# hangg7/soar

Hardware: AMD Instinct MI355X
Metric: fwd+bwd frames/sec @100k Gaussians, 1080p; achieved HBM GB/s vs roofline (higher is better)
Workload: dtype f32

## Files before the change

### include/soar_hip.h

```cpp
#ifndef SOAR_HIP_H
#define SOAR_HIP_H

#include <stddef.h>
#include <stdint.h>

#ifdef __cplusplus
extern "C" {
#endif

#define SOAR_HIP_ABI_VERSION 8

typedef struct SoarRastParams {
    int32_t P;
    int32_t W, H;
    int32_t sh_degree;
    int32_t M;
    int32_t prefiltered;
    int32_t render_front;
    int32_t sort_descending;
    int32_t debug;
    int32_t cfg_surface;
    int32_t cfg_normalize_depth;
    int32_t cfg_perpix_depth;
    int32_t cfg_lrn_cam;
// ... 38 lines not shown
                             void *geom_buffer, void *binning_buffer, void *image_buffer,
                             int64_t num_rendered,
                             float *out_color, float *out_normal, float *out_depth, float *out_opac,
                             void *stream);

int soar_rast_forward_render_occ(const SoarRastParams *prm, const int32_t *radii,
                                 void *geom_buffer, void *binning_buffer, void *image_buffer,
                                 int64_t num_rendered,
                                 float *out_color, float *out_normal, float *out_depth, float *out_opac,
                                 const float *occ_values, float *out_occ,
                                 void *stream);

int soar_rast_backward(const SoarRastParams *prm,
                       const float *means3D, const int32_t *radii, const float *shs,
                       const float *colors_precomp, const float *scales, const float *rotations,
                       const float *cov3D_precomp,
                       const void *geom_buffer, const void *binning_buffer, const void *image_buffer,
                       int64_t num_rendered,
                       const float *dL_dout_color, const float *dL_dout_normal,
                       const float *dL_dout_depth, const float *dL_dout_opac,
                       float *dL_dmeans2D, float *dL_dcolors, float *dL_dopacity, float *dL_dmeans3D,
                       float *dL_dcov3D, float *dL_dsh, float *dL_dscales, float *dL_drotations,
                       float *dL_dviewmat, float *dL_dprojmat, float *dL_dcampos,
                       void *workspace, size_t workspace_bytes,
                       void *stream);
int soar_rast_occ_backward(const SoarRastParams *prm, const void *geom_buffer, const void *binning_buffer,
                           const void *image_buffer, int64_t num_rendered, const float *dL_dout_occ, float *dL_docc,
                           void *stream);
int soar_rast_backward_occ(const SoarRastParams *prm,
                           const float *means3D, const int32_t *radii, const float *shs,
                           const float *colors_precomp, const float *scales, const float *rotations,
                           const float *cov3D_precomp,
                           const void *geom_buffer, const void *binning_buffer, const void *image_buffer,
                           int64_t num_rendered,
                           const float *dL_dout_color, const float *dL_dout_normal,
                           const float *dL_dout_depth, const float *dL_dout_opac, const float *dL_dout_occ,
                           const float *normal_scale_dev,
                           int32_t occ_planes,
                           float *dL_dmeans2D, float *dL_dcolors, float *dL_dopacity, float *dL_dmeans3D,
                           float *dL_dcov3D, float *dL_dsh, float *dL_dscales, float *dL_drotations,
                           float *dL_dviewmat, float *dL_dprojmat, float *dL_dcampos, float *dL_docc,
                           void *workspace, size_t workspace_bytes,
                           void *stream);
int soar_rast_backward_scaled(const SoarRastParams *prm,
                              const float *means3D, const int32_t *radii, const float *shs,
                              const float *colors_precomp, const float *scales, const float *rotations,
                              const float *cov3D_precomp,
                              const void *geom_buffer, const void *binning_buffer, const void *image_buffer,
                              int64_t num_rendered,
                              const float *dL_dout_color, const float *dL_dout_normal,
                              const float *dL_dout_depth, const float *dL_dout_opac, const float *grad_scale_dev,
                              float *dL_dmeans2D, float *dL_dcolors, float *dL_dopacity, float *dL_dmeans3D,
                              float *dL_dcov3D, float *dL_dsh, float *dL_dscales, float *dL_drotations,
                              float *dL_dviewmat, float *dL_dprojmat, float *dL_dcampos,
                              void *workspace, size_t workspace_bytes,
                              void *stream);
int soar_rast_backward_plan(const SoarRastParams *prm, int32_t region,
                            const float *means3D, const int32_t *radii, const float *shs,
                            const float *colors_precomp, const float *scales, const float *rotations,
                            const float *cov3D_precomp,
                            const void *geom_buffer, const void *binning_buffer, const void *image_buffer,
                            int64_t num_rendered,
                            const float *dL_dout_color, const float *dL_dout_normal,
                            const float *dL_dout_depth, const float *dL_dout_opac,
                            float *dL_dmeans2D, float *dL_dcolors, float *dL_dopacity, float *dL_dmeans3D,
                            float *dL_dcov3D, float *dL_dsh, float *dL_dscales, float *dL_drotations,
                            float *dL_dviewmat, float *dL_dprojmat, float *dL_dcampos,
                            void *workspace, size_t workspace_bytes,
                            void *stream);
int soar_rast_backward_occ_plan(const SoarRastParams *prm, int32_t region,
                                const float *means3D, const int32_t *radii, const float *shs,
                                const float *colors_precomp, const float *scales, const float *rotations,
                                const float *cov3D_precomp,
                                const void *geom_buffer, const void *binning_buffer, const void *image_buffer,
                                int64_t num_rendered,
                                const float *dL_dout_color, const float *dL_dout_normal,
                                const float *dL_dout_depth, const float *dL_dout_opac, const float *dL_dout_occ,
                                const float *normal_scale_dev, int32_t occ_planes,
                                float *dL_dmeans2D, float *dL_dcolors, float *dL_dopacity, float *dL_dmeans3D,
                                float *dL_dcov3D, float *dL_dsh, float *dL_dscales, float *dL_drotations,
                                float *dL_dviewmat, float *dL_dprojmat, float *dL_dcampos, float *dL_docc,
                                void *workspace, size_t workspace_bytes,
                                void *stream);
int soar_rast_backward_region_counts(int64_t *single_blocks, int64_t *pairs);
int soar_rast_backward_workspace_bytes(int32_t P, size_t *bytes);

int soar_rast_mark_visible(int32_t P, const float *means3D, const float *viewmatrix, const float *projmatrix,
                           uint8_t *present, void *stream);

int soar_rast_export_state(const SoarRastParams *prm, const void *geom_buffer, const void *binning_buffer,
                           const void *image_buffer, int64_t num_rendered,
                           float *means2D, float *depths, float *conic_opacity, float *normal,
                           float *depth_plane, float *rgb, float *cov3D,
                           uint32_t *tiles_touched, uint32_t *point_offsets,
                           uint64_t *keys_unsorted, uint32_t *vals_unsorted,
                           uint64_t *keys_sorted, uint32_t *point_list, uint32_t *ranges,
                           float *final_T, float *final_D, uint32_t *n_contrib, void *stream);

int soar_lbs_knn_weights_bytes(int32_t P, int32_t V, size_t *bytes);
int soar_lbs_knn_weights(const float *xyz, int32_t P, const float *verts, int32_t V,
                         const float *vert_weights, int32_t J, int32_t K,
                         float *weights_out, int32_t *knn_idx_out,
                         void *workspace, size_t workspace_bytes, void *stream);

int soar_lbs_knn_grid_bytes(int32_t V, size_t *bytes);
int soar_lbs_knn_query_bytes(int32_t P, size_t *bytes);
int soar_lbs_knn_build_grid(const float *verts, int32_t V, const float *vert_weights, int32_t J, void *grid_buffer,
                            void *stream);
int soar_lbs_knn_query(const void *grid_buffer, int32_t V, const float *vert_weights, int32_t J,
                       const float *xyz, int32_t P, int32_t K, float *weights_out, int32_t *knn_idx_out,
                       void *query_workspace, size_t query_workspace_bytes, void *stream);
int soar_lbs_knn_query_ordered(const void *grid_buffer, int32_t V, const float *vert_weights, int32_t J,
                               const float *xyz, int32_t P, int32_t K, uint32_t *order, int32_t resort,
                               float *weights_out, int32_t *knn_idx_out,
                               void *query_workspace, size_t query_workspace_bytes, void *stream);

int soar_lbs_knn_state_bytes(int32_t P, size_t *bytes);
int soar_lbs_knn_query_state(const void *grid_buffer, int32_t V, const float *vert_weights, int32_t J, const float *xyz, int32_t P,
                             uint32_t *order, int32_t resort, float *weights_out, void *state_buffer, void *query_workspace,
                             size_t query_workspace_bytes, void *stream);
int soar_lbs_knn_refresh(const void *grid_buffer, int32_t V, int32_t J, const float *xyz, int32_t P, const uint32_t *order,
                         void *state_buffer, float *weights_out, uint32_t *searched_counter_dev, void *stream);

int soar_lbs_warp_forward(const float *xyz, const float *rot, const float *weights, const float *joint_mats,
                          const float *offsets, const float *axis_perm, int32_t P, int32_t J,
                          float *xyz_out, float *rot_out, float *pt_mats_out, void *stream);

int soar_lbs_warp_backward(const float *xyz, const float *rot, const float *weights, const float *joint_mats,
                           const float *axis_perm, int32_t P, int32_t J,
                           const float *dL_dxyz_out, const float *dL_drot_out,
                           float *dL_dxyz, float *dL_drot, void *stream);

typedef struct SoarFrameHead {
    const SoarRastParams *prm;
    void *geom_buffer;
    int32_t *radii;
} SoarFrameHead;
int soar_frames_warp_preprocess(int32_t n, const SoarFrameHead *frames, const float *xyz, const float *rot, const float *weights,
                                const float *joint_mats, int32_t P, int32_t J, const float *colors, const float *opacities, const float *scales,
                                float *xyz_out, float *rot_out, void *stream);

int soar_rast_backward_rows(const SoarRastParams *prm, const float *means3D, const int32_t *radii, const float *shs, const float *scales,
                            const float *rotations, const float *cov3D_precomp, const void *geom_buffer, const void *workspace,
                            float *dL_dmeans2D, float *dL_dcolors, float *dL_dopacity, float *dL_dmeans3D, float *dL_dcov3D, float *dL_dsh,
                            float *dL_dscales, float *dL_drotations, float *dL_dviewmat, float *dL_dprojmat, float *dL_dcampos, float *dL_docc,
                            void *stream);

typedef struct SoarFrameTail {
    const SoarRastParams *prm;
    const float *means3D;
    const float *rotations;
    const int32_t *radii;
    const void *geom_buffer;
    const void *workspace;
    float *dL_dmeans2D;
} SoarFrameTail;
int soar_frames_geometry_warp_backward(int32_t n, const SoarFrameTail *frames, const float *xyz, const float *rot, const float *weights,
                                       const float *joint_mats, int32_t P, int32_t J, const float *scales, float *dL_dxyz, float *dL_drot,
                                       float *dL_dscales, float *dL_dcolors, float *dL_docc, void *stream);
typedef struct SoarLossFinish {
    const float *sums4;
    float *loss_out;
    int32_t blocks, n;
    float w_color, w_mask, w_normal, w_depth;
} SoarLossFinish;
int soar_frames_geometry_warp_backward_losses(int32_t n, const SoarFrameTail *frames, const float *xyz, const float *rot,
// ... 114 lines not shown
    int32_t scale_width;
    int32_t warp;
    const float *xyz, *rot;
    const float *weights;
    const float *joint_mats;
    const float *offsets;
    const float *axis_perm;
    const float *colors;
    const float *scale_src;
    const float *occ;
    float *occ3;
    float *posed;
    float *grad_scratch;
    float *dL_dxyz, *dL_drot, *dL_dcolors, *dL_dscale;
    float *dL_docc;
} SoarPoseArgs;
typedef struct SoarViewArgs {
    SoarRastParams rast;
    float focal_k00, focal_k11;
    int32_t back;
    int32_t pad_;
    int64_t capacity;
    void *buffer;
    size_t buffer_bytes;
    float *out;
    int32_t *radii;
    uint32_t *status_pinned;
    const float *g_render, *g_normal, *g_depth, *g_pred_normal, *g_mask, *g_occ, *g_curv;
    float *dL_dmeans2D;
} SoarViewArgs;
int soar_view_buffer_bytes(int32_t P, int32_t W, int32_t H, int64_t capacity, int32_t back, size_t *bytes);
int soar_views_grad_scratch_floats(int32_t P, int32_t n_views, size_t *floats);
int soar_views_forward(const SoarPoseArgs *pose, int32_t n_views, const SoarViewArgs *views, void *stream);
int soar_views_backward(const SoarPoseArgs *pose, int32_t n_views, const SoarViewArgs *views, void *stream);
int soar_step_views_forward(int32_t n_poses, const SoarPoseArgs *poses, const int32_t *views_per_pose, const SoarViewArgs *views, void *stream);
int soar_step_views_backward(int32_t n_poses, const SoarPoseArgs *poses, const int32_t *views_per_pose, const SoarViewArgs *views, void *stream);
typedef struct SoarCameraSpec {
    double fovx, fovy, znear, zfar;
    double cx, cy, img_w, img_h;
    int32_t has_cxcy, pad_;
} SoarCameraSpec;
int soar_cameras_from_c2w(int32_t n, const float *c2w_dev, const float *c2w_host, const SoarCameraSpec *specs, float *out_dev, void *stream);
int soar_rast_forward_render_status(const SoarRastParams *prm, const int32_t *radii, void *geom_buffer, void *binning_buffer,
                                    void *image_buffer, int64_t num_rendered, float *out_color, float *out_normal, float *out_depth,
                                    float *out_opac, const float *occ_values, float *out_occ, uint32_t *status_pinned, void *stream);
int soar_lbs_warp_backward_views(const float *xyz, const float *rot, const float *weights, const float *joint_mats, const float *axis_perm,
                                 int32_t n, int32_t P, int32_t J, const float *dL_dxyz_out, const float *dL_drot_out, float *dL_dxyz,
                                 float *dL_drot, int32_t n_extra, const float *const *extra_src, float *const *extra_dst,
                                 const int32_t *extra_width, void *stream);

int soar_prof_enable(int on);
int soar_prof_reset(void);
int soar_prof_stage_count(void);
const char *soar_prof_stage_name(int stage);
int soar_prof_read(int stage, double *total_ms, int64_t *launches);
int soar_sum_frames(int32_t n_frames, int64_t count, const float *in_dev, float *out_dev, void *stream);
int soar_gather_step_inputs(int32_t n_frames, int32_t num_frames_seq, int32_t floats_per_frame, int32_t n_sets,
                            const int32_t *frame_ids_dev, const float *table_dev, float *mats_out_dev,
                            int32_t *set_index_out_dev, void *stream);
int soar_gather_step_inputs_ids(int32_t n_frames, int32_t num_frames_seq, int32_t floats_per_frame, int32_t n_sets,
                                const int32_t *frame_ids_host, const float *table_dev, float *mats_out_dev,
                                int32_t *set_index_out_dev, void *stream);

typedef struct SoarAdamRow {
    float *param;
    const float *grad;
    float *exp_avg;
    float *exp_avg_sq;
    int64_t count;
    float lr;
    int32_t pad_;
} SoarAdamRow;
int soar_adam_step(int32_t n_rows, const SoarAdamRow *rows_host, double beta1, double beta2, double eps, void *state_dev, void *stream);
int soar_adam_step_at(int32_t n_rows, const SoarAdamRow *rows, double beta1, double beta2, double eps, int64_t step, void *stream);
int soar_adam_step_at_gather(int32_t n_rows, const SoarAdamRow *rows, double beta1, double beta2, double eps, int64_t step,
                             int32_t n_frames, int32_t num_frames_seq, int32_t floats_per_frame, int32_t n_sets,
                             const int32_t *frame_ids_host, const float *table_dev, float *mats_out_dev, int32_t *set_index_out_dev,
                             void *stream);
int soar_adam_step_rows(int32_t n_rows, const SoarAdamRow *rows, double beta1, double beta2, double eps, void *state_dev, int32_t advance,
                        void *stream);
int soar_adam_step_rows_wide(int32_t n_rows, const SoarAdamRow *rows, double beta1, double beta2, double eps, void *state_dev,
                             int32_t advance, void *stream);

int soar_prof_timestamp(unsigned long long *ring_dev, int64_t capacity, int64_t tag, void *stream);

int soar_selftest_affine_scan(const float *m64_dev, const float *b64_dev, float *out192_dev, void *stream);

int soar_selftest_exp(const float *x_dev, int32_t n, float *out_dev, float *expf_dev, void *stream);

int soar_tsdf_integrate(int32_t n_views, int32_t H, int32_t W, const float *depth, const float *opac, const float *viewmatrix,
                        const float *projmatrix, const float *prcppoint, float origin_x, float origin_y, float origin_z, float voxel,
                        int32_t X, int32_t Y, int32_t Z, float trunc, float znear, float min_opacity, float *sum, float *weight,
                        void *stream);
int soar_mc_workspace_bytes(int32_t X, int32_t Y, int32_t Z, size_t *bytes);
int soar_mc_count(int32_t X, int32_t Y, int32_t Z, const float *values, const uint8_t *valid, float level, void *workspace,
                  size_t workspace_bytes, int64_t *counts_host, void *stream);
int soar_mc_emit(int32_t X, int32_t Y, int32_t Z, const float *values, const uint8_t *valid, float level, const void *workspace,
                 size_t workspace_bytes, float *verts, int32_t *faces, void *stream);
int soar_mesh_filter_bytes(int32_t V, int32_t F, size_t *bytes);
int soar_mesh_filter_components(int32_t V, int32_t F, const float *verts, const int32_t *faces, int32_t min_faces, float min_diag_frac,
                                void *workspace, size_t workspace_bytes, float *verts_out, int32_t *faces_out, int64_t *counts_host,
                                void *stream);
int soar_mesh_simplify_bytes(int32_t V, int32_t F, size_t *bytes);
int soar_mesh_simplify_count(int32_t V, int32_t F, const float *verts, const int32_t *faces, float cell, void *workspace,
                             size_t workspace_bytes, int64_t *counts_host, void *stream);
int soar_mesh_simplify(int32_t V, int32_t F, const float *verts, const int32_t *faces, float cell, void *workspace,
                       size_t workspace_bytes, float *verts_out, int32_t *faces_out, int64_t *counts_host, void *stream);
int soar_mesh_attr_transfer_bytes(int32_t V, int32_t K, size_t *bytes);
int soar_mesh_attr_transfer(int32_t V, int32_t N, int32_t K, const float *verts, const float *points, const float *colors,
                            const int32_t *idx, void *workspace, size_t workspace_bytes, float *color_out, float *quality_out,
                            float *d2_out, void *stream);
int soar_mesh_adjacency_bytes(int32_t V, int32_t F, size_t *bytes);
int soar_mesh_adjacency(int32_t V, int32_t F, const int32_t *faces, void *workspace, size_t workspace_bytes, int32_t *row_start,
                        int32_t *nbr, uint8_t *border, void *stream);
int soar_mesh_smooth_bytes(int32_t V, size_t *bytes);
int soar_mesh_smooth(int32_t V, int32_t nnz, const float *verts, const int32_t *row_start, const int32_t *nbr, const uint8_t *border,
                     int32_t steps, void *workspace, size_t workspace_bytes, float *verts_out, void *stream);
int soar_mesh_prune_bytes(int32_t V, int32_t F, size_t *bytes);
int soar_mesh_prune(int32_t V, int32_t F, const float *verts, const int32_t *faces, const float *quality, float thresh, void *workspace,
                    size_t workspace_bytes, float *verts_out, int32_t *faces_out, int32_t *keep_out, int64_t *counts_host, void *stream);
int soar_mesh_close_holes_bytes(int32_t V, int32_t F, size_t *bytes);
int soar_mesh_close_holes(int32_t V, int32_t F, const float *verts, const int32_t *faces, int32_t max_hole_edges, void *workspace,
                          size_t workspace_bytes, float *verts_out, int32_t *faces_out, int32_t *loop_edges_out, int64_t *counts_host,
                          void *stream);

#define SOAR_FIELD_LEVELS 16
#define SOAR_FIELD_HIDDEN 64
#define SOAR_FIELD_HEAD_FLOATS(in, out) (SOAR_FIELD_HIDDEN * (in) + SOAR_FIELD_HIDDEN + (out) * SOAR_FIELD_HIDDEN + (out))
typedef struct SoarFieldHead {
    const float *w1, *b1, *w2, *b2;
} SoarFieldHead;

typedef struct SoarFieldArgs {
    int32_t N;
    int32_t log2_T;
    int32_t normalized;
    int32_t pad_;
    float res[SOAR_FIELD_LEVELS];
    const float *xyz;
    const float *aabb;
    const float *table, *qtable;
    const float *z;
    SoarFieldHead head[5];
    float *enc, *qenc;
    float *out[5];
    const float *g_out[5];
    float *d_table, *d_qtable;
    float *d_head[5];
    float *d_xyz, *d_z;
} SoarFieldArgs;

int soar_field_workspace_bytes(int32_t N, size_t *bytes);
int soar_field_forward(const SoarFieldArgs *args, void *stream);
int soar_field_backward(const SoarFieldArgs *args, void *workspace, size_t workspace_bytes, void *stream);

#define SOAR_ENVMAP_ENC 9
#define SOAR_ENVMAP_HIDDEN 16
#define SOAR_ENVMAP_WEIGHTS (SOAR_ENVMAP_HIDDEN * SOAR_ENVMAP_ENC + SOAR_ENVMAP_HIDDEN * SOAR_ENVMAP_HIDDEN + 3 * SOAR_ENVMAP_HIDDEN)
typedef struct SoarEnvmapArgs {
    int32_t B, H, W;
    int32_t n_comp;
    int32_t color_rows;
    int32_t pad_;
    int64_t render_stride, mask_stride;
    int64_t g_comp_stride[4];
    const float *dirs;
// ... 166 lines not shown
```

### soar_amd/csrc/api.hip

```cpp
#include "soar_common.h"

#include <mutex>

#include <dlfcn.h>

#include <cstdarg>
#include <cstdio>
#include <cstring>

namespace soar {

static thread_local char g_error[1024] = "";

void set_error(const char *fmt, ...)
{
    va_list ap;
    va_start(ap, fmt);
    vsnprintf(g_error, sizeof(g_error), fmt, ap);
    va_end(ap);
}

int check_hip(hipError_t e, const char *what, const char *file, int line)
{
    if (e == hipSuccess) return 0;
// ... 531 lines not shown
            const soar::BatchCtx &bc = soar::batch_ctx();
            if (!bc.n || pending_serial != bc.serial) pending.clear();
            pending_serial = bc.serial;
            status_pinned[0] = 0xFFFFFFFFu;
            status_pinned[1] = 0xFFFFFFFFu;
            pending.push_back({status_pinned, g.header + H_TOTAL});
            if (!bc.n || bc.f == bc.n - 1) {
                for (const auto &c : pending)
                    SOAR_HIP_OK(hipMemcpyAsync(c.first, c.second, 2 * sizeof(uint32_t), hipMemcpyDeviceToHost, stream));
                pending.clear();
            }
        }
    } else {
        if (launch_scan(*prm, g, stream)) return 1;
        if (launch_binning(*prm, g, b, img, num_rendered, stream)) return 1;
    }
    if (num_rendered > 0 && launch_tile_order_binned(*prm, g, b, img, num_rendered, stream)) return 1;
    if (launch_render_forward(*prm, g, b, img, out_color, out_normal, out_depth, out_opac, occ_values, out_occ, stream)) return 1;
    return 0;
}

int soar_rast_occ_backward(const SoarRastParams *prm, const void *geom_buffer, const void *binning_buffer, const void *image_buffer,
                           int64_t num_rendered, const float *dL_dout_occ, float *dL_docc, void *stream_)
{
    hipStream_t stream = static_cast<hipStream_t>(stream_);
    if (check_params(prm)) return 1;
    if (prm->P == 0) return 0;
    if (!dL_dout_occ || !dL_docc) { set_error("soar_rast_occ_backward: a required pointer is NULL"); return 1; }
    if (prm->sort_descending || prm->render_front) {
        set_error("soar_rast_occ_backward: the fused occlusion pass belongs to a main pass with render_front = 0 and sort_descending = 0");
        return 1;
    }
    if (check_aligned(geom_buffer, "geom_buffer") || check_aligned(image_buffer, "image_buffer")) return 1;
    if (num_rendered > 0 && check_aligned(binning_buffer, "binning_buffer")) return 1;
    GeomBuf g;
    ImageBuf img;
    BinBuf b;
    carve_geom(const_cast<void *>(geom_buffer), prm->P, prm->M, &g);
    carve_image(const_cast<void *>(image_buffer), prm->W, prm->H, &img);
    carve_binning(const_cast<void *>(binning_buffer), num_rendered, &b);
    return launch_occ_backward(*prm, g, b, img, dL_dout_occ, dL_docc, stream);
}

int soar_rast_backward(const SoarRastParams *prm, const float *means3D, const int32_t *radii, const float *shs,
                       const float *colors_precomp, const float *scales, const float *rotations,
                       const float *cov3D_precomp, const void *geom_buffer, const void *binning_buffer,
                       const void *image_buffer, int64_t num_rendered, const float *dL_dout_color,
                       const float *dL_dout_normal, const float *dL_dout_depth, const float *dL_dout_opac,
                       float *dL_dmeans2D, float *dL_dcolors, float *dL_dopacity, float *dL_dmeans3D, float *dL_dcov3D,
                       float *dL_dsh, float *dL_dscales, float *dL_drotations, float *dL_dviewmat, float *dL_dprojmat,
                       float *dL_dcampos, void *workspace, size_t workspace_bytes, void *stream_)
{
    return soar_rast_backward_scaled(prm, means3D, radii, shs, colors_precomp, scales, rotations, cov3D_precomp, geom_buffer,
                                     binning_buffer, image_buffer, num_rendered, dL_dout_color, dL_dout_normal, dL_dout_depth,
                                     dL_dout_opac, nullptr, dL_dmeans2D, dL_dcolors, dL_dopacity, dL_dmeans3D, dL_dcov3D, dL_dsh,
                                     dL_dscales, dL_drotations, dL_dviewmat, dL_dprojmat, dL_dcampos, workspace, workspace_bytes,
                                     stream_);
}

int soar_rast_backward_rows(const SoarRastParams *prm, const float *means3D, const int32_t *radii, const float *shs, const float *scales,
                            const float *rotations, const float *cov3D_precomp, const void *geom_buffer, const void *workspace,
                            float *dL_dmeans2D, float *dL_dcolors, float *dL_dopacity, float *dL_dmeans3D, float *dL_dcov3D, float *dL_dsh,
                            float *dL_dscales, float *dL_drotations, float *dL_dviewmat, float *dL_dprojmat, float *dL_dcampos, float *dL_docc,
                            void *stream_)
{
    hipStream_t stream = static_cast<hipStream_t>(stream_);
    if (check_params(prm)) return 1;
    if (prm->P == 0) return 0;
    if (check_aligned(geom_buffer, "geom_buffer") || check_aligned(workspace, "workspace")) return 1;
    if (!means3D || !radii || !dL_dmeans2D || !dL_dcolors || !dL_dopacity || !dL_dmeans3D || !dL_dcov3D || !dL_dscales || !dL_drotations ||
        !dL_dviewmat || !dL_dprojmat || !dL_dcampos) {
        set_error("soar_rast_backward_rows: a required pointer is NULL");
        return 1;
    }
    GeomBuf g;
    carve_geom(const_cast<void *>(geom_buffer), prm->P, prm->M, &g);
    return launch_geometry_backward(*prm, means3D, radii, shs, scales, rotations, cov3D_precomp, g, static_cast<const float *>(workspace),
                                    dL_dmeans2D, dL_dcolors, dL_dopacity, dL_dmeans3D, dL_dcov3D, dL_dsh, dL_dscales, dL_drotations,
                                    dL_dviewmat, dL_dprojmat, dL_dcampos, true, stream, dL_docc);
}

}

static int backward_impl(const SoarRastParams *prm, const float *means3D, const int32_t *radii, const float *shs,
                              const float *colors_precomp, const float *scales, const float *rotations,
                              const float *cov3D_precomp, const void *geom_buffer, const void *binning_buffer,
                              const void *image_buffer, int64_t num_rendered, const float *dL_dout_color,
                              const float *dL_dout_normal, const float *dL_dout_depth, const float *dL_dout_opac,
                              const float *grad_scale_dev, float *dL_dmeans2D, float *dL_dcolors, float *dL_dopacity,
                              float *dL_dmeans3D, float *dL_dcov3D, float *dL_dsh, float *dL_dscales, float *dL_drotations,
                              float *dL_dviewmat, float *dL_dprojmat, float *dL_dcampos, void *workspace,
                              size_t workspace_bytes, const float *dL_dout_occ, float *dL_docc, const float *normal_scale_dev, int occ_planes,
                              int region, void *stream_)
{
    hipStream_t stream = static_cast<hipStream_t>(stream_);
    if (check_params(prm)) return 1;
    if (!dL_dviewmat || !dL_dprojmat || !dL_dcampos) { set_error("camera gradient pointers must not be NULL"); return 1; }
    if ((dL_dout_occ == nullptr) != (dL_docc == nullptr)) { set_error("soar_rast_backward_occ: dL_dout_occ and dL_docc go together"); return 1; }
    if (dL_dout_occ && (prm->render_front != 0 || prm->sort_descending != 0)) {
        set_error("soar_rast_backward_occ: the fused occlusion chain belongs to a main pass (render_front = 0, ascending)");
        return 1;
    }
    if (prm->P == 0) {
        SOAR_HIP_OK(hipMemsetAsync(dL_dviewmat, 0, 16 * sizeof(float), stream));
        SOAR_HIP_OK(hipMemsetAsync(dL_dprojmat, 0, 16 * sizeof(float), stream));
        SOAR_HIP_OK(hipMemsetAsync(dL_dcampos, 0, 3 * sizeof(float), stream));
        return 0;
    }
    if (check_aligned(geom_buffer, "geom_buffer") || check_aligned(image_buffer, "image_buffer") ||
        check_aligned(workspace, "workspace"))
        return 1;
    if (num_rendered > 0 && check_aligned(binning_buffer, "binning_buffer")) return 1;
    size_t need = 0;
    soar_rast_backward_workspace_bytes(prm->P, &need);
    if (workspace_bytes < need - ALIGN) { set_error("workspace too small: %zu < %zu", workspace_bytes, need); return 1; }
    if (!means3D || !radii || !dL_dout_color || !dL_dout_normal || !dL_dout_depth || !dL_dout_opac || !dL_dmeans2D ||
        !dL_dcolors || !dL_dopacity || !dL_dmeans3D || !dL_dcov3D || !dL_dscales || !dL_drotations) {
        set_error("soar_rast_backward: a required pointer is NULL");
        return 1;
    }
    if (prm->M > 0 && shs && !dL_dsh) { set_error("dL_dsh is NULL but SHs are in use"); return 1; }
    (void)colors_precomp;

    GeomBuf g;
    ImageBuf img;
    BinBuf b;
    carve_geom(const_cast<void *>(geom_buffer), prm->P, prm->M, &g);
    carve_image(const_cast<void *>(image_buffer), prm->W, prm->H, &img);
    carve_binning(const_cast<void *>(binning_buffer), num_rendered, &b);
    float *acc = static_cast<float *>(workspace);
    const bool wide = (prm->debug & 2) != 0;
    double *acc64 = wide ? reinterpret_cast<double *>(static_cast<char *>(workspace) + align_up(sizeof(float) * ACC_STRIDE * (size_t)prm->P))
                         : nullptr;
    {
        const ZeroRange zr[4] = {{wide ? (void *)acc64 : (void *)acc, (wide ? sizeof(double) : sizeof(float)) * ACC_STRIDE * (size_t)prm->P},
                                 {dL_dviewmat, 16 * sizeof(float)}, {dL_dprojmat, 16 * sizeof(float)}, {dL_dcampos, 3 * sizeof(float)}};
        if (launch_zero_ranges(zr, 4, stream)) return 1;
    }
    if (num_rendered > 0 || wide) {
        if (launch_render_backward(*prm, g, b, img, dL_dout_color, dL_dout_normal, dL_dout_depth, dL_dout_opac, grad_scale_dev, acc,
                                   acc64, num_rendered > 0, dL_dout_occ, dL_docc, normal_scale_dev, occ_planes, region, stream))
            return 1;
    }
    if ((prm->debug & 8) != 0) return 0;
    if (launch_geometry_backward(*prm, means3D, radii, shs, scales, rotations, cov3D_precomp, g, acc, dL_dmeans2D, dL_dcolors,
                                 dL_dopacity, dL_dmeans3D, dL_dcov3D, dL_dsh, dL_dscales, dL_drotations, dL_dviewmat,
                                 dL_dprojmat, dL_dcampos, false, stream, dL_docc))
        return 1;
    return 0;
}


extern "C" {

int soar_rast_backward_scaled(const SoarRastParams *prm, const float *means3D, const int32_t *radii, const float *shs,
                              const float *colors_precomp, const float *scales, const float *rotations,
                              const float *cov3D_precomp, const void *geom_buffer, const void *binning_buffer,
                              const void *image_buffer, int64_t num_rendered, const float *dL_dout_color,
                              const float *dL_dout_normal, const float *dL_dout_depth, const float *dL_dout_opac,
                              const float *grad_scale_dev, float *dL_dmeans2D, float *dL_dcolors, float *dL_dopacity,
                              float *dL_dmeans3D, float *dL_dcov3D, float *dL_dsh, float *dL_dscales, float *dL_drotations,
                              float *dL_dviewmat, float *dL_dprojmat, float *dL_dcampos, void *workspace,
                              size_t workspace_bytes, void *stream_)
{
    return backward_impl(prm, means3D, radii, shs, colors_precomp, scales, rotations, cov3D_precomp, geom_buffer, binning_buffer, image_buffer,
                         num_rendered, dL_dout_color, dL_dout_normal, dL_dout_depth, dL_dout_opac, grad_scale_dev, dL_dmeans2D, dL_dcolors,
                         dL_dopacity, dL_dmeans3D, dL_dcov3D, dL_dsh, dL_dscales, dL_drotations, dL_dviewmat, dL_dprojmat, dL_dcampos, workspace,
                         workspace_bytes, nullptr, nullptr, nullptr, 3, 0, stream_);
}

int soar_rast_backward_occ(const SoarRastParams *prm, const float *means3D, const int32_t *radii, const float *shs,
                           const float *colors_precomp, const float *scales, const float *rotations,
                           const float *cov3D_precomp, const void *geom_buffer, const void *binning_buffer,
                           const void *image_buffer, int64_t num_rendered, const float *dL_dout_color,
                           const float *dL_dout_normal, const float *dL_dout_depth, const float *dL_dout_opac,
                           const float *dL_dout_occ, const float *normal_scale_dev, int32_t occ_planes, float *dL_dmeans2D, float *dL_dcolors,
                           float *dL_dopacity,
                           float *dL_dmeans3D, float *dL_dcov3D, float *dL_dsh, float *dL_dscales, float *dL_drotations,
                           float *dL_dviewmat, float *dL_dprojmat, float *dL_dcampos, float *dL_docc, void *workspace,
                           size_t workspace_bytes, void *stream_)
{
    if (!dL_dout_occ || !dL_docc) { set_error("soar_rast_backward_occ: dL_dout_occ / dL_docc must not be NULL"); return 1; }
    if (occ_planes != 1 && occ_planes != 3) { set_error("soar_rast_backward_occ: occ_planes is 3 or 1, got %d", occ_planes); return 1; }
    return backward_impl(prm, means3D, radii, shs, colors_precomp, scales, rotations, cov3D_precomp, geom_buffer, binning_buffer, image_buffer,
                         num_rendered, dL_dout_color, dL_dout_normal, dL_dout_depth, dL_dout_opac, nullptr, dL_dmeans2D, dL_dcolors,
                         dL_dopacity, dL_dmeans3D, dL_dcov3D, dL_dsh, dL_dscales, dL_drotations, dL_dviewmat, dL_dprojmat, dL_dcampos, workspace,
                         workspace_bytes, dL_dout_occ, dL_docc, normal_scale_dev, occ_planes, 0, stream_);
}

int soar_rast_backward_plan(const SoarRastParams *prm, int32_t region, const float *means3D, const int32_t *radii, const float *shs,
                            const float *colors_precomp, const float *scales, const float *rotations,
                            const float *cov3D_precomp, const void *geom_buffer, const void *binning_buffer,
                            const void *image_buffer, int64_t num_rendered, const float *dL_dout_color,
                            const float *dL_dout_normal, const float *dL_dout_depth, const float *dL_dout_opac,
                            float *dL_dmeans2D, float *dL_dcolors, float *dL_dopacity, float *dL_dmeans3D, float *dL_dcov3D,
                            float *dL_dsh, float *dL_dscales, float *dL_drotations, float *dL_dviewmat, float *dL_dprojmat,
                            float *dL_dcampos, void *workspace, size_t workspace_bytes, void *stream_)
{
    if (region != 1 && region != 2) { set_error("soar_rast_backward_plan: region is 1 or 2, got %d", region); return 1; }
    return backward_impl(prm, means3D, radii, shs, colors_precomp, scales, rotations, cov3D_precomp, geom_buffer, binning_buffer, image_buffer,
                         num_rendered, dL_dout_color, dL_dout_normal, dL_dout_depth, dL_dout_opac, nullptr, dL_dmeans2D, dL_dcolors,
                         dL_dopacity, dL_dmeans3D, dL_dcov3D, dL_dsh, dL_dscales, dL_drotations, dL_dviewmat, dL_dprojmat, dL_dcampos, workspace,
                         workspace_bytes, nullptr, nullptr, nullptr, 3, region, stream_);
}

int soar_rast_backward_occ_plan(const SoarRastParams *prm, int32_t region, const float *means3D, const int32_t *radii, const float *shs,
                                const float *colors_precomp, const float *scales, const float *rotations,
                                const float *cov3D_precomp, const void *geom_buffer, const void *binning_buffer,
                                const void *image_buffer, int64_t num_rendered, const float *dL_dout_color,
                                const float *dL_dout_normal, const float *dL_dout_depth, const float *dL_dout_opac,
                                const float *dL_dout_occ, const float *normal_scale_dev, int32_t occ_planes, float *dL_dmeans2D,
                                float *dL_dcolors, float *dL_dopacity, float *dL_dmeans3D, float *dL_dcov3D, float *dL_dsh,
                                float *dL_dscales, float *dL_drotations, float *dL_dviewmat, float *dL_dprojmat, float *dL_dcampos,
                                float *dL_docc, void *workspace, size_t workspace_bytes, void *stream_)
{
    if (region != 1 && region != 2) { set_error("soar_rast_backward_occ_plan: region is 1 or 2, got %d", region); return 1; }
    if (!dL_dout_occ || !dL_docc) { set_error("soar_rast_backward_occ_plan: dL_dout_occ / dL_docc must not be NULL"); return 1; }
    if (occ_planes != 1 && occ_planes != 3) { set_error("soar_rast_backward_occ_plan: occ_planes is 3 or 1, got %d", occ_planes); return 1; }
    return backward_impl(prm, means3D, radii, shs, colors_precomp, scales, rotations, cov3D_precomp, geom_buffer, binning_buffer, image_buffer,
                         num_rendered, dL_dout_color, dL_dout_normal, dL_dout_depth, dL_dout_opac, nullptr, dL_dmeans2D, dL_dcolors,
                         dL_dopacity, dL_dmeans3D, dL_dcov3D, dL_dsh, dL_dscales, dL_drotations, dL_dviewmat, dL_dprojmat, dL_dcampos, workspace,
                         workspace_bytes, dL_dout_occ, dL_docc, normal_scale_dev, occ_planes, region, stream_);
}

int soar_rast_backward_region_counts(int64_t *single_blocks, int64_t *pairs)
{
    if (!single_blocks || !pairs) { set_error("soar_rast_backward_region_counts: NULL"); return 1; }
    long long s = 0, p = 0;
    render_backward_region_counts(&s, &p);
    *single_blocks = (int64_t)s; *pairs = (int64_t)p;
    return 0;
}

int soar_rast_mark_visible(int32_t P, const float *means3D, const float *viewmatrix, const float *projmatrix,
                           uint8_t *present, void *stream_)
{
    (void)means3D; (void)viewmatrix; (void)projmatrix;
    hipStream_t stream = static_cast<hipStream_t>(stream_);
    if (P < 0) { set_error("P < 0"); return 1; }
    if (P == 0) return 0;
    if (!present) { set_error("present is NULL"); return 1; }
    SOAR_HIP_OK(hipMemsetAsync(present, 0, (size_t)P, stream));
    return 0;
}

}

namespace soar {
namespace {
__global__ void export_records_kernel(int P, const GaussRec *rec, float *means2D, float *depths, float *conic_opacity,
                                      float *normal, float *depth_plane, float *rgb)
{
    const int i = blockIdx.x * blockDim.x + threadIdx.x;
    if (i >= P) return;
    const GaussRec r = rec[i];
    if (means2D) { means2D[2 * i] = r.q0.x; means2D[2 * i + 1] = r.q0.y; }
    if (depths) depths[i] = r.q1.z;
    if (conic_opacity) {
        conic_opacity[4 * i] = r.q0.z; conic_opacity[4 * i + 1] = r.q0.w; conic_opacity[4 * i + 2] = r.q1.x;
        conic_opacity[4 * i + 3] = r.q1.y;
    }
    if (normal) { normal[3 * i] = r.q3.x; normal[3 * i + 1] = r.q3.y; normal[3 * i + 2] = r.q3.z; }
    if (depth_plane) { depth_plane[2 * i] = r.q1.w; depth_plane[2 * i + 1] = r.q2.x; }
    if (rgb) { rgb[3 * i] = r.q2.y; rgb[3 * i + 1] = r.q2.z; rgb[3 * i + 2] = r.q2.w; }
}
__global__ void __launch_bounds__(1024) export_pack_ranges_kernel(int T, const uint2 *__restrict__ ranges, uint2 *__restrict__ packed,
                                                                  int descending)
{
    __shared__ uint32_t part[1024];
    const int tid = threadIdx.x, per = (T + 1023) / 1024, t0 = tid * per, t1 = min(T, t0 + per);
    auto tile = [&](int k) { return descending ? T - 1 - k : k; };
    uint32_t s = 0;
    for (int k = t0; k < t1; k++) s += ranges[tile(k)].y - ranges[tile(k)].x;
    part[tid] = s;
    __syncthreads();
    if (tid == 0) {
        uint32_t run = 0;
        for (int k = 0; k < 1024; k++) { const uint32_t c = part[k]; part[k] = run; run += c; }
    }
    __syncthreads();
    uint32_t run = part[tid];
    for (int k = t0; k < t1; k++) {
        const int t = tile(k);
        const uint32_t c = ranges[t].y - ranges[t].x;
        packed[t] = c ? make_uint2(run, run + c) : make_uint2(0u, 0u);
        run += c;
    }
}
__global__ void __launch_bounds__(64) export_pack_lists_kernel(const uint2 *__restrict__ ranges, const uint2 *__restrict__ packed,
                                                               const uint32_t *__restrict__ list, uint32_t *__restrict__ out)
{
    const uint2 from = ranges[blockIdx.x], to = packed[blockIdx.x];
    for (uint32_t k = threadIdx.x; k < from.y - from.x; k += 64) out[to.x + k] = list[from.x + k];
}

}
}

extern "C" int soar_rast_export_state(const SoarRastParams *prm, const void *geom_buffer, const void *binning_buffer,
                                      const void *image_buffer, int64_t num_rendered, float *means2D, float *depths,
                                      float *conic_opacity, float *normal, float *depth_plane, float *rgb, float *cov3D,
                                      uint32_t *tiles_touched, uint32_t *point_offsets, uint64_t *keys_unsorted,
                                      uint32_t *vals_unsorted, uint64_t *keys_sorted, uint32_t *point_list,
                                      uint32_t *ranges, float *final_T, float *final_D, uint32_t *n_contrib, void *stream_)
{
// ... 64 lines not shown
```

### soar_amd/csrc/lbs_knn.hip

```cpp
#include "soar_common.h"

#include <cstdio>
#include <cstdlib>
#include <cstring>
#include <rocprim/device/device_radix_sort.hpp>

namespace soar {

namespace {

constexpr int KNN_THREADS = 128;
constexpr int KNN_MAXK = 32;
constexpr int GRID_MAX = 64;
constexpr int GRID_RES = 28;
constexpr int KNN_K = 30;
constexpr int KNN_JMAX = 56;
constexpr int GRID_CELLS = GRID_MAX * GRID_MAX * GRID_MAX;

struct GridMeta {
    float minx, miny, minz, h, inv_h;
    int nx, ny, nz;
};

__global__ void __launch_bounds__(256) grid_meta_kernel(const float *__restrict__ verts, int V, GridMeta *meta)
{
    __shared__ float lo[3][256], hi[3][256];
    const int tid = threadIdx.x;
    float l[3] = {3.0e38f, 3.0e38f, 3.0e38f}, h[3] = {-3.0e38f, -3.0e38f, -3.0e38f};
    for (int v = tid; v < V; v += 256)
#pragma unroll
        for (int k = 0; k < 3; k++) {
            const float c = verts[3 * v + k];
            l[k] = fminf(l[k], c);
            h[k] = fmaxf(h[k], c);
        }
#pragma unroll
    for (int k = 0; k < 3; k++) { lo[k][tid] = l[k]; hi[k][tid] = h[k]; }
    __syncthreads();
    for (int s = 128; s > 0; s >>= 1) {
        if (tid < s)
#pragma unroll
            for (int k = 0; k < 3; k++) {
                lo[k][tid] = fminf(lo[k][tid], lo[k][tid + s]);
                hi[k][tid] = fmaxf(hi[k][tid], hi[k][tid + s]);
            }
        __syncthreads();
    }
    if (tid == 0) {
        const float ex = hi[0][0] - lo[0][0], ey = hi[1][0] - lo[1][0], ez = hi[2][0] - lo[2][0];
        const float ext = fmaxf(fmaxf(ex, ey), fmaxf(ez, 1e-6f));
        GridMeta m;
        m.h = ext / GRID_RES;
        m.inv_h = 1.0f / m.h;
        m.minx = lo[0][0]; m.miny = lo[1][0]; m.minz = lo[2][0];
        m.nx = min(GRID_MAX, (int)(ex * m.inv_h) + 1);
        m.ny = min(GRID_MAX, (int)(ey * m.inv_h) + 1);
        m.nz = min(GRID_MAX, (int)(ez * m.inv_h) + 1);
        *meta = m;
    }
}

__device__ __forceinline__ int cell_coord(float v, float lo, float inv_h, int n)
{
    return min(n - 1, max(0, (int)floorf((v - lo) * inv_h)));
}

__global__ void __launch_bounds__(256)
grid_cells_kernel(const float *__restrict__ verts, int V, const GridMeta *__restrict__ meta, uint32_t *__restrict__ keys,
                  uint32_t *__restrict__ vals)
{
    const int v = blockIdx.x * 256 + threadIdx.x;
    if (v >= V) return;
    const GridMeta m = *meta;
    const int cx = cell_coord(verts[3 * v], m.minx, m.inv_h, m.nx);
    const int cy = cell_coord(verts[3 * v + 1], m.miny, m.inv_h, m.ny);
    const int cz = cell_coord(verts[3 * v + 2], m.minz, m.inv_h, m.nz);
    keys[v] = (uint32_t)((cz * GRID_MAX + cy) * GRID_MAX + cx);
    vals[v] = (uint32_t)v;
}

__global__ void __launch_bounds__(256)
grid_ranges_kernel(const float *__restrict__ verts, int V, const uint32_t *__restrict__ keys_sorted,
// ... 573 lines not shown
}

constexpr int KNN_FSLOTS = 4;
struct KnnSlots { uint2 list[KNN_FSLOTS][KNN_KEEP]; int p[KNN_FSLOTS]; };
__device__ __forceinline__ void slots_fill_pair(KnnSlots &sl, int slot_lo, int p, uint32_t mask, uint32_t pos, float d2, int lane)
{
    const int slot = slot_lo + (lane >> 5), l5 = lane & (KNN_KEEP - 1);
    if (p >= 0 && ((mask >> l5) & 1u)) {
        const int at = __builtin_popcount(mask & ((1u << l5) - 1u));
        sl.list[slot][at] = make_uint2(pos * (uint32_t)(KNN_JMAX * sizeof(float)), __float_as_uint(1.0f / fminf(fmaxf(sqrtf(d2), 0.0001f), 1.0f)));
    }
    if (l5 == 0) sl.p[slot] = p;
}
template <int UNROLL>
__device__ __forceinline__ void slots_blend(KnnSlots &sl, int lane, const float *__restrict__ rows_padded, int J,
                                            float *__restrict__ weights_out)
{
    static_assert(KNN_K % 2 == 0 && KNN_JMAX % 4 == 0 && KNN_JMAX / 4 <= 16 && KNN_FSLOTS * 16 == WAVE && KNN_KEEP * 2 == WAVE &&
                  KNN_JMAX * sizeof(float) <= KNN_KEEP * sizeof(uint2) && KNN_JMAX <= WAVE, "slot layout");
    __builtin_amdgcn_fence(__ATOMIC_RELEASE, "wavefront");
    __builtin_amdgcn_wave_barrier();
    __builtin_amdgcn_fence(__ATOMIC_ACQUIRE, "wavefront");
    const int g = lane >> 4, t = lane & 15;
    const int p = sl.p[g];
    if (p >= 0) {
        const uint32_t t16 = (uint32_t)min(t, KNN_JMAX / 4 - 1) * 16u;
        const char *rows_bytes = reinterpret_cast<const char *>(rows_padded);
        const uint4 *mine = reinterpret_cast<const uint4 *>(sl.list[g]);
        float4 acc = make_float4(0.f, 0.f, 0.f, 0.f);
        float norm = 0.f;
#pragma unroll UNROLL
        for (int k2 = 0; k2 < KNN_K / 2; k2++) {
            const uint4 e = mine[k2];
            const float4 r0 = *reinterpret_cast<const float4 *>(rows_bytes + (e.x + t16));
            const float4 r1 = *reinterpret_cast<const float4 *>(rows_bytes + (e.z + t16));
            const float w0 = __uint_as_float(e.y), w1 = __uint_as_float(e.w);
            acc.x = __builtin_fmaf(w0, r0.x, acc.x); acc.y = __builtin_fmaf(w0, r0.y, acc.y);
            acc.z = __builtin_fmaf(w0, r0.z, acc.z); acc.w = __builtin_fmaf(w0, r0.w, acc.w);
            norm += w0;
            acc.x = __builtin_fmaf(w1, r1.x, acc.x); acc.y = __builtin_fmaf(w1, r1.y, acc.y);
            acc.z = __builtin_fmaf(w1, r1.z, acc.z); acc.w = __builtin_fmaf(w1, r1.w, acc.w);
            norm += w1;
        }
        float4 *mine_out = reinterpret_cast<float4 *>(sl.list[g]);
        if (t < KNN_JMAX / 4) mine_out[t] = make_float4(acc.x / norm, acc.y / norm, acc.z / norm, acc.w / norm);
    }
    __builtin_amdgcn_fence(__ATOMIC_RELEASE, "wavefront");
    __builtin_amdgcn_wave_barrier();
    __builtin_amdgcn_fence(__ATOMIC_ACQUIRE, "wavefront");
#pragma unroll
    for (int r = 0; r < KNN_FSLOTS; r++) {
        const int pr = sl.p[r];
        if (pr >= 0 && lane < J) weights_out[(size_t)pr * J + lane] = reinterpret_cast<const float *>(sl.list[r])[lane];
    }
    __builtin_amdgcn_fence(__ATOMIC_RELEASE, "wavefront");
    __builtin_amdgcn_wave_barrier();
}

__device__ __forceinline__ uint32_t rank_32_halves(float d2, int lane, float &h30)
{
    const int l5 = lane & (KNN_KEEP - 1), base = lane & KNN_KEEP;
    int rank = 0;
#pragma unroll
    for (int j = 0; j < KNN_KEEP; j++) {
        const float dj = __shfl(d2, base + j);
        rank += (dj < d2 || (dj == d2 && j < l5)) ? 1 : 0;
    }
    const bool in = rank < KNN_K;
    float d_in = in ? d2 : 0.f, d_out = in ? 3.0e38f : d2;
#pragma unroll
    for (int off = KNN_KEEP / 2; off > 0; off >>= 1) {
        d_in = fmaxf(d_in, __shfl_xor(d_in, off));
        d_out = fminf(d_out, __shfl_xor(d_out, off));
    }
    h30 = half_gap(d_in, d_out);
    const unsigned long long b = __ballot(in);
    return (uint32_t)(base ? (b >> 32) : b);
}

#ifndef SOAR_KNN_CERT_PAIRS
#define SOAR_KNN_CERT_PAIRS 2
#endif
constexpr int KNN_CERT_PAIRS = SOAR_KNN_CERT_PAIRS;
__global__ void __launch_bounds__(KNN_WAVES *WAVE)
knn_certify_kernel(const float *__restrict__ xyz, int P, const float4 *__restrict__ sorted_verts, const uint32_t *__restrict__ order,
                   KnnStatePtrs st)
{
    const int wave = threadIdx.x >> 6, lane = threadIdx.x & 63, l5 = lane & (KNN_KEEP - 1);
    const int q_base = ((int)blockIdx.x * KNN_WAVES + wave) * (2 * KNN_CERT_PAIRS) + (lane >> 5);
    if (q_base - (lane >> 5) >= P) return;
    int qs[KNN_CERT_PAIRS];
    float4 ra[KNN_CERT_PAIRS], rb[KNN_CERT_PAIRS], vv[KNN_CERT_PAIRS];
    float xs[KNN_CERT_PAIRS], ys[KNN_CERT_PAIRS], zs[KNN_CERT_PAIRS];
#pragma unroll
    for (int i = 0; i < KNN_CERT_PAIRS; i++) {
        qs[i] = q_base + 2 * i;
        const int qc = min(qs[i], P - 1);
        const int p = order ? (int)order[qc] : qc;
        const uint32_t pos = st.nbr[(size_t)qc * KNN_STATE_STRIDE + l5];
        ra[i] = st.ref30[qc]; rb[i] = st.ref32[qc];
        xs[i] = xyz[3 * p]; ys[i] = xyz[3 * p + 1]; zs[i] = xyz[3 * p + 2];
        vv[i] = sorted_verts[pos];
    }
#pragma unroll
    for (int i = 0; i < KNN_CERT_PAIRS; i++) {
        const int q = qs[i];
        const bool valid = q < P;
        const float x = xs[i], y = ys[i], z = zs[i];
        const float d2 = dist2_exact(x, y, z, vv[i]);
        const float ax = x - ra[i].x, ay = y - ra[i].y, az = z - ra[i].z, bx = x - rb[i].x, by = y - rb[i].y, bz = z - rb[i].z;
        const float moved_a = __builtin_amdgcn_sqrtf((ax * ax + ay * ay) + az * az) * 1.0001f + 1.0e-12f;
        const float moved_b = __builtin_amdgcn_sqrtf((bx * bx + by * by) + bz * bz) * 1.0001f + 1.0e-12f;
        const bool ok_a = ra[i].w > 0.f && moved_a < ra[i].w, ok_b = rb[i].w > 0.f && moved_b < rb[i].w;
        const bool tier3 = valid && !ok_a && !ok_b, tier2 = valid && !ok_a && ok_b;
        if (__ballot(tier3)) {
            float far = d2;
#pragma unroll
            for (int off = KNN_KEEP / 2; off > 0; off >>= 1) far = fmaxf(far, __shfl_xor(far, off));
            if (tier3 && l5 == 0) {
                const uint32_t list = knn_work_list_of((uint32_t)q);
                uint32_t *item = knn_work_item(st.work, P, list, atomicAdd(st.work + list * KNN_WORK_LINE, 1u));
                item[0] = (uint32_t)q;
                item[1] = __float_as_uint(far);
            }
        }
        if (__ballot(tier2)) {
            float h30;
            const uint32_t mask = rank_32_halves(d2, lane, h30);
            if (tier2 && l5 == 0) { st.ref30[q] = make_float4(x, y, z, h30); st.in30[q] = mask; }
        }
        if (valid) st.d2[(size_t)q * KNN_STATE_STRIDE + l5] = tier3 ? -1.f : d2;
    }
}

#ifndef SOAR_KNN_SEARCH_BLOCKS
#define SOAR_KNN_SEARCH_BLOCKS 768
#endif
#ifndef SOAR_KNN_BS_WPE
#define SOAR_KNN_BS_WPE 4
#endif
__global__ void __launch_bounds__(KNN_WAVES *WAVE) __attribute__((amdgpu_waves_per_eu(SOAR_KNN_BS_WPE, 8)))
knn_blend_search_kernel(const float *__restrict__ xyz, int P, int search_blocks, const GridMeta *__restrict__ meta,
                        const uint2 *__restrict__ cell_range, const float4 *__restrict__ sorted_verts, const float *__restrict__ rows_padded,
                        int J, const uint32_t *__restrict__ order, KnnStatePtrs st, float *__restrict__ weights_out,
                        uint32_t *__restrict__ counters)
{
    constexpr int KEEP = KNN_KEEP;
    __shared__ uint32_t c_pos[KNN_WAVES][RF_CAP];
    __shared__ float c_d[KNN_WAVES][RF_CAP];
    __shared__ uint32_t row_first[KNN_WAVES][WAVE], row_end[KNN_WAVES][WAVE];
    __shared__ __attribute__((aligned(16))) KnnSlots slots[KNN_WAVES];
    const int wave = threadIdx.x >> 6, lane = threadIdx.x & 63;
    if ((int)blockIdx.x >= search_blocks) {
        const int q0 = (((int)blockIdx.x - search_blocks) * KNN_WAVES + wave) * KNN_FSLOTS;
        if (q0 >= P) return;
        const int l5 = lane & (KNN_KEEP - 1);
        float dd[2];
        uint32_t pp[2], mm[2];
        int pq[2];
#pragma unroll
        for (int r = 0; r < 2; r++) {
            const int q = q0 + 2 * r + (lane >> 5);
            const size_t at = (size_t)min(q, P - 1) * KNN_STATE_STRIDE + l5;
            dd[r] = st.d2[at];
            pp[r] = st.nbr[at];
            mm[r] = st.in30[min(q, P - 1)];
            pq[r] = order ? (int)order[min(q, P - 1)] : min(q, P - 1);
            if (q >= P) dd[r] = -1.f;
        }
#pragma unroll
        for (int r = 0; r < 2; r++) slots_fill_pair(slots[wave], 2 * r, dd[r] >= 0.f ? pq[r] : -1, mm[r], pp[r], dd[r], lane);
        slots_blend<SOAR_KNN_SLOT_UNROLL>(slots[wave], lane, rows_padded, J, weights_out);
        return;
    }
    uint32_t *cp = c_pos[wave];
    float *cd = c_d[wave];
    const GridMeta m = *meta;
    const uint32_t searcher = blockIdx.x * KNN_WAVES + wave, my_list = searcher % KNN_WORK_LISTS;
    const uint32_t n_mine = min(st.work[my_list * KNN_WORK_LINE], knn_work_cap(P));
    for (uint32_t w = searcher / KNN_WORK_LISTS; w < n_mine; w += (uint32_t)search_blocks * KNN_WAVES / KNN_WORK_LISTS) {
        const uint32_t *item = knn_work_item(st.work, P, my_list, w);
        const size_t q = item[0];
        const float tau_ub = __uint_as_float(item[1]);
        const int p = order ? (int)order[q] : (int)q;
        const float x = xyz[3 * p], y = xyz[3 * p + 1], z = xyz[3 * p + 2];
        int n_in = 0;
        float next_d2 = 3.0e38f, ball2 = 0.f;
        bool sane = (x - x == 0.f) && (y - y == 0.f) && (z - z == 0.f) && (tau_ub >= 0.f);
        int growths = 0;
        for (float grow = 1.0f + 1.0f / 15.0f; sane; grow *= 1.3f) {
            if (++growths > 96) { sane = false; break; }
            const float ball = sqrtf(tau_ub) * grow + 1.0e-6f;
            ball2 = ball * ball;
            const float rho = ball * 1.0001f + 1.0e-7f;
            const int cx0 = cell_coord(x - rho, m.minx, m.inv_h, m.nx), cx1 = cell_coord(x + rho, m.minx, m.inv_h, m.nx);
            const int cy0 = cell_coord(y - rho, m.miny, m.inv_h, m.ny), cy1 = cell_coord(y + rho, m.miny, m.inv_h, m.ny);
            const int cz0 = cell_coord(z - rho, m.minz, m.inv_h, m.nz), cz1 = cell_coord(z + rho, m.minz, m.inv_h, m.nz);
            const int ny_b = cy1 - cy0 + 1, n_rows = ny_b * (cz1 - cz0 + 1);
            n_in = 0;
            next_d2 = 3.0e38f;
            auto select_keep = [&]() {
                if (n_in <= WAVE) {
                    const bool have = lane < n_in;
                    const uint32_t pos0 = have ? cp[lane] : 0u;
                    const float d0 = have ? cd[lane] : 3.0e38f;
                    int rk = 0;
                    for (int j = 0; j < n_in; j++) {
                        const float dj = __int_as_float(__builtin_amdgcn_readlane(__float_as_int(d0), j));
                        rk += (dj < d0 || (dj == d0 && j < lane)) ? 1 : 0;
                    }
                    const bool keep = have && rk < KEEP;
                    const unsigned long long km = __ballot(keep);
                    if (keep) {
                        const int at = (int)__builtin_amdgcn_mbcnt_hi((uint32_t)(km >> 32), __builtin_amdgcn_mbcnt_lo((uint32_t)km, 0u));
                        cp[at] = pos0;
                        cd[at] = d0;
                    }
                    float dropped = (have && !keep) ? d0 : 3.0e38f;
#pragma unroll
                    for (int off = 32; off > 0; off >>= 1) dropped = fminf(dropped, __shfl_xor(dropped, off));
                    next_d2 = fminf(next_d2, dropped);
                    n_in = (int)__builtin_popcountll(km);
                    __builtin_amdgcn_fence(__ATOMIC_RELEASE, "wavefront");
                    __builtin_amdgcn_wave_barrier();
                    return;
                }
                uint32_t e_pos[RF_CAP / WAVE];
                float e_d[RF_CAP / WAVE];
// ... 77 lines not shown
#pragma unroll
                for (int u = 0; u < TRIPS; u++) {
                    const int g0 = g00 + u * WAVE;
                    if (g0 >= n_cand) break;
                    const int g = g0 + lane;
                    const uint32_t t = tt[u];
                    const bool have = g < n_cand;
                    const float d = have ? dist2_exact(x, y, z, vv[u]) : 3.0e38f;
                    const bool in = d <= tau_cur;
                    float out_d = (have && !in) ? d : 3.0e38f;
#pragma unroll
                    for (int off = 32; off > 0; off >>= 1) out_d = fminf(out_d, __shfl_xor(out_d, off));
                    next_d2 = fminf(next_d2, out_d);
                    const unsigned long long im = __ballot(in);
                    if (im == 0ull) continue;
                    if (n_in + (int)__builtin_popcountll(im) > RF_CAP) {
                        select_keep();
                        float worst = lane < KEEP ? cd[lane] : 0.f;
#pragma unroll
                        for (int off = 32; off > 0; off >>= 1) worst = fmaxf(worst, __shfl_xor(worst, off));
                        tau_cur = worst;
                    }
                    const bool in2 = d <= tau_cur;
                    const unsigned long long im2 = __ballot(in2);
                    if (in2) {
                        const int at = n_in + (int)__builtin_amdgcn_mbcnt_hi((uint32_t)(im2 >> 32), __builtin_amdgcn_mbcnt_lo((uint32_t)im2, 0u));
                        cp[at] = t;
                        cd[at] = d;
                    }
                    float out2 = (in && !in2) ? d : 3.0e38f;
#pragma unroll
                    for (int off = 32; off > 0; off >>= 1) out2 = fminf(out2, __shfl_xor(out2, off));
                    next_d2 = fminf(next_d2, out2);
                    n_in += (int)__builtin_popcountll(im2);
                    __builtin_amdgcn_fence(__ATOMIC_RELEASE, "wavefront");
                    __builtin_amdgcn_wave_barrier();
                }
                }
                __builtin_amdgcn_fence(__ATOMIC_RELEASE, "wavefront");
                __builtin_amdgcn_wave_barrier();
            }
            if (n_in >= KEEP) { select_keep(); break; }
        }
        if (!sane) {
            const float nan = __uint_as_float(0x7FC00000u);
            if (lane < J) weights_out[(size_t)p * J + lane] = nan;
            if (lane == 0) {
                st.ref30[q] = make_float4(x, y, z, -1.f);
                st.ref32[q] = make_float4(x, y, z, -1.f);
            }
            continue;
        }
        const uint32_t pos = lane < KEEP ? cp[lane] : 0u;
        const float d2 = lane < KEEP ? cd[lane] : 3.0e38f;
        float far = lane < KEEP ? d2 : 0.f;
#pragma unroll
        for (int off = 32; off > 0; off >>= 1) far = fmaxf(far, __shfl_xor(far, off));
        const float h32 = half_gap(far, fminf(next_d2, ball2));
        float h30;
        const uint32_t mask = rank_32(lane < KEEP ? d2 : 3.0e38f, lane, h30);
        if (lane < KEEP) st.nbr[q * KNN_STATE_STRIDE + lane] = pos;
        if (lane == 0) {
            st.ref30[q] = make_float4(x, y, z, h30);
            st.ref32[q] = make_float4(x, y, z, h32);
            st.in30[q] = mask;
        }
        __builtin_amdgcn_fence(__ATOMIC_RELEASE, "wavefront");
        __builtin_amdgcn_wave_barrier();
        slots_fill_pair(slots[wave], 0, lane < KNN_KEEP ? p : -1, mask, pos, d2, lane);
        if (lane == 0) { slots[wave].p[2] = -1; slots[wave].p[3] = -1; }
        slots_blend<SOAR_KNN_SEARCH_UNROLL>(slots[wave], lane, rows_padded, J, weights_out);
    }
    if (lane == 0) {
        uint32_t *line = st.work + my_list * KNN_WORK_LINE;
        if (atomicAdd(line + 1, 1u) == (uint32_t)search_blocks * KNN_WAVES / KNN_WORK_LISTS - 1u) {
            const uint32_t n = line[0];
            if (counters && n) atomicAdd(counters, n);
            line[0] = 0u;
            line[1] = 0u;
        }
    }
}

}

}

using namespace soar;

namespace {

struct KnnGrid {
    GridMeta *meta;
    uint2 *cell_range;
    float4 *sorted_verts;
    float *rows;
    uint32_t *k0, *k1, *v0, *v1;
    void *sort_tmp;
    size_t sort_bytes;
    size_t total;
};

int carve_knn_grid(void *base, int32_t V, KnnGrid *g, hipStream_t stream)
{
    size_t sort_bytes = 0;
    (void)rocprim::radix_sort_pairs((void *)nullptr, sort_bytes, (uint32_t *)nullptr, (uint32_t *)nullptr,
                                    (uint32_t *)nullptr, (uint32_t *)nullptr, (size_t)V, 0u, 18u, stream);
    char *b = static_cast<char *>(base);
    size_t off = 0;
    auto carve = [&](size_t n) { size_t o = off; off = align_up(off + n); return b + o; };
    g->meta = reinterpret_cast<GridMeta *>(carve(sizeof(GridMeta)));
    g->cell_range = reinterpret_cast<uint2 *>(carve(sizeof(uint2) * (size_t)GRID_CELLS));
    g->sorted_verts = reinterpret_cast<float4 *>(carve(sizeof(float4) * (size_t)V));
    g->rows = reinterpret_cast<float *>(carve(sizeof(float) * (size_t)V * KNN_JMAX));
    g->k0 = reinterpret_cast<uint32_t *>(carve(4 * (size_t)V));
    g->k1 = reinterpret_cast<uint32_t *>(carve(4 * (size_t)V));
    g->v0 = reinterpret_cast<uint32_t *>(carve(4 * (size_t)V));
    g->v1 = reinterpret_cast<uint32_t *>(carve(4 * (size_t)V));
    g->sort_tmp = carve(sort_bytes);
    g->sort_bytes = sort_bytes;
    g->total = off + ALIGN;
    return 0;
}

int knn_build(const float *verts, int32_t V, const float *vert_weights, int32_t J, const KnnGrid &g, hipStream_t stream)
{
    hipLaunchKernelGGL(grid_meta_kernel, dim3(1), dim3(256), 0, stream, verts, V, g.meta);
    hipLaunchKernelGGL(grid_cells_kernel, dim3((V + 255) / 256), dim3(256), 0, stream, verts, V, g.meta, g.k0, g.v0);
    size_t sort_bytes = g.sort_bytes;
    SOAR_HIP_OK(rocprim::radix_sort_pairs(g.sort_tmp, sort_bytes, g.k0, g.k1, g.v0, g.v1, (size_t)V, 0u, 18u, stream));
    SOAR_HIP_OK(hipMemsetAsync(g.cell_range, 0, sizeof(uint2) * (size_t)GRID_CELLS, stream));
    hipLaunchKernelGGL(grid_ranges_kernel, dim3((V + 255) / 256), dim3(256), 0, stream, verts, V, g.k1, g.v1, g.cell_range,
                       g.sorted_verts);
    if (J <= KNN_JMAX)
        hipLaunchKernelGGL(pad_rows_kernel, dim3((V * KNN_JMAX + 255) / 256), dim3(256), 0, stream, vert_weights, V, J,
                           g.sorted_verts, g.rows);
    SOAR_LAUNCH_OK("lbs_knn_build_grid", stream, 0);
    return 0;
}

struct QueryWs {
    size_t sort_bytes, total;
    uint32_t *qk0, *qk1, *qv0, *qv1;
    uint32_t *item_cost, *item_order;
};
int carve_query_ws(void *base, int32_t P, QueryWs *out, hipStream_t stream)
{
    size_t qsort_bytes = 0;
    (void)rocprim::radix_sort_pairs((void *)nullptr, qsort_bytes, (uint32_t *)nullptr, (uint32_t *)nullptr,
                                    (uint32_t *)nullptr, (uint32_t *)nullptr, (size_t)(P > 0 ? P : 1), 0u, 18u, stream);
    size_t off = 0;
    auto carve = [&](size_t n) { size_t o = off; off = align_up(off + n); return o; };
    const size_t o_tmp = carve(qsort_bytes), o_qk0 = carve(4 * (size_t)P), o_qk1 = carve(4 * (size_t)P),
                 o_qv0 = carve(4 * (size_t)P), o_qv1 = carve(4 * (size_t)P), o_cost = carve(4 * KNN_SLOTS * (((size_t)P + WAVE - 1) / WAVE)),
                 o_ord = carve(4 * (KNN_SLOTS * (((size_t)P + WAVE - 1) / WAVE) + 1));
    (void)o_tmp;
    char *b = static_cast<char *>(base);
    out->sort_bytes = qsort_bytes;
    out->total = off;
    out->qk0 = reinterpret_cast<uint32_t *>(b + o_qk0); out->qk1 = reinterpret_cast<uint32_t *>(b + o_qk1);
    out->qv0 = reinterpret_cast<uint32_t *>(b + o_qv0); out->qv1 = reinterpret_cast<uint32_t *>(b + o_qv1);
    out->item_cost = reinterpret_cast<uint32_t *>(b + o_cost); out->item_order = reinterpret_cast<uint32_t *>(b + o_ord);
    return 0;
}

struct KnnState { KnnStatePtrs p; size_t total; };
// ... 112 lines not shown
    hipStream_t stream = static_cast<hipStream_t>(stream_);
    if (check_knn_sizes(P, V, J, K)) return 1;
    if (P == 0) return 0;
    if (!grid_buffer || !xyz || !vert_weights || !weights_out) { set_error("soar_lbs_knn_query: NULL pointer"); return 1; }
    if (check_ws("soar_lbs_knn_query", query_workspace, query_workspace_bytes)) return 1;
    KnnGrid g;
    if (carve_knn_grid(const_cast<void *>(grid_buffer), V, &g, stream)) return 1;
    StageTimer timer(ST_LBS_KNN, stream);
    return knn_query(g, V, vert_weights, J, xyz, P, K, weights_out, knn_idx_out, nullptr, 1, query_workspace, query_workspace_bytes,
                     stream);
}

extern "C" int soar_lbs_knn_query_ordered(const void *grid_buffer, int32_t V, const float *vert_weights, int32_t J, const float *xyz,
                                          int32_t P, int32_t K, uint32_t *order, int32_t resort, float *weights_out,
                                          int32_t *knn_idx_out, void *query_workspace, size_t query_workspace_bytes, void *stream_)
{
    hipStream_t stream = static_cast<hipStream_t>(stream_);
    if (check_knn_sizes(P, V, J, K)) return 1;
    if (P == 0) return 0;
    if (!grid_buffer || !xyz || !vert_weights || !weights_out || !order) { set_error("soar_lbs_knn_query_ordered: NULL pointer"); return 1; }
    if (check_ws("soar_lbs_knn_query_ordered", query_workspace, query_workspace_bytes)) return 1;
    KnnGrid g;
    if (carve_knn_grid(const_cast<void *>(grid_buffer), V, &g, stream)) return 1;
    StageTimer timer(ST_LBS_KNN, stream);
    return knn_query(g, V, vert_weights, J, xyz, P, K, weights_out, knn_idx_out, order, resort, query_workspace,
                     query_workspace_bytes, stream);
}

extern "C" int soar_lbs_knn_state_bytes(int32_t P, size_t *bytes)
{
    if (P < 0 || !bytes) { set_error("soar_lbs_knn_state_bytes: bad arguments"); return 1; }
    KnnState st;
    carve_knn_state(nullptr, P, &st);
    *bytes = st.total;
    return 0;
}

extern "C" int soar_lbs_knn_query_state(const void *grid_buffer, int32_t V, const float *vert_weights, int32_t J, const float *xyz,
                                        int32_t P, uint32_t *order, int32_t resort, float *weights_out, void *state_buffer,
                                        void *query_workspace, size_t query_workspace_bytes, void *stream_)
{
    hipStream_t stream = static_cast<hipStream_t>(stream_);
    if (check_knn_sizes(P, V, J, KNN_K)) return 1;
    if (V < KNN_STATE_STRIDE) { set_error("soar_lbs_knn_query_state: the neighbour state keeps %d vertices per query, V=%d", KNN_STATE_STRIDE, V); return 1; }
    if (P == 0) return 0;
    if (!grid_buffer || !xyz || !vert_weights || !weights_out || !order || !state_buffer) { set_error("soar_lbs_knn_query_state: NULL pointer"); return 1; }
    if (check_ws("soar_lbs_knn_query_state", query_workspace, query_workspace_bytes) || check_ws("soar_lbs_knn_query_state", state_buffer, 0)) return 1;
    KnnGrid g;
    if (carve_knn_grid(const_cast<void *>(grid_buffer), V, &g, stream)) return 1;
    if (V <= KNN_KEEP) { set_error("soar_lbs_knn_query_state: the neighbour state keeps %d vertices per query, V = %d", KNN_KEEP, V); return 1; }
    KnnState st;
    carve_knn_state(state_buffer, P, &st);
    StageTimer timer(ST_LBS_KNN, stream);
    SOAR_HIP_OK(hipMemsetAsync(st.p.work, 0, KNN_WORK_LISTS * KNN_WORK_LINE * sizeof(uint32_t), stream));
    return knn_query(g, V, vert_weights, J, xyz, P, KNN_K, weights_out, nullptr, order, resort, query_workspace, query_workspace_bytes,
                     stream, &st);
}

extern "C" int soar_lbs_knn_refresh(const void *grid_buffer, int32_t V, int32_t J, const float *xyz, int32_t P, const uint32_t *order,
                                    void *state_buffer, float *weights_out, uint32_t *searched_counter_dev, void *stream_)
{
    hipStream_t stream = static_cast<hipStream_t>(stream_);
    if (check_knn_sizes(P, V, J, KNN_K)) return 1;
    if (J > KNN_JMAX) { set_error("soar_lbs_knn_refresh: J <= %d", KNN_JMAX); return 1; }
    if (V < KNN_STATE_STRIDE) { set_error("soar_lbs_knn_refresh: the neighbour state keeps %d vertices per query, V=%d", KNN_STATE_STRIDE, V); return 1; }
    if (P == 0) return 0;
    if (!grid_buffer || !xyz || !weights_out || !state_buffer || !order) { set_error("soar_lbs_knn_refresh: NULL pointer"); return 1; }
    if (check_ws("soar_lbs_knn_refresh", state_buffer, 0)) return 1;
    KnnGrid g;
    if (carve_knn_grid(const_cast<void *>(grid_buffer), V, &g, stream)) return 1;
    KnnState st;
    carve_knn_state(state_buffer, P, &st);
    StageTimer timer(ST_LBS_KNN, stream);
    const int per_block = KNN_WAVES * 2 * KNN_CERT_PAIRS, nblocks = (P + per_block - 1) / per_block;
    static_assert(SOAR_KNN_SEARCH_BLOCKS * KNN_WAVES % KNN_WORK_LISTS == 0, "searchers per list");
    hipLaunchKernelGGL(knn_certify_kernel, dim3(nblocks), dim3(KNN_WAVES * WAVE), 0, stream, xyz, P, g.sorted_verts, order, st.p);
    const int search_blocks = SOAR_KNN_SEARCH_BLOCKS, blend_blocks = (P + KNN_WAVES * KNN_FSLOTS - 1) / (KNN_WAVES * KNN_FSLOTS);
    hipLaunchKernelGGL(knn_blend_search_kernel, dim3(search_blocks + blend_blocks), dim3(KNN_WAVES * WAVE), 0, stream, xyz, P, search_blocks,
                       g.meta, g.cell_range, g.sorted_verts, g.rows, J, order, st.p, weights_out, searched_counter_dev);
    SOAR_LAUNCH_OK("lbs_knn_refresh", stream, 0);
    return 0;
}

extern "C" int soar_lbs_knn_weights_bytes(int32_t P, int32_t V, size_t *bytes)
{
    if (P < 0 || V <= 0 || !bytes) { set_error("soar_lbs_knn_weights_bytes: bad arguments"); return 1; }
    KnnGrid g;
    if (carve_knn_grid(nullptr, V, &g, nullptr)) return 1;
    QueryWs ws;
    if (carve_query_ws(nullptr, P, &ws, nullptr)) return 1;
    *bytes = align_up(g.total) + ws.total;
    return 0;
}

extern "C" int soar_lbs_knn_weights(const float *xyz, int32_t P, const float *verts, int32_t V, const float *vert_weights,
                                    int32_t J, int32_t K, float *weights_out, int32_t *knn_idx_out, void *workspace,
                                    size_t workspace_bytes, void *stream_)
{
    hipStream_t stream = static_cast<hipStream_t>(stream_);
    if (check_knn_sizes(P, V, J, K)) return 1;
    if (P == 0) return 0;
    if (!xyz || !verts || !vert_weights || !weights_out) { set_error("soar_lbs_knn_weights: NULL pointer"); return 1; }
    if (check_ws("soar_lbs_knn_weights", workspace, workspace_bytes)) return 1;
    KnnGrid g;
    if (carve_knn_grid(workspace, V, &g, stream)) return 1;
    QueryWs ws;
    if (carve_query_ws(nullptr, P, &ws, stream)) return 1;
    const size_t grid_part = align_up(g.total);
    if (workspace_bytes < grid_part + ws.total) {
        set_error("soar_lbs_knn_weights: workspace too small (%zu bytes, need %zu)", workspace_bytes, grid_part + ws.total);
        return 1;
    }
    StageTimer timer(ST_LBS_KNN, stream);
    if (knn_build(verts, V, vert_weights, J, g, stream)) return 1;
    return knn_query(g, V, vert_weights, J, xyz, P, K, weights_out, knn_idx_out, nullptr, 1,
                     static_cast<char *>(workspace) + grid_part, workspace_bytes - grid_part, stream);
}
```

### soar_amd/csrc/optim.hip

```cpp
#include "soar_common.h"

#include <cmath>
#include <cstdint>

namespace soar {

namespace {

constexpr int ADAM_MAX_ROWS = 8;
constexpr int ADAM_MAX_ROWS_WIDE = 40;
template <int N>
struct AdamTableT {
    SoarAdamRow row[N];
    int64_t first_block[N + 1];
    int n;
};
using AdamTable = AdamTableT<ADAM_MAX_ROWS>;
using AdamTableWide = AdamTableT<ADAM_MAX_ROWS_WIDE>;
struct AdamState {
    int32_t step;
    float bias_correction1, bias_correction2_sqrt;
    int32_t pad;
};

__global__ void adam_tick_kernel(AdamState *st, double beta1, double beta2)
{
    const int t = st->step + 1;
    st->step = t;
    st->bias_correction1 = (float)(1.0 - pow(beta1, (double)t));
    st->bias_correction2_sqrt = (float)sqrt(1.0 - pow(beta2, (double)t));
}

struct AdamGather {
    int n_frames, num_frames_seq, floats_per_frame, n_sets;
    int64_t first_block;
    int32_t id[MAX_BATCH];
    const float *table;
    float *mats_out;
    int32_t *set_out;
};

template <typename Table>
__global__ void __launch_bounds__(256) adam_update_kernel(Table tab, const AdamState *__restrict__ st_dev, AdamState st_host, float beta2,
                                                          float one_minus_b1, float one_minus_b2, float eps, AdamGather ga)
{
    if (ga.n_frames && (int64_t)blockIdx.x >= ga.first_block) {
        const int f = (int)((int64_t)blockIdx.x - ga.first_block);
        int id = ga.id[f] % ga.num_frames_seq;
        if (id < 0) id += ga.num_frames_seq;
        for (int k = threadIdx.x; k < ga.floats_per_frame; k += 256)
            ga.mats_out[(size_t)f * ga.floats_per_frame + k] = ga.table[(size_t)id * ga.floats_per_frame + k];
        if (threadIdx.x == 0 && ga.set_out) ga.set_out[f] = ga.n_sets > 0 ? id % ga.n_sets : 0;
        return;
    }
    const AdamState *st = st_dev ? st_dev : &st_host;
    if (st->step <= 0) return;
    int r = 0;
    while (r + 1 < tab.n && (int64_t)blockIdx.x >= tab.first_block[r + 1]) r++;
    const SoarAdamRow row = tab.row[r];
    const int64_t i0 = ((int64_t)blockIdx.x - tab.first_block[r]) * 1024 + threadIdx.x * 4;
    const float step_size = row.lr / st->bias_correction1, bc2s = st->bias_correction2_sqrt;
    auto update = [&](float g, float &p, float &m, float &v) {
#pragma clang fp contract(off)
        m = m + (g - m) * one_minus_b1;
        v = beta2 * v + one_minus_b2 * (g * g);
        const float denom = sqrtf(v) / bc2s + eps;
        p = p - step_size * (m / denom);
    };
    const bool vec = i0 + 3 < row.count && (((uintptr_t)row.param | (uintptr_t)row.grad | (uintptr_t)row.exp_avg | (uintptr_t)row.exp_avg_sq) & 15u) == 0u;
    if (vec) {
        const float4 g = *reinterpret_cast<const float4 *>(row.grad + i0);
        float4 p = *reinterpret_cast<const float4 *>(row.param + i0), m = *reinterpret_cast<const float4 *>(row.exp_avg + i0),
               v = *reinterpret_cast<const float4 *>(row.exp_avg_sq + i0);
        update(g.x, p.x, m.x, v.x); update(g.y, p.y, m.y, v.y); update(g.z, p.z, m.z, v.z); update(g.w, p.w, m.w, v.w);
        *reinterpret_cast<float4 *>(row.param + i0) = p;
        *reinterpret_cast<float4 *>(row.exp_avg + i0) = m;
        *reinterpret_cast<float4 *>(row.exp_avg_sq + i0) = v;
        return;
    }
    for (int k = 0; k < 4; k++) {
        const int64_t i = i0 + k;
        if (i >= row.count) break;
        float p = row.param[i], m = row.exp_avg[i], v = row.exp_avg_sq[i];
        update(row.grad[i], p, m, v);
        row.param[i] = p;
        row.exp_avg[i] = m;
        row.exp_avg_sq[i] = v;
    }
}

template <typename Table>
bool adam_fill(Table &tab, int32_t n_rows, const SoarAdamRow *rows_host, int max_rows, int64_t &blocks, const char *who)
{
    tab.n = n_rows;
    blocks = 0;
    for (int r = 0; r < n_rows; r++) {
        const SoarAdamRow &w = rows_host[r];
        if (w.count < 0 || (w.count && (!w.param || !w.grad || !w.exp_avg || !w.exp_avg_sq))) {
            set_error("%s: row %d has a NULL pointer or a negative count", who, r);
            return false;
        }
        tab.row[r] = w;
        tab.first_block[r] = blocks;
        blocks += (w.count + 1023) / 1024;
    }
    for (int r = n_rows; r <= max_rows; r++) tab.first_block[r] = blocks;
    return true;
}

}

}

using namespace soar;

extern "C" int soar_adam_step(int32_t n_rows, const SoarAdamRow *rows_host, double beta1, double beta2, double eps, void *state_dev,
                              void *stream_)
{
    return soar_adam_step_rows(n_rows, rows_host, beta1, beta2, eps, state_dev, 1, stream_);
}

static int adam_step_at(int32_t n_rows, const SoarAdamRow *rows_host, double beta1, double beta2, double eps, int64_t step,
                        const AdamGather *gather, hipStream_t stream);

extern "C" int soar_adam_step_at(int32_t n_rows, const SoarAdamRow *rows_host, double beta1, double beta2, double eps, int64_t step,
                                 void *stream_)
{
    return adam_step_at(n_rows, rows_host, beta1, beta2, eps, step, nullptr, static_cast<hipStream_t>(stream_));
}

extern "C" int soar_adam_step_at_gather(int32_t n_rows, const SoarAdamRow *rows_host, double beta1, double beta2, double eps, int64_t step,
                                        int32_t n_frames, int32_t num_frames_seq, int32_t floats_per_frame, int32_t n_sets,
                                        const int32_t *frame_ids_host, const float *table_dev, float *mats_out_dev,
                                        int32_t *set_index_out_dev, void *stream_)
{
    if (n_frames <= 0 || n_frames > MAX_BATCH || num_frames_seq <= 0 || floats_per_frame <= 0 || !frame_ids_host || !table_dev || !mats_out_dev) {
        set_error("soar_adam_step_at_gather: bad gather arguments (at most %d frames per step)", MAX_BATCH);
        return 1;
    }
    AdamGather ga = {};
    ga.n_frames = n_frames; ga.num_frames_seq = num_frames_seq; ga.floats_per_frame = floats_per_frame; ga.n_sets = n_sets;
    for (int f = 0; f < n_frames; f++) ga.id[f] = frame_ids_host[f];
    ga.table = table_dev; ga.mats_out = mats_out_dev; ga.set_out = set_index_out_dev;
    return adam_step_at(n_rows, rows_host, beta1, beta2, eps, step, &ga, static_cast<hipStream_t>(stream_));
}

static int adam_step_at(int32_t n_rows, const SoarAdamRow *rows_host, double beta1, double beta2, double eps, int64_t step,
                        const AdamGather *gather, hipStream_t stream)
{
    if (n_rows < 0 || n_rows > ADAM_MAX_ROWS || (n_rows && !rows_host) || step < 1) {
        set_error("soar_adam_step_at: 0 <= n_rows <= %d, rows must be given, step >= 1", ADAM_MAX_ROWS);
        return 1;
    }
    AdamTable tab;
    tab.n = n_rows;
    int64_t blocks = 0;
    for (int r = 0; r < n_rows; r++) {
        const SoarAdamRow &w = rows_host[r];
        if (w.count < 0 || (w.count && (!w.param || !w.grad || !w.exp_avg || !w.exp_avg_sq))) {
            set_error("soar_adam_step_at: row %d has a NULL pointer or a negative count", r);
            return 1;
        }
        tab.row[r] = w;
        tab.first_block[r] = blocks;
        blocks += (w.count + 1023) / 1024;
    }
    for (int r = n_rows; r <= ADAM_MAX_ROWS; r++) tab.first_block[r] = blocks;
    AdamState st;
    st.step = (int32_t)step;
    st.bias_correction1 = (float)(1.0 - pow(beta1, (double)step));
    st.bias_correction2_sqrt = (float)sqrt(1.0 - pow(beta2, (double)step));
    st.pad = 0;
    AdamGather ga = {};
    if (gather) { ga = *gather; ga.first_block = blocks; }
    StageTimer timer(ST_OPTIMIZER, stream);
    if (blocks + ga.n_frames > 0)
        hipLaunchKernelGGL(adam_update_kernel<AdamTable>, dim3((unsigned)(blocks + ga.n_frames)), dim3(256), 0, stream, tab, (const AdamState *)nullptr, st,
                           (float)beta2, (float)(1.0 - beta1), (float)(1.0 - beta2), (float)eps, ga);
    SOAR_LAUNCH_OK("adam_step_at", stream, 0);
    return 0;
}

extern "C" int soar_adam_step_rows(int32_t n_rows, const SoarAdamRow *rows_host, double beta1, double beta2, double eps, void *state_dev,
                                   int32_t advance, void *stream_)
{
    hipStream_t stream = static_cast<hipStream_t>(stream_);
    if (n_rows < 0 || n_rows > ADAM_MAX_ROWS || (n_rows && !rows_host) || !state_dev) {
        set_error("soar_adam_step: 0 <= n_rows <= %d, rows and the 16-byte device state must be given", ADAM_MAX_ROWS);
        return 1;
    }
    AdamTable tab;
    int64_t blocks = 0;
    if (!adam_fill(tab, n_rows, rows_host, ADAM_MAX_ROWS, blocks, "soar_adam_step")) return 1;
    AdamState *st = static_cast<AdamState *>(state_dev);
    StageTimer timer(ST_OPTIMIZER, stream);
    if (advance) hipLaunchKernelGGL(adam_tick_kernel, dim3(1), dim3(1), 0, stream, st, beta1, beta2);
    if (blocks > 0)
        hipLaunchKernelGGL(adam_update_kernel<AdamTable>, dim3((unsigned)blocks), dim3(256), 0, stream, tab, st, AdamState{}, (float)beta2,
                           (float)(1.0 - beta1), (float)(1.0 - beta2), (float)eps, AdamGather{});
    SOAR_LAUNCH_OK("adam_step", stream, 0);
    return 0;
}

extern "C" int soar_adam_step_rows_wide(int32_t n_rows, const SoarAdamRow *rows_host, double beta1, double beta2, double eps, void *state_dev,
                                        int32_t advance, void *stream_)
{
    hipStream_t stream = static_cast<hipStream_t>(stream_);
    if (n_rows < 0 || n_rows > ADAM_MAX_ROWS_WIDE || (n_rows && !rows_host) || !state_dev) {
        set_error("soar_adam_step_rows_wide: 0 <= n_rows <= %d, rows and the 16-byte device state must be given", ADAM_MAX_ROWS_WIDE);
        return 1;
    }
    AdamTableWide tab;
    int64_t blocks = 0;
    if (!adam_fill(tab, n_rows, rows_host, ADAM_MAX_ROWS_WIDE, blocks, "soar_adam_step_rows_wide")) return 1;
    AdamState *st = static_cast<AdamState *>(state_dev);
    StageTimer timer(ST_OPTIMIZER, stream);
    if (advance) hipLaunchKernelGGL(adam_tick_kernel, dim3(1), dim3(1), 0, stream, st, beta1, beta2);
    if (blocks > 0)
        hipLaunchKernelGGL(adam_update_kernel<AdamTableWide>, dim3((unsigned)blocks), dim3(256), 0, stream, tab, st, AdamState{}, (float)beta2,
                           (float)(1.0 - beta1), (float)(1.0 - beta2), (float)eps, AdamGather{});
    SOAR_LAUNCH_OK("adam_step_rows_wide", stream, 0);
    return 0;
}
```

### soar_amd/hip_lib.py

```python
from __future__ import annotations

import ctypes as C
import os
from typing import Optional

_HERE = os.path.dirname(os.path.abspath(__file__))
LIB_PATH = os.environ.get("SOAR_HIP_LIB") or os.path.join(_HERE, "_lib", "libsoar_hip.so")
if os.environ.get("SOAR_HIP_LIB"):
    import sys as _sys
    print(f"[soar_amd] SOAR_HIP_LIB is set: loading {LIB_PATH} instead of the in-tree build (development A/B runs only)", file=_sys.stderr)

FRAME_LOSS_SCRATCH_FLOATS = 4 * 2048
ABI_VERSION = 8
c_f32p = C.c_void_p
_vp = C.c_void_p


class SoarRastParams(C.Structure):
    _fields_ = [
        ("P", C.c_int32), ("W", C.c_int32), ("H", C.c_int32), ("sh_degree", C.c_int32), ("M", C.c_int32),
        ("prefiltered", C.c_int32), ("render_front", C.c_int32), ("sort_descending", C.c_int32), ("debug", C.c_int32),
        ("cfg_surface", C.c_int32), ("cfg_normalize_depth", C.c_int32), ("cfg_perpix_depth", C.c_int32),
        ("cfg_lrn_cam", C.c_int32),
        ("tanfovx", C.c_float), ("tanfovy", C.c_float), ("scale_modifier", C.c_float),
        ("bg_dev", _vp), ("viewmatrix_dev", _vp), ("projmatrix_dev", _vp), ("prcppoint_dev", _vp),
        ("patchbbox_dev", _vp), ("campos_dev", _vp),
    ]


class SoarDensifyRow(C.Structure):
    _fields_ = [("src", _vp), ("dst", _vp), ("width", C.c_int32), ("mode", C.c_int32)]


class SoarAdamRow(C.Structure):
    _fields_ = [("param", _vp), ("grad", _vp), ("exp_avg", _vp), ("exp_avg_sq", _vp), ("count", C.c_int64), ("lr", C.c_float),
                ("pad_", C.c_int32)]


class SoarPoseArgs(C.Structure):
    _fields_ = [("P", C.c_int32), ("J", C.c_int32), ("scale_width", C.c_int32), ("warp", C.c_int32),
                ("xyz", _vp), ("rot", _vp), ("weights", _vp), ("joint_mats", _vp), ("offsets", _vp), ("axis_perm", _vp),
                ("colors", _vp), ("scale_src", _vp), ("occ", _vp), ("occ3", _vp), ("posed", _vp),
                ("grad_scratch", _vp), ("dL_dxyz", _vp), ("dL_drot", _vp), ("dL_dcolors", _vp), ("dL_dscale", _vp), ("dL_docc", _vp)]


class SoarCameraSpec(C.Structure):
    _fields_ = [("fovx", C.c_double), ("fovy", C.c_double), ("znear", C.c_double), ("zfar", C.c_double), ("cx", C.c_double),
                ("cy", C.c_double), ("img_w", C.c_double), ("img_h", C.c_double), ("has_cxcy", C.c_int32), ("pad_", C.c_int32)]


class SoarFrameHead(C.Structure):
    _fields_ = [("prm", _vp), ("geom_buffer", _vp), ("radii", _vp)]


class SoarFrameTail(C.Structure):
    _fields_ = [("prm", _vp), ("means3D", _vp), ("rotations", _vp), ("radii", _vp), ("geom_buffer", _vp), ("workspace", _vp),
                ("dL_dmeans2D", _vp)]


class SoarLossFinish(C.Structure):
    _fields_ = [("sums4", _vp), ("loss_out", _vp), ("blocks", C.c_int32), ("n", C.c_int32), ("w_color", C.c_float), ("w_mask", C.c_float),
                ("w_normal", C.c_float), ("w_depth", C.c_float)]


class SoarViewArgs(C.Structure):
    _fields_ = [("rast", SoarRastParams), ("focal_k00", C.c_float), ("focal_k11", C.c_float), ("back", C.c_int32), ("pad_", C.c_int32),
                ("capacity", C.c_int64),
                ("buffer", _vp), ("buffer_bytes", C.c_size_t), ("out", _vp), ("radii", _vp), ("status_pinned", _vp),
                ("g_render", _vp), ("g_normal", _vp), ("g_depth", _vp), ("g_pred_normal", _vp), ("g_mask", _vp), ("g_occ", _vp),
                ("g_curv", _vp), ("dL_dmeans2D", _vp)]


class SoarAvatarLossArgs(C.Structure):
    _fields_ = [("H", C.c_int32), ("W", C.c_int32), ("cos_limit", C.c_float), ("cos_weight", C.c_float),
                ("render", _vp), ("gt_rgb", _vp), ("mask_img", _vp), ("gt_mask", _vp), ("normal", _vp), ("gt_normal", _vp), ("occ", _vp),
                ("sel", _vp), ("sel_normal", _vp), ("sel_occ", _vp), ("stats", _vp), ("stats_occ", _vp), ("scratch", _vp), ("counts", _vp),
                ("up_l1", _vp), ("up_l1m", _vp), ("up_cos", _vp), ("up_occ", _vp), ("up_ssim", _vp), ("g_ssim", _vp),
                ("g_render", _vp), ("g_mask", _vp), ("g_normal", _vp), ("g_occ", _vp),
                ("normal_raw", C.c_int32), ("occ_grad_summed", C.c_int32), ("cos_scale_out", _vp), ("background", _vp)]


class SoarFieldHead(C.Structure):
    _fields_ = [("w1", _vp), ("b1", _vp), ("w2", _vp), ("b2", _vp)]


FIELD_LEVELS = 16


class SoarFieldArgs(C.Structure):
    _fields_ = [("N", C.c_int32), ("log2_T", C.c_int32), ("normalized", C.c_int32), ("pad_", C.c_int32),
                ("res", C.c_float * FIELD_LEVELS), ("xyz", _vp), ("aabb", _vp), ("table", _vp), ("qtable", _vp), ("z", _vp),
                ("head", SoarFieldHead * 5), ("enc", _vp), ("qenc", _vp), ("out", _vp * 5), ("g_out", _vp * 5),
                ("d_table", _vp), ("d_qtable", _vp), ("d_head", _vp * 5), ("d_xyz", _vp), ("d_z", _vp)]


class SoarEnvmapArgs(C.Structure):
    _fields_ = [("B", C.c_int32), ("H", C.c_int32), ("W", C.c_int32), ("n_comp", C.c_int32), ("color_rows", C.c_int32),
                ("pad_", C.c_int32), ("render_stride", C.c_int64), ("mask_stride", C.c_int64), ("g_comp_stride", C.c_int64 * 4),
                ("dirs", _vp), ("w1", _vp), ("w2", _vp), ("w3", _vp), ("color", _vp), ("render", _vp), ("mask", _vp),
                ("bg", _vp), ("comp", _vp), ("g_comp", _vp), ("g_bg", _vp), ("g_mask", _vp), ("d_w1", _vp), ("d_w2", _vp), ("d_w3", _vp)]


LPIPS_LAYERS, LPIPS_TAPS = 13, 5


class SoarLpipsWeights(C.Structure):
    _fields_ = [("conv_w", _vp * LPIPS_LAYERS), ("conv_b", _vp * LPIPS_LAYERS), ("lin", _vp * LPIPS_TAPS), ("shift", _vp), ("scale", _vp)]


class SoarLpipsArgs(C.Structure):
    _fields_ = [("N", C.c_int32), ("H", C.c_int32), ("W", C.c_int32), ("grads", C.c_int32), ("in0", _vp), ("in1", _vp),
                ("in0_stride", C.c_int64 * 4), ("in1_stride", C.c_int64 * 4), ("weights", _vp), ("out", _vp), ("g_out", _vp),
                ("g_in0", _vp), ("g_in1", _vp), ("g_in0_stride", C.c_int64 * 4), ("g_in1_stride", C.c_int64 * 4)]


class SoarVaeArgs(C.Structure):
    _fields_ = [("N", C.c_int32), ("H", C.c_int32), ("W", C.c_int32), ("image_size", C.c_int32), ("x", _vp), ("x_stride", C.c_int64 * 4),
                ("weights", _vp), ("scale_factor", C.c_float), ("eps", _vp), ("mean", _vp), ("logvar", _vp), ("latents", _vp),
                ("g_latents", _vp), ("g_scale", _vp), ("grad_scale", _vp), ("grad_scale_stride", C.c_int64 * 3), ("g_x", _vp),
                ("g_x_stride", C.c_int64 * 4)]


SDS_PLAIN, SDS_RECON = 0, 1


class SoarSdsArgs(C.Structure):
    _fields_ = [("B", C.c_int32), ("n_view", C.c_int32), ("h", C.c_int32), ("w", C.c_int32), ("mode", C.c_int32), ("n_timesteps", C.c_int32),
                ("guidance_scale", C.c_float), ("recon_std_rescale", C.c_float), ("grad_clip", C.c_float), ("t", _vp), ("tables", _vp),
                ("latents", _vp), ("noise", _vp), ("eps_pred", _vp), ("x_in", _vp), ("loss", _vp), ("grad_norm", _vp), ("g_lat", _vp)]


DATA_CROP, DATA_MAX_VIEWS, DATA_SMALL_FLOATS = 512, 8, 256


class SoarDataStepArgs(C.Structure):
    _fields_ = [("B", C.c_int32), ("H", C.c_int32), ("W", C.c_int32), ("n_frames", C.c_int32), ("Hv", C.c_int32), ("Wv", C.c_int32),
                ("frame", C.c_int32), ("rays_d_normalize", C.c_int32), ("gt_has_cxcy", C.c_int32), ("n_small", C.c_int32),
                ("near_plane", C.c_double), ("far_plane", C.c_double), ("gt_near", C.c_double),
                ("c2w", (C.c_float * 16) * DATA_MAX_VIEWS), ("focal", C.c_float * DATA_MAX_VIEWS), ("tan_half", C.c_float * DATA_MAX_VIEWS),
                ("gt_c2w", C.c_float * 16), ("gt_tan_half", C.c_float), ("gt_cx", C.c_float), ("gt_cy", C.c_float),
                ("small", C.c_float * DATA_SMALL_FLOATS),
                ("images", _vp), ("masks", _vp), ("normal_F", _vp), ("normal_B", _vp), ("normal_mask", _vp),
                ("rgb_crop", _vp), ("mask_crop", _vp), ("normal_Ks", _vp),
                ("rays_d", _vp), ("cam_d", _vp), ("gt_rays_d", _vp), ("gt_cam_d", _vp),
                ("gt_rgb", _vp), ("gt_mask", _vp), ("gt_normal_F", _vp), ("gt_normal_B", _vp), ("gt_normal_mask", _vp),
                ("gt_rgb_crop", _vp), ("gt_mask_crop", _vp),
                ("mvp_mtx", _vp), ("proj", _vp), ("gt_mvp_mtx", _vp), ("small_out", _vp)]


class SoarEvalArgs(C.Structure):
    _fields_ = [("N", C.c_int32), ("H", C.c_int32), ("W", C.c_int32), ("pad_", C.c_int32), ("pred", _vp), ("gt_rgb", _vp), ("gt_mask", _vp),
                ("pred_stride", C.c_int64 * 4), ("gt_stride", C.c_int64 * 4), ("mask_stride", C.c_int64 * 3),
                ("gt_white", _vp), ("pred2", _vp), ("gt2", _vp), ("grid", _vp), ("metrics", _vp)]


class SoarPlaybackArgs(C.Structure):
    _fields_ = [("B", C.c_int32), ("H", C.c_int32), ("W", C.c_int32), ("normal_as_rgb", C.c_int32), ("render", _vp), ("normal", _vp),
                ("mask", _vp), ("occ", _vp), ("render_stride", C.c_int64), ("normal_stride", C.c_int64), ("mask_stride", C.c_int64),
                ("occ_stride", C.c_int64), ("rgb", _vp), ("normal_out", _vp), ("occ_out", _vp), ("mask_out", _vp)]


SIGNATURES = {
    "soar_last_error": (C.c_char_p, []),
    "soar_abi_version": (C.c_int, []),
    "soar_rast_geometry_bytes": (C.c_int, [C.c_int32, C.c_int32, C.POINTER(C.c_size_t)]),
    "soar_rast_image_bytes": (C.c_int, [C.c_int32, C.c_int32, C.POINTER(C.c_size_t)]),
    "soar_rast_binning_bytes": (C.c_int, [C.c_int64, C.POINTER(C.c_size_t)]),
    "soar_rast_backward_workspace_bytes": (C.c_int, [C.c_int32, C.POINTER(C.c_size_t)]),
    "soar_rast_forward_geometry": (C.c_int, [C.POINTER(SoarRastParams)] + [_vp] * 7 + [_vp, _vp, C.POINTER(C.c_int64), _vp]),
    "soar_rast_num_rendered": (C.c_int, [_vp, C.c_int32, C.c_int32, C.POINTER(C.c_int64), _vp]),
    "soar_rast_binning_status": (C.c_int, [_vp, C.c_int32, C.c_int32, C.POINTER(C.c_int64), C.POINTER(C.c_int64), _vp]),
    "soar_rast_binning_status_sticky": (C.c_int, [_vp, C.c_int32, C.c_int32, C.POINTER(C.c_int64), C.POINTER(C.c_int64), C.c_int32, _vp]),
    "soar_rast_binning_status_async": (C.c_int, [_vp, C.c_int32, C.c_int32, _vp, _vp]),
    "soar_rast_prefilter_violations": (C.c_int, [_vp, C.c_int32, C.c_int32, C.POINTER(C.c_int64), _vp]),
    "soar_rast_forward_render": (C.c_int, [C.POINTER(SoarRastParams), _vp, _vp, _vp, _vp, C.c_int64, _vp, _vp, _vp, _vp, _vp]),
    "soar_rast_forward_render_occ": (C.c_int, [C.POINTER(SoarRastParams), _vp, _vp, _vp, _vp, C.c_int64, _vp, _vp, _vp, _vp,
                                               _vp, _vp, _vp]),
    "soar_rast_backward": (C.c_int, [C.POINTER(SoarRastParams)] + [_vp] * 7 + [_vp, _vp, _vp, C.c_int64] + [_vp] * 4
                           + [_vp] * 11 + [_vp, C.c_size_t, _vp]),
    "soar_rast_backward_scaled": (C.c_int, [C.POINTER(SoarRastParams)] + [_vp] * 7 + [_vp, _vp, _vp, C.c_int64] + [_vp] * 5
                                  + [_vp] * 11 + [_vp, C.c_size_t, _vp]),
    "soar_rast_backward_occ": (C.c_int, [C.POINTER(SoarRastParams)] + [_vp] * 7 + [_vp, _vp, _vp, C.c_int64] + [_vp] * 6 + [C.c_int32]
                               + [_vp] * 12 + [_vp, C.c_size_t, _vp]),
    "soar_rast_backward_plan": (C.c_int, [C.POINTER(SoarRastParams), C.c_int32] + [_vp] * 7 + [_vp, _vp, _vp, C.c_int64] + [_vp] * 4
                                + [_vp] * 11 + [_vp, C.c_size_t, _vp]),
    "soar_rast_backward_occ_plan": (C.c_int, [C.POINTER(SoarRastParams), C.c_int32] + [_vp] * 7 + [_vp, _vp, _vp, C.c_int64] + [_vp] * 6
                                    + [C.c_int32] + [_vp] * 12 + [_vp, C.c_size_t, _vp]),
    "soar_rast_backward_region_counts": (C.c_int, [C.POINTER(C.c_int64), C.POINTER(C.c_int64)]),
    "soar_batch_begin": (C.c_int, [C.c_int32]),
    "soar_batch_frame": (C.c_int, [C.c_int32]),
    "soar_batch_end": (C.c_int, []),
    "soar_rast_occ_backward": (C.c_int, [C.POINTER(SoarRastParams), _vp, _vp, _vp, C.c_int64, _vp, _vp, _vp]),
    "soar_rast_mark_visible": (C.c_int, [C.c_int32, _vp, _vp, _vp, _vp, _vp]),
    "soar_rast_export_state": (C.c_int, [C.POINTER(SoarRastParams), _vp, _vp, _vp, C.c_int64] + [_vp] * 17 + [_vp]),
    "soar_lbs_knn_weights_bytes": (C.c_int, [C.c_int32, C.c_int32, C.POINTER(C.c_size_t)]),
    "soar_lbs_knn_weights": (C.c_int, [_vp, C.c_int32, _vp, C.c_int32, _vp, C.c_int32, C.c_int32, _vp, _vp, _vp, C.c_size_t, _vp]),
    "soar_lbs_knn_grid_bytes": (C.c_int, [C.c_int32, C.POINTER(C.c_size_t)]),
    "soar_lbs_knn_query_bytes": (C.c_int, [C.c_int32, C.POINTER(C.c_size_t)]),
    "soar_lbs_knn_build_grid": (C.c_int, [_vp, C.c_int32, _vp, C.c_int32, _vp, _vp]),
    "soar_lbs_knn_query": (C.c_int, [_vp, C.c_int32, _vp, C.c_int32, _vp, C.c_int32, C.c_int32, _vp, _vp, _vp, C.c_size_t, _vp]),
    "soar_lbs_knn_query_ordered": (C.c_int, [_vp, C.c_int32, _vp, C.c_int32, _vp, C.c_int32, C.c_int32, _vp, C.c_int32, _vp, _vp,
                                             _vp, C.c_size_t, _vp]),
    "soar_lbs_knn_state_bytes": (C.c_int, [C.c_int32, C.POINTER(C.c_size_t)]),
    "soar_lbs_knn_query_state": (C.c_int, [_vp, C.c_int32, _vp, C.c_int32, _vp, C.c_int32, _vp, C.c_int32, _vp, _vp, _vp, C.c_size_t, _vp]),
    "soar_lbs_knn_refresh": (C.c_int, [_vp, C.c_int32, C.c_int32, _vp, C.c_int32, _vp, _vp, _vp, _vp, _vp]),
    "soar_lbs_warp_forward": (C.c_int, [_vp] * 6 + [C.c_int32, C.c_int32] + [_vp] * 4),
    "soar_lbs_warp_backward": (C.c_int, [_vp] * 5 + [C.c_int32, C.c_int32] + [_vp] * 5),
    "soar_lbs_warp_forward_batch": (C.c_int, [_vp] * 4 + [C.c_int32] * 3 + [_vp] * 3),
    "soar_lbs_warp_backward_sum": (C.c_int, [_vp] * 4 + [C.c_int32] * 3 + [_vp] * 4 + [C.c_int32, _vp, _vp, _vp, _vp]),
    "soar_frames_warp_preprocess": (C.c_int, [C.c_int32, _vp] + [_vp] * 4 + [C.c_int32, C.c_int32] + [_vp] * 6),
    "soar_rast_backward_rows": (C.c_int, [_vp] * 22),
    "soar_frames_geometry_warp_backward": (C.c_int, [C.c_int32, _vp] + [_vp] * 4 + [C.c_int32, C.c_int32] + [_vp] * 7),
    "soar_frames_geometry_warp_backward_losses": (C.c_int, [C.c_int32, _vp] + [_vp] * 4 + [C.c_int32, C.c_int32] + [_vp] * 8),
    "soar_dist2_knn3": (C.c_int, [_vp, C.c_int32, _vp, _vp]),
    "soar_depth2normal": (C.c_int, [C.c_int32, C.c_int32, _vp, _vp, C.c_float, C.c_float, C.c_float, C.c_float, _vp, _vp]),
    "soar_depth2normal_backward": (C.c_int, [C.c_int32, C.c_int32, _vp, _vp, C.c_float, C.c_float, C.c_float, C.c_float, _vp, _vp,
                                             _vp]),
    "soar_normal2curv": (C.c_int, [C.c_int32, C.c_int32, _vp, _vp, _vp, _vp]),
    "soar_normal2curv_backward": (C.c_int, [C.c_int32, C.c_int32, _vp, _vp, _vp, _vp, _vp]),
    "soar_view_finish": (C.c_int, [C.c_int32, C.c_int32, _vp, _vp, _vp, _vp, C.c_float, C.c_float, _vp, _vp, _vp, _vp]),
    "soar_view_finish_backward": (C.c_int, [C.c_int32, C.c_int32, _vp, _vp, _vp, _vp, C.c_float, C.c_float, _vp, _vp, _vp, _vp,
                                            _vp, _vp]),
    "soar_ssim_scratch_floats": (C.c_int, [C.c_int32, C.c_int32, C.c_int32, C.POINTER(C.c_size_t)]),
    "soar_ssim": (C.c_int, [C.c_int32, C.c_int32, C.c_int32, _vp, _vp, _vp, _vp, _vp, _vp]),
    "soar_ssim_rendered": (C.c_int, [C.c_int32, C.c_int32, C.c_int32, _vp, _vp, _vp, _vp, _vp, _vp, _vp]),
    "soar_densify_stats": (C.c_int, [C.c_int32, _vp, _vp, C.c_int32, _vp, _vp, _vp, _vp, _vp, _vp]),
    "soar_densify_plan_bytes": (C.c_int, [C.c_int32, C.POINTER(C.c_size_t)]),
    "soar_densify_plan": (C.c_int, [C.c_int32, _vp, _vp, _vp, C.c_int32, C.c_int32, C.c_float, C.c_float, C.c_float, C.c_float,
                                    C.c_float, _vp, C.POINTER(C.c_int64), _vp]),
    "soar_densify_flags": (C.c_int, [C.c_int32, _vp, _vp, _vp]),
    "soar_densify_apply": (C.c_int, [C.c_int32, C.c_int32, _vp, C.c_int32, C.POINTER(SoarDensifyRow), _vp, _vp, _vp, C.c_int32, _vp]),
    "soar_smplx_joint_mats": (C.c_int, [C.c_int32, C.c_int32, C.c_int32, _vp, C.c_int32, _vp, _vp, _vp, _vp, _vp, _vp, _vp, _vp]),
    "soar_image_loss_scratch_floats": (C.c_int, [C.POINTER(C.c_size_t)]),
    "soar_masked_l1": (C.c_int, [C.c_int32, C.c_int32, C.c_int32, _vp, _vp, _vp, _vp, _vp, _vp]),
    "soar_masked_l1_backward": (C.c_int, [C.c_int32, C.c_int32, C.c_int32, _vp, _vp, _vp, _vp, _vp, _vp, _vp]),
    "soar_cos_loss": (C.c_int, [C.c_int32, C.c_int32, C.c_int32, _vp, _vp, _vp, C.c_float, C.c_float, _vp, _vp, _vp]),
    "soar_cos_loss_backward": (C.c_int, [C.c_int32, C.c_int32, C.c_int32, _vp, _vp, _vp, C.c_float, C.c_float, _vp, _vp, _vp, _vp]),
    "soar_frame_loss": (C.c_int, [C.c_int32, C.c_int32, _vp, _vp, _vp, _vp, _vp, _vp, _vp, C.c_float, C.c_float, C.c_float,
                                  C.c_float, _vp, _vp, _vp, _vp, _vp, _vp, _vp, _vp, C.c_int32, _vp]),
    "soar_frame_loss_pooled": (C.c_int, [C.c_int32, C.c_int32, _vp, _vp, _vp, _vp, _vp, C.c_int32, _vp, C.c_float, C.c_float, C.c_float,
                                         C.c_float, _vp, _vp, _vp, _vp, _vp, _vp, _vp, _vp, C.c_int32, _vp]),
    "soar_frame_loss_partials": (C.c_int, [C.c_int32, C.c_int32, _vp, _vp, _vp, _vp, _vp, _vp, _vp, C.c_float, C.c_float, C.c_float,
                                           C.c_float, _vp, _vp, _vp, _vp, _vp, _vp, _vp, _vp, C.c_int32, _vp, _vp]),
    "soar_frame_loss_pooled_partials": (C.c_int, [C.c_int32, C.c_int32, _vp, _vp, _vp, _vp, _vp, C.c_int32, _vp, C.c_float, C.c_float,
                                                  C.c_float, C.c_float, _vp, _vp, _vp, _vp, _vp, _vp, _vp, _vp, C.c_int32, _vp, _vp]),
    "soar_selftest_exp": (C.c_int, [_vp, C.c_int32, _vp, _vp, _vp]),
    "soar_selftest_affine_scan": (C.c_int, [_vp, _vp, _vp, _vp]),
    "soar_prof_enable": (C.c_int, [C.c_int]),
    "soar_prof_reset": (C.c_int, []),
    "soar_prof_stage_count": (C.c_int, []),
    "soar_prof_stage_name": (C.c_char_p, [C.c_int]),
    "soar_prof_read": (C.c_int, [C.c_int, C.POINTER(C.c_double), C.POINTER(C.c_int64)]),
    "soar_sum_frames": (C.c_int, [C.c_int32, C.c_int64, _vp, _vp, _vp]),
    "soar_gather_step_inputs": (C.c_int, [C.c_int32, C.c_int32, C.c_int32, C.c_int32, _vp, _vp, _vp, _vp, _vp]),
    "soar_gather_step_inputs_ids": (C.c_int, [C.c_int32, C.c_int32, C.c_int32, C.c_int32, C.POINTER(C.c_int32), _vp, _vp, _vp, _vp]),
    "soar_prof_timestamp": (C.c_int, [_vp, C.c_int64, C.c_int64, _vp]),
    "soar_view_buffer_bytes": (C.c_int, [C.c_int32, C.c_int32, C.c_int32, C.c_int64, C.c_int32, C.POINTER(C.c_size_t)]),
    "soar_views_grad_scratch_floats": (C.c_int, [C.c_int32, C.c_int32, C.POINTER(C.c_size_t)]),
    "soar_views_forward": (C.c_int, [C.POINTER(SoarPoseArgs), C.c_int32, C.POINTER(SoarViewArgs), _vp]),
    "soar_views_backward": (C.c_int, [C.POINTER(SoarPoseArgs), C.c_int32, C.POINTER(SoarViewArgs), _vp]),
    "soar_step_views_forward": (C.c_int, [C.c_int32, C.POINTER(SoarPoseArgs), C.POINTER(C.c_int32), C.POINTER(SoarViewArgs), _vp]),
    "soar_step_views_backward": (C.c_int, [C.c_int32, C.POINTER(SoarPoseArgs), C.POINTER(C.c_int32), C.POINTER(SoarViewArgs), _vp]),
    "soar_cameras_from_c2w": (C.c_int, [C.c_int32, _vp, C.POINTER(C.c_float), C.POINTER(SoarCameraSpec), _vp, _vp]),
    "soar_rast_forward_render_status": (C.c_int, [C.POINTER(SoarRastParams), _vp, _vp, _vp, _vp, C.c_int64, _vp, _vp, _vp, _vp,
                                                  _vp, _vp, _vp, _vp]),
    "soar_lbs_warp_backward_views": (C.c_int, [_vp] * 5 + [C.c_int32] * 3 + [_vp] * 4 + [C.c_int32, _vp, _vp, _vp, _vp]),
    "soar_avatar_loss_scratch_floats": (C.c_int, [C.POINTER(C.c_size_t)]),
    "soar_avatar_pixel_losses": (C.c_int, [C.POINTER(SoarAvatarLossArgs), C.c_int32, _vp]),
    "soar_adam_step": (C.c_int, [C.c_int32, C.POINTER(SoarAdamRow), C.c_double, C.c_double, C.c_double, _vp, _vp]),
    "soar_adam_step_at": (C.c_int, [C.c_int32, C.POINTER(SoarAdamRow), C.c_double, C.c_double, C.c_double, C.c_int64, _vp]),
    "soar_adam_step_at_gather": (C.c_int, [C.c_int32, C.POINTER(SoarAdamRow), C.c_double, C.c_double, C.c_double, C.c_int64] + [C.c_int32] * 4
                                 + [C.POINTER(C.c_int32), _vp, _vp, _vp, _vp]),
    "soar_adam_step_rows": (C.c_int, [C.c_int32, C.POINTER(SoarAdamRow), C.c_double, C.c_double, C.c_double, _vp, C.c_int32, _vp]),
    "soar_adam_step_rows_wide": (C.c_int, [C.c_int32, C.POINTER(SoarAdamRow), C.c_double, C.c_double, C.c_double, _vp, C.c_int32, _vp]),
    "soar_tsdf_integrate": (C.c_int, [C.c_int32] * 3 + [_vp] * 5 + [C.c_float] * 4 + [C.c_int32] * 3 + [C.c_float] * 3 + [_vp] * 3),
    "soar_mc_workspace_bytes": (C.c_int, [C.c_int32] * 3 + [C.POINTER(C.c_size_t)]),
    "soar_mc_count": (C.c_int, [C.c_int32] * 3 + [_vp, _vp, C.c_float, _vp, C.c_size_t, C.POINTER(C.c_int64), _vp]),
    "soar_mc_emit": (C.c_int, [C.c_int32] * 3 + [_vp, _vp, C.c_float, _vp, C.c_size_t, _vp, _vp, _vp]),
    "soar_mesh_filter_bytes": (C.c_int, [C.c_int32, C.c_int32, C.POINTER(C.c_size_t)]),
    "soar_mesh_filter_components": (C.c_int, [C.c_int32, C.c_int32, _vp, _vp, C.c_int32, C.c_float, _vp, C.c_size_t, _vp, _vp,
                                              C.POINTER(C.c_int64), _vp]),
    "soar_mesh_simplify_bytes": (C.c_int, [C.c_int32, C.c_int32, C.POINTER(C.c_size_t)]),
    "soar_mesh_simplify_count": (C.c_int, [C.c_int32, C.c_int32, _vp, _vp, C.c_float, _vp, C.c_size_t, C.POINTER(C.c_int64), _vp]),
    "soar_mesh_simplify": (C.c_int, [C.c_int32, C.c_int32, _vp, _vp, C.c_float, _vp, C.c_size_t, _vp, _vp, C.POINTER(C.c_int64), _vp]),
    "soar_mesh_attr_transfer_bytes": (C.c_int, [C.c_int32, C.c_int32, C.POINTER(C.c_size_t)]),
    "soar_mesh_attr_transfer": (C.c_int, [C.c_int32, C.c_int32, C.c_int32, _vp, _vp, _vp, _vp, _vp, C.c_size_t, _vp, _vp, _vp, _vp]),
    "soar_mesh_adjacency_bytes": (C.c_int, [C.c_int32, C.c_int32, C.POINTER(C.c_size_t)]),
    "soar_mesh_adjacency": (C.c_int, [C.c_int32, C.c_int32, _vp, _vp, C.c_size_t, _vp, _vp, _vp, _vp]),
# ... 87 lines not shown
```

### soar_amd/lbs.py

```python
from __future__ import annotations

from typing import Optional, Tuple

import torch

from . import hip_lib
from .hip_lib import check, ptr

KNN_K = 30


def _need_hip(t: torch.Tensor, name: str):
    if not t.is_cuda:
        raise RuntimeError(f"{name} is on '{t.device}': soar_amd runs on HIP devices only; there is no CPU fallback")


def _f32(t: torch.Tensor) -> torch.Tensor:
    return t.detach().float().contiguous()


def _stream(device):
    return torch.cuda.current_stream(device).cuda_stream


# ... 3 lines not shown
        _need_hip(verts, "verts")
        L = hip_lib.lib()
        self.verts = _f32(verts)
        self.V = int(self.verts.shape[0])
        self.weights = _f32(vert_weights.to(verts.device)).reshape(self.V, -1)
        self.J = int(self.weights.shape[1])
        import ctypes as C
        n = C.c_size_t(0)
        check(L.soar_lbs_knn_grid_bytes(self.V, C.byref(n)), "soar_lbs_knn_grid_bytes")
        self.buffer = torch.empty(int(n.value), dtype=torch.uint8, device=verts.device)
        with torch.cuda.device(verts.device):
            check(L.soar_lbs_knn_build_grid(ptr(self.verts), self.V, ptr(self.weights), self.J, ptr(self.buffer),
                                            _stream(verts.device)), "soar_lbs_knn_build_grid")

    RESORT_EVERY = 8

    def query_workspace(self, P: int) -> torch.Tensor:
        import ctypes as C
        n = C.c_size_t(0)
        check(hip_lib.lib().soar_lbs_knn_query_bytes(int(P), C.byref(n)), "soar_lbs_knn_query_bytes")
        return torch.empty(int(n.value), dtype=torch.uint8, device=self.verts.device)

    def query(self, xyz: torch.Tensor, K: int = 30, return_idx: bool = False, out: Optional[torch.Tensor] = None):
        _need_hip(xyz, "xyz")
        L = hip_lib.lib()
        x = _f32(xyz)
        P = int(x.shape[0])
        if out is None:
            out = torch.empty((P, self.J), dtype=torch.float32, device=x.device)
        idx = torch.empty((P, K), dtype=torch.int32, device=x.device) if return_idx else None
        order = getattr(self, "_order", None)
        resort = order is None or order.numel() != P or self._since_sort >= self.RESORT_EVERY
        if resort:
            if order is None or order.numel() != P:
                order = self._order = torch.empty((P,), dtype=torch.int32, device=x.device)
            self._since_sort = 0
        self._since_sort += 1
        stream = _stream(x.device)
        cache = self.__dict__.setdefault("_query_ws", {})
        ws = cache.get((P, stream))
        if ws is None:
            ws = cache[(P, stream)] = self.query_workspace(P)
        with torch.cuda.device(x.device):
            check(L.soar_lbs_knn_query_ordered(ptr(self.buffer), self.V, ptr(self.weights), self.J, ptr(x), P, K, ptr(order),
                                               int(resort), ptr(out), ptr(idx), ptr(ws), ws.numel(), stream),
                  "soar_lbs_knn_query_ordered")
        return (out, idx) if return_idx else out


class KnnFollower:

    RESORT_EVERY = 1024

    def __init__(self, grid: "KnnGrid", P: int):
        import ctypes as C
        self.grid, self.P = grid, int(P)
        dev = grid.verts.device
        n = C.c_size_t(0)
        check(hip_lib.lib().soar_lbs_knn_state_bytes(self.P, C.byref(n)), "soar_lbs_knn_state_bytes")
        self.state = torch.empty(int(n.value), dtype=torch.uint8, device=dev)
        self.order = torch.empty((self.P,), dtype=torch.int32, device=dev)
        self.ws = grid.query_workspace(self.P)
        self.searched = torch.zeros((1,), dtype=torch.int32, device=dev)
        self.calls = 0

    def full(self, xyz: torch.Tensor, out: torch.Tensor, stream: Optional[int] = None) -> torch.Tensor:
        g = self.grid
        stream = _stream(xyz.device) if stream is None else stream
        check(hip_lib.lib().soar_lbs_knn_query_state(ptr(g.buffer), g.V, ptr(g.weights), g.J, ptr(xyz), self.P, ptr(self.order), 1,
                                                     ptr(out), ptr(self.state), ptr(self.ws), self.ws.numel(), stream),
              "soar_lbs_knn_query_state")
        self.calls = 1
        return out

    def refresh(self, xyz: torch.Tensor, out: torch.Tensor, stream: Optional[int] = None) -> torch.Tensor:
        g = self.grid
        stream = _stream(xyz.device) if stream is None else stream
        if self.calls == 0 or self.calls % self.RESORT_EVERY == 0:
            return self.full(xyz, out, stream)
        check(hip_lib.lib().soar_lbs_knn_refresh(ptr(g.buffer), g.V, g.J, ptr(xyz), self.P, ptr(self.order), ptr(self.state), ptr(out),
                                                 ptr(self.searched), stream), "soar_lbs_knn_refresh")
        self.calls += 1
        return out

    def __call__(self, xyz: torch.Tensor, out: Optional[torch.Tensor] = None) -> torch.Tensor:
        _need_hip(xyz, "xyz")
        x = _f32(xyz)
        if int(x.shape[0]) != self.P:
            raise ValueError(f"KnnFollower was built for {self.P} queries, got {int(x.shape[0])}")
        if out is None:
            out = torch.empty((self.P, self.grid.J), dtype=torch.float32, device=x.device)
        with torch.cuda.device(x.device):
            return self.refresh(x, out)


def knn_blend_weights(xyz: torch.Tensor, verts: torch.Tensor, vert_weights: torch.Tensor, K: int = KNN_K,
                      return_idx: bool = False):
    _need_hip(xyz, "xyz")
    L = hip_lib.lib()
    x, v, w = _f32(xyz), _f32(verts.to(xyz.device)), _f32(vert_weights.to(xyz.device))
    P, V, J = x.shape[0], v.shape[0], w.shape[-1]
    w = w.reshape(V, J)
    out = torch.empty((P, J), dtype=torch.float32, device=x.device)
    idx = torch.empty((P, K), dtype=torch.int32, device=x.device) if return_idx else None
    import ctypes as C
    n = C.c_size_t(0)
    check(L.soar_lbs_knn_weights_bytes(P, V, C.byref(n)), "soar_lbs_knn_weights_bytes")
    ws = torch.empty(int(n.value), dtype=torch.uint8, device=x.device)
    with torch.cuda.device(x.device):
        check(L.soar_lbs_knn_weights(ptr(x), P, ptr(v), V, ptr(w), J, K, ptr(out), ptr(idx), ptr(ws), ws.numel(),
                                     _stream(x.device)), "soar_lbs_knn_weights")
    return (out, idx) if return_idx else out


class _LbsWarp(torch.autograd.Function):
    @staticmethod
    def forward(ctx, xyz, rot, weights, joint_mats, offsets, axis_perm):
        _need_hip(xyz, "xyz")
        L = hip_lib.lib()
        dev = xyz.device
        x, q, A = _f32(xyz), _f32(rot), _f32(joint_mats).reshape(-1, 16)
        off = _f32(offsets) if offsets is not None else None
        T = _f32(axis_perm.to(dev)) if axis_perm is not None else None
        P = x.shape[0]
        if weights is None:
            w, J = None, 0
            if A.shape[0] != P:
                raise ValueError(f"per-point matrices must be [{P},4,4], got {tuple(joint_mats.shape)}")
        else:
            w, J = _f32(weights), A.shape[0]
            if w.shape != (P, J):
                raise ValueError(f"weights must be [{P},{J}], got {tuple(w.shape)}")
        xyz_out = torch.empty_like(x)
        rot_out = torch.empty_like(q)
        with torch.cuda.device(dev):
            check(L.soar_lbs_warp_forward(ptr(x), ptr(q), ptr(w), ptr(A), ptr(off), ptr(T), P, J, ptr(xyz_out),
                                          ptr(rot_out), None, _stream(dev)), "soar_lbs_warp_forward")
        ctx.J = J
        ctx.save_for_backward(x, q, w if w is not None else torch.empty(0, device=dev), A,
                              T if T is not None else torch.empty(0, device=dev))
        ctx.has_offsets = offsets is not None and offsets.requires_grad
        return xyz_out, rot_out

    @staticmethod
    def backward(ctx, g_xyz_out, g_rot_out):
        L = hip_lib.lib()
        x, q, w, A, T = ctx.saved_tensors
        dev = x.device
        P, J = x.shape[0], ctx.J
        gx = _f32(g_xyz_out) if g_xyz_out is not None else torch.zeros_like(x)
        gq = _f32(g_rot_out) if g_rot_out is not None else torch.zeros_like(q)
        g_xyz = torch.empty_like(x)
        g_rot = torch.empty_like(q)
        with torch.cuda.device(dev):
            check(L.soar_lbs_warp_backward(ptr(x), ptr(q), ptr(w), ptr(A), ptr(T), P, J, ptr(gx), ptr(gq), ptr(g_xyz),
                                           ptr(g_rot), _stream(dev)), "soar_lbs_warp_backward")
        g_off = None
        if ctx.has_offsets:
            g_off = gx if T.numel() == 0 else gx @ T.t()
        return g_xyz, g_rot, None, None, g_off, None


def lbs_warp(xyz: torch.Tensor, rot: torch.Tensor, weights: torch.Tensor, joint_mats: torch.Tensor,
             offsets: Optional[torch.Tensor] = None, axis_perm: Optional[torch.Tensor] = None
             ) -> Tuple[torch.Tensor, torch.Tensor]:
    return _LbsWarp.apply(xyz, rot, weights, joint_mats, offsets, axis_perm)
# ... 28 lines not shown
```

### soar_amd/optim.py

```python
from __future__ import annotations

import ctypes as C
from typing import Dict, Optional

import torch

from . import hip_lib
from .hip_lib import check, ptr

REFERENCE_LR = {"xyz": 1.6e-5, "rot": 1e-3, "scales": 5e-3, "colors": 1e-2, "opacity": 1e-2, "occ": 0.1}


class FusedAdam:
    def __init__(self, flat, lr: Optional[Dict[str, float]] = None, betas=(0.9, 0.999), eps: float = 1e-15):
        self.flat = flat
        self.lr = dict(REFERENCE_LR if lr is None else lr)
        self.betas, self.eps = (float(betas[0]), float(betas[1])), float(eps)
        self.names = [n for n in flat.leaves if n in self.lr]
        dev = flat.flat.device
        self.exp_avg = {n: torch.zeros_like(flat.leaves[n]) for n in self.names}
        self.exp_avg_sq = {n: torch.zeros_like(flat.leaves[n]) for n in self.names}
        self.state = torch.zeros((4,), dtype=torch.int32, device=dev)
        self.device_counter, self.steps = False, 0
        self._rows = None

    def _table(self, names=None):
        names = self.names if names is None else names
        rows = (hip_lib.SoarAdamRow * len(names))()
        for k, n in enumerate(names):
            p = self.flat.leaves[n]
            if not p.is_contiguous():
                raise ValueError(f"leaf {n} must be contiguous")
            rows[k].param, rows[k].grad = ptr(p), ptr(self.flat.views[n])
            rows[k].exp_avg, rows[k].exp_avg_sq = ptr(self.exp_avg[n]), ptr(self.exp_avg_sq[n])
            rows[k].count, rows[k].lr = p.numel(), self.lr[n]
        return rows

    def step(self, stream: Optional[int] = None, names=None, advance: bool = True, gather=None) -> None:
        self.flat.check_views()
        dev = self.flat.flat.device
        names = self.names if names is None else [n for n in self.names if n in names]
        rows = self._table(names)
        with torch.cuda.device(dev):
            stream = torch.cuda.current_stream(dev).cuda_stream if stream is None else stream
            if self.device_counter:
                if gather is not None:
                    raise ValueError("gather rides with the host step counter only (device_counter = False)")
                check(hip_lib.lib().soar_adam_step_rows(len(names), rows, self.betas[0], self.betas[1], self.eps, ptr(self.state),
                                                        1 if advance else 0, stream), "soar_adam_step_rows")
            else:
                if advance:
                    self.steps += 1
                if gather is not None:
                    check(hip_lib.lib().soar_adam_step_at_gather(len(names), rows, self.betas[0], self.betas[1], self.eps, self.steps,
                                                                 *gather, stream), "soar_adam_step_at_gather")
                    return
                check(hip_lib.lib().soar_adam_step_at(len(names), rows, self.betas[0], self.betas[1], self.eps, self.steps, stream),
                      "soar_adam_step_at")
```

### soar_amd/step_plan.py

```python
from __future__ import annotations

import ctypes as C
import os
from typing import Dict, List, Optional, Sequence

import torch

from . import hip_lib
from .hip_lib import check, ptr
from .rasterizer import _Ctx


class FrameStepPlan:
    def __init__(self, seq, n_frames: int, targets: Dict[str, torch.Tensor], bg: torch.Tensor, capacity: int, flat,
                 loss_weights: Sequence[float] = (1.0, 1.0, 0.1, 0.01), use_graphs: bool = True, batched: Optional[bool] = None,
                 loss: str = "synthetic", lambdas: Optional[Dict[str, float]] = None):
        if loss not in ("synthetic", "avatar"):
            raise ValueError(f"loss must be 'synthetic' or 'avatar', got {loss!r}")
        self.loss_kind = loss
        if loss == "avatar" and (use_graphs or not torch.is_tensor(targets)):
            raise ValueError("loss='avatar' needs a resident target pool and use_graphs=False")
        L = hip_lib.lib()
        self.L, self.seq, self.flat, self.n = L, seq, flat, int(n_frames)
        dev = seq.device
# ... 10 lines not shown
            self.pool = targets
            self.targets = None
        else:
            self.targets = [targets[k].to(**f).contiguous() for k in ("color", "mask", "normal")]
        self.frame_sel = torch.zeros((self.n,), dtype=torch.int32, device=dev)
        self.frame_ids = torch.zeros((self.n,), dtype=torch.int32, device=dev)
        self._ids_pinned = torch.zeros((64, self.n), dtype=torch.int32).pin_memory()
        self._ids_copied = [None] * 64
        self.mats = torch.empty((self.n, 55, 4, 4), **f)
        self.blend_weights = torch.empty((P, seq.lbs_weights.shape[1]), **f)
        self.ones = torch.ones((P, 1), **f)
        self.ctx = _Ctx(P, 0, H, W, seq.camera.tanfovx, seq.camera.tanfovy, 1.0, 0, False, False, False, False, self.bg,
                        seq.view, seq.proj, seq.prcp, seq.patch, seq.campos, seq.config, dev)
        nbytes = C.c_size_t(0)
        check(L.soar_rast_geometry_bytes(P, 0, C.byref(nbytes)), "geometry_bytes"); geom_b = nbytes.value
        check(L.soar_rast_image_bytes(W, H, C.byref(nbytes)), "image_bytes"); img_b = nbytes.value
        check(L.soar_rast_binning_bytes(self.capacity, C.byref(nbytes)), "binning_bytes"); bin_b = nbytes.value
        check(L.soar_rast_backward_workspace_bytes(P, C.byref(nbytes)), "workspace_bytes"); work_b = nbytes.value
        u8 = dict(dtype=torch.uint8, device=dev)
        self.xyz_p_all, self.rot_p_all = torch.empty((self.n, P, 3), **f), torch.empty((self.n, P, 4), **f)
        self.g_means3D_all, self.g_rot_p_all = torch.empty((self.n, P, 3), **f), torch.empty((self.n, P, 4), **f)
        self.views: List[dict] = []
        for i in range(self.n):
            v = dict(
                xyz_p=self.xyz_p_all[i], rot_p=self.rot_p_all[i], radii=torch.empty((P,), dtype=torch.int32, device=dev),
                color=torch.empty((3, H, W), **f), normal=torch.empty((3, H, W), **f), depth=torch.empty((1, H, W), **f),
                opac=torch.empty((1, H, W), **f), occ=torch.empty((3, H, W), **f),
                geom=torch.empty(geom_b, **u8), img=torch.empty(img_b, **u8), binning=torch.empty(bin_b, **u8),
                work=torch.empty(work_b, **u8), loss=torch.empty((), **f), sums=torch.empty((hip_lib.FRAME_LOSS_SCRATCH_FLOATS,), **f),
                gC=torch.empty((3, H, W), **f), gN=torch.empty((3, H, W), **f), gD=torch.empty((1, H, W), **f),
                gO=torch.empty((1, H, W), **f),
                g_means2D=torch.empty((P, 3), **f), g_colors=torch.empty((P, 3), **f), g_opacity=torch.empty((P, 1), **f),
                g_means3D=self.g_means3D_all[i], g_cov3D=torch.empty((P, 6), **f), g_scales=torch.empty((P, 3), **f),
                g_rot_p=self.g_rot_p_all[i], g_view=torch.empty((4, 4), **f), g_proj=torch.empty((4, 4), **f),
                g_campos=torch.empty((3,), **f))
            v["geom"][:256].zero_()
            self.views.append(v)
        self.fused_tail = os.environ.get("SOAR_PLAN_FUSED_TAIL", "1") != "0" and self.n <= 8
        if self.fused_tail:
            self.ctx.params.debug |= 8
            self._tail_frames = (hip_lib.SoarFrameTail * self.n)()
            for i, v in enumerate(self.views):
                t = self._tail_frames[i]
                t.prm = C.addressof(self.ctx.params)
                t.means3D, t.rotations, t.radii = v["xyz_p"].data_ptr(), v["rot_p"].data_ptr(), v["radii"].data_ptr()
                t.geom_buffer, t.workspace, t.dL_dmeans2D = v["geom"].data_ptr(), v["work"].data_ptr(), v["g_means2D"].data_ptr()
        env = os.environ.get("SOAR_PLAN_BWD_REGION")
        self.bwd_region = int(env) if env in ("1", "2") else (2 if W * H >= (1 << 20) else 1)
        self.fused_head = os.environ.get("SOAR_PLAN_FUSED_HEAD", "1") != "0" and self.n <= 8
        if self.fused_head:
            self.ctx.params.debug |= 16
            self._head_frames = (hip_lib.SoarFrameHead * self.n)()
            for i, v in enumerate(self.views):
                h = self._head_frames[i]
                h.prm, h.geom_buffer, h.radii = C.addressof(self.ctx.params), v["geom"].data_ptr(), v["radii"].data_ptr()
        self.g_xyz = torch.empty((self.n, P, 3), **f)
        self.g_rot = torch.empty((self.n, P, 4), **f)
        self.g_scales = torch.empty((self.n, P, 3), **f)
        self.g_colors = torch.empty((self.n, P, 3), **f)
        self.losses = torch.empty((self.n,), **f)
        from . import lbs as _lbs
        self.knn = _lbs.KnnFollower(seq.knn_grid, P)
        for name in ("opacity", "occ"):
            if name in flat.views:
                flat.views[name].zero_()
        if loss == "avatar":
            self._setup_avatar(lambdas)
        self.steps = 0
        self.STAMP_CAP = 8192
        self.stamps = torch.zeros((1 + 2 * self.STAMP_CAP,), dtype=torch.int64, device=dev) if os.environ.get("SOAR_PLAN_TIMESTAMPS") in ("1", "2") else None
        self.fine_stamps = os.environ.get("SOAR_PLAN_TIMESTAMPS") == "2"
        self.stale = None
        self._baked = self._leaf_signature()
        self.streams = [torch.cuda.Stream(device=dev) for _ in range(self.n)]
        if batched is None:
            env = os.environ.get("SOAR_PLAN_BATCHED")
            batched = (env != "0") if env in ("0", "1") else (self.W * self.H <= 3_000_000)
        self.batched = bool(batched) and self.n <= 8
        fold = self.batched and not use_graphs
        self.loss_in_tail = fold and self.fused_tail and loss == "synthetic" and os.environ.get("SOAR_PLAN_LOSS_IN_TAIL", "1") != "0"
        if self.loss_in_tail:
            self._loss_finish = (hip_lib.SoarLossFinish * self.n)()
        self.gather_in_adam = fold and self.n <= 8 and os.environ.get("SOAR_PLAN_GATHER_IN_ADAM", "1") != "0"
        self._call_cache = {}
        self.optimizer = None
        self.optimizer_in_two_parts = None
        self.graphs = None
        self._ids_by_value = not use_graphs and self.n <= 8
        if use_graphs:
            if os.environ.get("DEBUG_CLR_GRAPH_PACKET_CAPTURE") != "0":
                raise RuntimeError("FrameStepPlan(use_graphs=True) needs DEBUG_CLR_GRAPH_PACKET_CAPTURE=0 in the environment "
                                   "before the HIP runtime starts (see the module docstring); use use_graphs=False otherwise")
            self._capture()

    def _setup_avatar(self, lambdas):
        from .losses import _AvatarStageLoss as S
        L, dev, H, W, P = self.L, self.device, self.H, self.W, self.P
        f = dict(dtype=torch.float32, device=dev)
        lam = dict(recon=1.0, mask=1.0, normal=1.0, occ=0.1)
        lam.update(lambdas or {})
        self.lam = lam
        pool = self.pool
        n_sets = int(pool.shape[0])
        m = pool[:, 3:4]
        self.av = dict(rgb=pool[:, 0:3], mask=m, normal=pool[:, 4:7],
                       sel=(m > 1e-5).reshape(n_sets, H, W).contiguous().view(torch.uint8),
                       sel_occ=(m > 0).reshape(n_sets, H, W).contiguous().view(torch.uint8),
                       blended=(pool[:, 0:3] * m + self.bg.reshape(1, 3, 1, 1) * (1 - m)).contiguous())
        k = C.c_size_t(0)
        check(L.soar_image_loss_scratch_floats(C.byref(k)), "soar_image_loss_scratch_floats")
        n_loss = int(k.value)
        check(L.soar_ssim_scratch_floats(3, H, W, C.byref(k)), "soar_ssim_scratch_floats")
        n_ssim = int(k.value)
        coef = [0.0] * S.N
        coef[S.L1], coef[S.SSIM], coef[S.ONE] = 0.8 * lam["recon"], -0.2 * lam["recon"], 0.2 * lam["recon"]
        coef[S.L1M], coef[S.COS] = lam["mask"], 0.2 * lam["normal"]
        self.av_coef = torch.tensor(coef, **f)
        self.av_occ_up = torch.tensor([lam["occ"]], **f)
        self.av_counts = torch.stack([self.av["sel"].reshape(n_sets, -1).sum(1).float(), torch.full((n_sets,), float(H * W), **f),
                                      torch.zeros((n_sets,), **f), self.av["sel_occ"].reshape(n_sets, -1).sum(1).float()], dim=1).contiguous()
        self.av_cos_scale_all = torch.zeros((self.n,), **f)
        check(L.soar_avatar_loss_scratch_floats(C.byref(k)), "soar_avatar_loss_scratch_floats")
        n_pix = int(k.value)
        self._av_args = {}
        self.av_focal = (H / (2.0 * self.seq.camera.tanfovy), W / (2.0 * self.seq.camera.tanfovx))
        self.g_occ_all = torch.empty((self.n, P), **f)
        self.av_gC_all, self.av_g_ssim_all = torch.empty((self.n, 3, H, W), **f), torch.empty((self.n, 3, H, W), **f)
        self.av_terms_all, self.av_occ_terms_all = torch.zeros((self.n, S.N), **f), torch.zeros((self.n, 2), **f)
        self.av_terms_all[:, S.ONE] = 1.0
        for i, v in enumerate(self.views):
            g_nd = torch.zeros((4, H, W), **f)
            v.update(normal_out=torch.empty((3, H, W), **f), curv=torch.empty((1, H, W), **f), pred=torch.empty((3, H, W), **f),
                     gC=self.av_gC_all[i], g_ssim=self.av_g_ssim_all[i], g_nd=g_nd,
                     g_occ_img=torch.empty((3, H, W), **f), terms=self.av_terms_all[i], occ_terms=self.av_occ_terms_all[i],
                     av_scratch=torch.empty((max(n_loss, n_ssim),), **f), av_pix_scratch=torch.empty((n_pix,), **f))
            v["gN"], v["gD"] = g_nd[:3], g_nd[3:]

    def _av(self, i: int):
        from .losses import _AvatarStageLoss as S
        v = self.views[i]
        k = self._frames_now[i] % int(self.pool.shape[0])
        at = lambda t, j: t.data_ptr() + 4 * j
        return S, self.L, v, self.W, self.H, self.av, k, at, ptr(v["av_scratch"]), v["terms"], self.av_coef

    def _av_finish(self, i, stream):
        S, L, v, W, H, a, k, at, sc, t, up = self._av(i)
        check(L.soar_view_finish(W, H, ptr(v["normal"]), ptr(v["depth"]), ptr(v["opac"]), ptr(self.ctx.keep[3]), self.av_focal[0],
                                 self.av_focal[1], ptr(v["normal_out"]), ptr(v["curv"]), ptr(v["pred"]), stream), "soar_view_finish")

    def _av_ssim(self, i, stream):
        S, L, v, W, H, a, k, at, sc, t, up = self._av(i)
        check(L.soar_ssim_rendered(3, H, W, ptr(v["color"]), ptr(a["blended"][k]), at(t, S.SSIM), sc, ptr(v["g_ssim"]), ptr(v["opac"]), stream),
              "soar_ssim_rendered")

    def _av_pixel_args(self, i):
        S, L, v, W, H, a, k, at, sc, t, up = self._av(i)
        return hip_lib.SoarAvatarLossArgs(
            H=H, W=W, cos_limit=1.0, cos_weight=1.0, render=ptr(v["color"]), gt_rgb=ptr(a["rgb"][k]), mask_img=ptr(v["opac"]),
            gt_mask=ptr(a["mask"][k]), normal=ptr(v["normal_out"]), gt_normal=ptr(a["normal"][k]), occ=ptr(v["occ"]),
            sel=ptr(a["sel"][k]), sel_normal=ptr(a["sel"][k]), sel_occ=ptr(a["sel_occ"][k]), stats=at(t, S.L1), stats_occ=ptr(v["occ_terms"]),
            scratch=ptr(v["av_pix_scratch"]), counts=ptr(self.av_counts[k]), up_l1=at(up, S.L1), up_l1m=at(up, S.L1M), up_cos=at(up, S.COS),
            up_occ=ptr(self.av_occ_up), up_ssim=at(up, S.SSIM), g_ssim=ptr(v["g_ssim"]), g_render=ptr(v["gC"]), g_mask=ptr(v["gO"]),
            g_normal=ptr(v["gN"]), g_occ=ptr(v["g_occ_img"]), normal_raw=1, occ_grad_summed=1, cos_scale_out=self.av_cos_scale_all.data_ptr() + 4 * i,
            background=self.ctx.params.bg_dev)

    def _av_pixel(self, i, stream):
        key = ("av_pixel", i, self._frames_now[i] % int(self.pool.shape[0]))
        args = self._av_args.get(key)
        if args is None:
            args = self._av_args[key] = self._av_pixel_args(i)
        check(self.L.soar_avatar_pixel_losses(C.byref(args), 3, stream), "soar_avatar_pixel_losses")

    def _f_avatar_loss(self, i: int, frame: int, stream: int) -> None:
        v, up = self.views[i], self.av_coef
        for stage in (self._av_finish, self._av_ssim, self._av_pixel):
            stage(i, stream)
        torch.add(torch.dot(v["terms"], up), v["occ_terms"][0] * self.av_occ_up[0], out=self.losses[i])

    def _leaf_signature(self):
        s = self.seq
        return tuple((t.data_ptr(), tuple(t.shape)) for t in (s.xyz, s.rot, s.scales, s.colors, s.occ))

    def invalidate(self, reason: str):
        self.stale = reason

    def _check_fresh(self):
        if self.stale is None and self._leaf_signature() != self._baked:
            self.stale = "the sequence's parameter tensors changed (pointer or shape) since the plan was built"
        if self.stale is not None:
            raise RuntimeError(f"FrameStepPlan is stale: {self.stale}; build a new plan (buffers and HIP graphs hold the old "
                               "pointers)")

    RESORT_EVERY = 1024

    def _stamp(self, k: int, stream: int) -> None:
        if self.stamps is not None:
            check(self.L.soar_prof_timestamp(self.stamps.data_ptr(), self.STAMP_CAP, k, stream), "timestamp")

    def _stage_stamp(self, i: int, stage: int, stream: int) -> None:
        if self.stamps is not None and self.fine_stamps:
            self._stamp(100 + 10 * i + stage, stream)

    def _gather_args(self):
        s = self.seq
        n_sets = int(self.pool.shape[0]) if self.pool is not None else 0
        return (self.n, s.num_frames, 55 * 16, n_sets, (C.c_int32 * self.n)(*self._frames_now), ptr(s.cano2live), ptr(self.mats), ptr(self.frame_sel))

    def _prologue(self, stream: int, resort: bool = True, gathered: bool = False) -> None:
        L, s = self.L, self.seq
        self._stamp(0, stream)
        n_sets = int(self.pool.shape[0]) if self.pool is not None else 0
        if gathered:
            pass
        elif self._ids_by_value:
            ids = (C.c_int32 * self.n)(*self._frames_now)
            check(L.soar_gather_step_inputs_ids(self.n, s.num_frames, 55 * 16, n_sets, ids, ptr(s.cano2live), ptr(self.mats),
                                                ptr(self.frame_sel), stream), "gather_step_inputs")
        else:
            check(L.soar_gather_step_inputs(self.n, s.num_frames, 55 * 16, n_sets, ptr(self.frame_ids), ptr(s.cano2live), ptr(self.mats),
                                            ptr(self.frame_sel), stream), "gather_step_inputs")
        if resort:
            self.knn.full(s.xyz.detach(), self.blend_weights, stream)
        else:
            self.knn.calls = 1
            self.knn.refresh(s.xyz.detach(), self.blend_weights, stream)
        self._stamp(1, stream)

    def _warp_all(self, stream: int) -> None:
        L, s = self.L, self.seq
        J = int(self.blend_weights.shape[1])
        if self.fused_head:
            check(L.soar_frames_warp_preprocess(self.n, self._head_frames, ptr(s.xyz.detach()), ptr(s.rot.detach()), ptr(self.blend_weights),
                                                ptr(self.mats), self.P, J, ptr(s.colors.detach()), ptr(self.ones), ptr(s.scales.detach()),
                                                ptr(self.xyz_p_all), ptr(self.rot_p_all), stream), "frames_warp_preprocess")
            return
        check(L.soar_lbs_warp_forward_batch(ptr(s.xyz.detach()), ptr(s.rot.detach()), ptr(self.blend_weights), ptr(self.mats), self.n,
                                            self.P, J, ptr(self.xyz_p_all), ptr(self.rot_p_all), stream), "warp_forward_batch")

    def _call(self, key, build) -> None:
        c = self._call_cache.get(key)
        if c is None:
            c = self._call_cache[key] = build()
        if c[0](*c[1]) != 0:
            check(1, c[2])

    def _f_geometry(self, i: int, stream: int) -> None:
        def build():
            L, s, v = self.L, self.seq, self.views[i]
            return (L.soar_rast_forward_geometry, (C.byref(self.ctx.params), ptr(v["xyz_p"]), None, ptr(s.colors.detach()), ptr(self.ones),
                                                   ptr(s.scales.detach()), ptr(v["rot_p"]), None, ptr(v["geom"]), ptr(v["radii"]), None, stream),
                    "geometry")
        self._call(("geometry", i, stream), build)

    def _f_render(self, i: int, stream: int) -> None:
        def build():
            L, s, v = self.L, self.seq, self.views[i]
            return (L.soar_rast_forward_render_occ, (C.byref(self.ctx.params), ptr(v["radii"]), ptr(v["geom"]), ptr(v["binning"]), ptr(v["img"]),
                                                     self.capacity, ptr(v["color"]), ptr(v["normal"]), ptr(v["depth"]), ptr(v["opac"]),
                                                     ptr(s.occ), ptr(v["occ"]), stream), "render")
        self._call(("render", i, stream), build)

    def _f_loss(self, i: int, stream: int) -> None:
        def build():
            L, v, W, H = self.L, self.views[i], self.W, self.H
            wc, wm, wn, wd = self.weights
            if self.loss_in_tail:
                fin = C.addressof(self._loss_finish[i])
                if self.pool is not None:
                    return (L.soar_frame_loss_pooled_partials, (W, H, ptr(v["color"]), ptr(v["normal"]), ptr(v["depth"]), ptr(v["opac"]), ptr(self.pool),
                                                                int(self.pool.shape[0]), ptr(self.frame_sel[i]), wc, wm, wn, wd, ptr(self.losses[i]),
                                                                ptr(v["sums"]), ptr(v["gC"]), ptr(v["gN"]), ptr(v["gD"]), ptr(v["gO"]), ptr(v["img"]),
                                                                self.ctx.params.bg_dev, int(self.ctx.params.cfg_normalize_depth), fin, stream),
                            "frame_loss_pooled_partials")
                tc, tm, tn = self.targets
                return (L.soar_frame_loss_partials, (W, H, ptr(v["color"]), ptr(v["normal"]), ptr(v["depth"]), ptr(v["opac"]), ptr(tc), ptr(tm), ptr(tn),
                                                     wc, wm, wn, wd, ptr(self.losses[i]), ptr(v["sums"]), ptr(v["gC"]), ptr(v["gN"]), ptr(v["gD"]),
                                                     ptr(v["gO"]), ptr(v["img"]), self.ctx.params.bg_dev, int(self.ctx.params.cfg_normalize_depth),
                                                     fin, stream), "frame_loss_partials")
            if self.pool is not None:
                return (L.soar_frame_loss_pooled, (W, H, ptr(v["color"]), ptr(v["normal"]), ptr(v["depth"]), ptr(v["opac"]), ptr(self.pool),
                                                   int(self.pool.shape[0]), ptr(self.frame_sel[i]), wc, wm, wn, wd, ptr(self.losses[i]),
                                                   ptr(v["sums"]), ptr(v["gC"]), ptr(v["gN"]), ptr(v["gD"]), ptr(v["gO"]), ptr(v["img"]),
                                                   self.ctx.params.bg_dev, int(self.ctx.params.cfg_normalize_depth), stream),
                        "frame_loss_pooled")
            tc, tm, tn = self.targets
            return (L.soar_frame_loss, (W, H, ptr(v["color"]), ptr(v["normal"]), ptr(v["depth"]), ptr(v["opac"]), ptr(tc), ptr(tm), ptr(tn),
                                        wc, wm, wn, wd, ptr(self.losses[i]), ptr(v["sums"]), ptr(v["gC"]), ptr(v["gN"]), ptr(v["gD"]),
                                        ptr(v["gO"]), ptr(v["img"]), self.ctx.params.bg_dev, int(self.ctx.params.cfg_normalize_depth), stream),
                    "frame_loss")
        self._call(("loss", i, stream), build)

    def _f_backward(self, i: int, stream: int) -> None:
        def build():
            L, s, v = self.L, self.seq, self.views[i]
            return (L.soar_rast_backward_plan, (C.byref(self.ctx.params), self.bwd_region, ptr(v["xyz_p"]), ptr(v["radii"]), None,
                                                ptr(s.colors.detach()), ptr(s.scales.detach()), ptr(v["rot_p"]), None, ptr(v["geom"]),
                                                ptr(v["binning"]), ptr(v["img"]), self.capacity, ptr(v["gC"]), ptr(v["gN"]), ptr(v["gD"]),
                                                ptr(v["gO"]), ptr(v["g_means2D"]), ptr(self.g_colors[i]), ptr(v["g_opacity"]),
                                                ptr(v["g_means3D"]), ptr(v["g_cov3D"]), None, ptr(self.g_scales[i]), ptr(v["g_rot_p"]),
                                                ptr(v["g_view"]), ptr(v["g_proj"]), ptr(v["g_campos"]), ptr(v["work"]), v["work"].numel(),
                                                stream), "backward")
        self._call(("backward", i, stream), build)

    def _f_backward_occ(self, i: int, stream: int) -> None:
        def build():
            L, s, v = self.L, self.seq, self.views[i]
            return (L.soar_rast_backward_occ_plan, (C.byref(self.ctx.params), self.bwd_region, ptr(v["xyz_p"]), ptr(v["radii"]), None, ptr(s.colors.detach()),
                                               ptr(s.scales.detach()), ptr(v["rot_p"]), None, ptr(v["geom"]), ptr(v["binning"]), ptr(v["img"]),
                                               self.capacity, ptr(v["gC"]), ptr(v["gN"]), ptr(v["gD"]), ptr(v["gO"]), ptr(v["g_occ_img"]),
                                               self.av_cos_scale_all.data_ptr() + 4 * i, 1, ptr(v["g_means2D"]), ptr(self.g_colors[i]), ptr(v["g_opacity"]), ptr(v["g_means3D"]),
                                               ptr(v["g_cov3D"]), None, ptr(self.g_scales[i]), ptr(v["g_rot_p"]), ptr(v["g_view"]),
                                               ptr(v["g_proj"]), ptr(v["g_campos"]), ptr(self.g_occ_all[i]), ptr(v["work"]), v["work"].numel(),
                                               stream), "backward_occ")
        self._call(("backward_occ", i, stream), build)

    def _frame(self, i: int, stream: int) -> None:
        self._stamp(2 + 2 * i, stream)
        if self.loss_kind == "avatar":
            self._f_geometry(i, stream)
            self._f_render(i, stream)
            self._f_avatar_loss(i, self._frames_now[i], stream)
            self._f_backward_occ(i, stream)
            self._stamp(3 + 2 * i, stream)
            return
        for k, stage in enumerate((self._f_geometry, self._f_render, self._f_loss, self._f_backward)):
            self._stage_stamp(i, k, stream)
            stage(i, stream)
        self._stage_stamp(i, 4, stream)
        self._stamp(3 + 2 * i, stream)

    def _frames_batched(self, stream: int, frames: Optional[Sequence[int]] = None) -> None:
        L = self.L
        frames = list(range(self.n)) if frames is None else list(frames)
        for i in frames:
            self._stamp(2 + 2 * i, stream)
        def batch(stages):
            check(L.soar_batch_begin(len(frames)), "batch_begin")
            try:
                for stage in stages:
                    for k, i in enumerate(frames):
                        check(L.soar_batch_frame(k), "batch_frame")
                        stage(i, stream)
            finally:
                L.soar_batch_end()
        if self.loss_kind == "avatar":
            from .losses import _AvatarStageLoss as S
            batch((self._f_geometry, self._f_render, self._av_finish, self._av_ssim, self._av_pixel, self._f_backward_occ))
            if len(frames) == self.n:
                torch.addmv(self.av_occ_terms_all[:, 0] * self.av_occ_up[0], self.av_terms_all, self.av_coef, out=self.losses)
            else:
                for i in frames:
                    v = self.views[i]
                    torch.add(torch.dot(v["terms"], self.av_coef), v["occ_terms"][0] * self.av_occ_up[0], out=self.losses[i])
        else:
            batch((self._f_geometry, self._f_render, self._f_loss, self._f_backward))
        for i in frames:
            self._stamp(3 + 2 * i, stream)

    def _epilogue(self, stream: int) -> None:
        L, s = self.L, self.seq
        self._stamp(2 * self.n + 2, stream)
        J = int(self.blend_weights.shape[1])
        fv = self.flat.views
        src = (C.c_void_p * 2)(ptr(self.g_scales), ptr(self.g_colors))
        dst = (C.c_void_p * 2)(ptr(fv["scales"]), ptr(fv["colors"]))
        width = (C.c_int32 * 2)(3, 3)
        if self.fused_tail:
            occ = ptr(fv["occ"]) if (self.loss_kind == "avatar" and "occ" in fv) else None
            if self.loss_in_tail:
                check(L.soar_frames_geometry_warp_backward_losses(self.n, self._tail_frames, ptr(s.xyz.detach()), ptr(s.rot.detach()),
                                                                  ptr(self.blend_weights), ptr(self.mats), self.P, J, ptr(s.scales.detach()),
                                                                  ptr(fv["xyz"]), ptr(fv["rot"]), ptr(fv["scales"]), ptr(fv["colors"]), occ,
                                                                  self._loss_finish, stream), "frames_geometry_warp_backward_losses")
            else:
                check(L.soar_frames_geometry_warp_backward(self.n, self._tail_frames, ptr(s.xyz.detach()), ptr(s.rot.detach()), ptr(self.blend_weights),
                                                           ptr(self.mats), self.P, J, ptr(s.scales.detach()), ptr(fv["xyz"]), ptr(fv["rot"]),
                                                           ptr(fv["scales"]), ptr(fv["colors"]), occ, stream), "frames_geometry_warp_backward")
            self._stamp(2 * self.n + 3, stream)
            return
        check(L.soar_lbs_warp_backward_sum(ptr(s.xyz.detach()), ptr(s.rot.detach()), ptr(self.blend_weights), ptr(self.mats), self.n,
                                           self.P, J, ptr(self.g_means3D_all), ptr(self.g_rot_p_all), ptr(fv["xyz"]), ptr(fv["rot"]),
                                           2, src, dst, width, stream), "warp_backward_sum")
        if self.loss_kind == "avatar" and "occ" in fv:
            check(L.soar_sum_frames(self.n, self.P, ptr(self.g_occ_all), ptr(fv["occ"]), stream), "sum_frames")
        self._stamp(2 * self.n + 3, stream)

    def _capture(self) -> None:
        dev = self.device
        self.frame_ids.copy_(torch.arange(self.n, dtype=torch.int32) % max(self.seq.num_frames, 1))
        self._run_eager()
        torch.cuda.synchronize(dev)
        cap = torch.cuda.Stream(device=dev)
        graphs = {}
        with torch.cuda.device(dev):
            for name, resort in (("prologue_resort", True), ("prologue", False)):
                g = torch.cuda.CUDAGraph()
                with torch.cuda.graph(g, stream=cap):
                    self._prologue(cap.cuda_stream, resort)
                graphs[name] = g
                g = torch.cuda.CUDAGraph()
                with torch.cuda.graph(g, stream=cap):
                    self._prologue(cap.cuda_stream, resort)
                    self._warp_all(cap.cuda_stream)
                graphs[name + "+warp"] = g
            for i in range(self.n):
                g = torch.cuda.CUDAGraph()
                with torch.cuda.graph(g, stream=cap):
                    self._frame(i, cap.cuda_stream)
                graphs[i] = g
            for name, fn in (("warp", self._warp_all), ("epilogue", self._epilogue)):
                g = torch.cuda.CUDAGraph()
                with torch.cuda.graph(g, stream=cap):
                    fn(cap.cuda_stream)
                graphs[name] = g
        torch.cuda.synchronize(dev)
        self.graphs = graphs

    def _run_eager(self) -> None:
        dev = self.device
        main = torch.cuda.current_stream(dev)
        with torch.cuda.device(dev):
            opt = self.optimizer if (self.optimizer is not None and self.steps > 0) else None
            in_flight = any(p is not None for p in self.flat.pending) if self.optimizer_in_two_parts is None else self.optimizer_in_two_parts
            in_flight = in_flight and self.flat.n_buckets > 1
            self.flat.wait_bucket(0)
            ride = opt is not None and self.gather_in_adam and self._ids_by_value and not opt.device_counter
            if opt is not None:
                opt.step(main.cuda_stream, names=("xyz",) if in_flight else None, advance=True, gather=self._gather_args() if ride else None)
            self._prologue(main.cuda_stream, self.steps % self.RESORT_EVERY == 0, gathered=ride)
            self.flat.wait_all()
            if opt is not None and in_flight:
                opt.step(main.cuda_stream, names=tuple(n for n in opt.names if n != "xyz"), advance=False)
            self._warp_all(main.cuda_stream)
            if self.batched:
                self._frames_batched(main.cuda_stream)
            else:
                self._fan_out(main, lambda i, s: self._frame(i, s.cuda_stream))
            self._epilogue(main.cuda_stream)
        self.steps += 1
        self.ctx.params.debug |= 4

    def _fan_out(self, main, fn) -> None:
        ev = torch.cuda.Event()
        ev.record(main)
        done = []
        for i, s in enumerate(self.streams):
            s.wait_event(ev)
            with torch.cuda.stream(s):
                fn(i, s)
            e = torch.cuda.Event()
            e.record(s)
            done.append(e)
        for e in done:
            main.wait_event(e)

    def run(self, frames: Sequence[int]):
        if len(frames) != self.n:
            raise ValueError(f"the plan was built for {self.n} frames per step, got {len(frames)}")
        self._check_fresh()
        dev = self.device
        self._frames_now = [int(f) % self.seq.num_frames for f in frames]
        if self._ids_by_value:
            self._run_eager()
            return self.losses
        k_slot = self.steps % self._ids_pinned.shape[0]
        slot = self._ids_pinned[k_slot]
        if self._ids_copied[k_slot] is not None:
            self._ids_copied[k_slot].synchronize()
        for k, f in enumerate(frames):
            slot[k] = int(f) % self.seq.num_frames
        self.frame_ids.copy_(slot, non_blocking=True)
        ev = self._ids_copied[k_slot] or torch.cuda.Event()
        ev.record(torch.cuda.current_stream(dev))
        self._ids_copied[k_slot] = ev
        if self.graphs is None:
            self._run_eager()
            return self.losses
        main = torch.cuda.current_stream(dev)
        self.flat.wait_bucket(0)
        name = "prologue_resort" if self.steps % self.RESORT_EVERY == 0 else "prologue"
        if any(p is not None for p in self.flat.pending):
            self.graphs[name].replay()
            self.flat.wait_all()
            self.graphs["warp"].replay()
        else:
            self.graphs[name + "+warp"].replay()
        self._fan_out(main, lambda i, s: self.graphs[i].replay())
        self.graphs["epilogue"].replay()
        self.steps += 1
        return self.losses

    def check(self, reset: bool = True):
        out = []
        for v in self.views:
            n, o = C.c_int64(0), C.c_int64(0)
            with torch.cuda.device(self.device):
                check(self.L.soar_rast_binning_status_sticky(ptr(v["geom"]), self.P, 0, C.byref(n), C.byref(o), 1 if reset else 0,
                                                             torch.cuda.current_stream(self.device).cuda_stream), "binning_status_sticky")
            out.append((int(n.value), int(o.value)))
        bad = [o for _, o in out if o]
        if bad:
            raise RuntimeError(f"binning capacity exceeded in a step since the last check: {max(bad)} (tile, Gaussian) instances needed; "
                               "raise `capacity`")
        return out
```

Baseline: 5512.

## Fold Adam step and backward zeroing into the KNN refresh launch

Adds a KNN refresh entry point that carries riders: the fused Adam update (with optional per-frame gather) and the zeroing of backward accumulator ranges. These now run inside the KNN certify/blend kernel instead of as separate launches. The backward then skips its own zero-range launch when the rows are already cleared. This removes several small kernel launches and a pass over parameter memory per step. The cost is tighter coupling and ordering constraints: Adam must update xyz before the KNN reads it, and the folding applies only to non-resort, non-collective, batched steps.

After: 5461. No clear change (-0.9%).

```diff
diff --git a/include/soar_hip.h b/include/soar_hip.h
--- a/include/soar_hip.h
+++ b/include/soar_hip.h
@@ -144,6 +144,33 @@
                                 float *dL_dviewmat, float *dL_dprojmat, float *dL_dcampos, float *dL_docc,
                                 void *workspace, size_t workspace_bytes,
                                 void *stream);
+int soar_rast_backward_plan_cleared(const SoarRastParams *prm, int32_t region, int32_t rows_cleared,
+                                    const float *means3D, const int32_t *radii, const float *shs,
+                                    const float *colors_precomp, const float *scales, const float *rotations,
+                                    const float *cov3D_precomp,
+                                    const void *geom_buffer, const void *binning_buffer, const void *image_buffer,
+                                    int64_t num_rendered,
+                                    const float *dL_dout_color, const float *dL_dout_normal,
+                                    const float *dL_dout_depth, const float *dL_dout_opac,
+                                    float *dL_dmeans2D, float *dL_dcolors, float *dL_dopacity, float *dL_dmeans3D,
+                                    float *dL_dcov3D, float *dL_dsh, float *dL_dscales, float *dL_drotations,
+                                    float *dL_dviewmat, float *dL_dprojmat, float *dL_dcampos,
+                                    void *workspace, size_t workspace_bytes,
+                                    void *stream);
+int soar_rast_backward_occ_plan_cleared(const SoarRastParams *prm, int32_t region, int32_t rows_cleared,
+                                        const float *means3D, const int32_t *radii, const float *shs,
+                                        const float *colors_precomp, const float *scales, const float *rotations,
+                                        const float *cov3D_precomp,
+                                        const void *geom_buffer, const void *binning_buffer, const void *image_buffer,
+                                        int64_t num_rendered,
+                                        const float *dL_dout_color, const float *dL_dout_normal,
+                                        const float *dL_dout_depth, const float *dL_dout_opac, const float *dL_dout_occ,
+                                        const float *normal_scale_dev, int32_t occ_planes,
+                                        float *dL_dmeans2D, float *dL_dcolors, float *dL_dopacity, float *dL_dmeans3D,
+                                        float *dL_dcov3D, float *dL_dsh, float *dL_dscales, float *dL_drotations,
+                                        float *dL_dviewmat, float *dL_dprojmat, float *dL_dcampos, float *dL_docc,
+                                        void *workspace, size_t workspace_bytes,
+                                        void *stream);
 int soar_rast_backward_region_counts(int64_t *single_blocks, int64_t *pairs);
 int soar_rast_backward_workspace_bytes(int32_t P, size_t *bytes);
 
@@ -424,6 +451,29 @@
 int soar_adam_step_rows_wide(int32_t n_rows, const SoarAdamRow *rows, double beta1, double beta2, double eps, void *state_dev,
                              int32_t advance, void *stream);
 
+typedef struct SoarZeroRange {
+    void *ptr;
+    size_t bytes;
+} SoarZeroRange;
+typedef struct SoarKnnStepRiders {
+    int32_t n_rows, xyz_row;
+    const SoarAdamRow *rows;
+    double beta1, beta2, eps;
+    int64_t step;
+    int32_t n_frames, num_frames_seq, floats_per_frame, n_sets;
+    const int32_t *frame_ids;
+    const float *table;
+    float *mats_out;
+    int32_t *set_index_out;
+    int32_t n_zero, in_certify;
+    const SoarZeroRange *zero;
+} SoarKnnStepRiders;
+int soar_lbs_knn_refresh_step(const void *grid_buffer, int32_t V, int32_t J, float *xyz, int32_t P, const uint32_t *order,
+                              void *state_buffer, float *weights_out, uint32_t *searched_counter_dev, const SoarKnnStepRiders *riders,
+                              void *stream);
+int soar_rast_backward_zero_ranges(const SoarRastParams *prm, void *workspace, float *dL_dviewmat, float *dL_dprojmat, float *dL_dcampos,
+                                   SoarZeroRange *out, int32_t *count);
+
 int soar_prof_timestamp(unsigned long long *ring_dev, int64_t capacity, int64_t tag, void *stream);
 
 int soar_selftest_affine_scan(const float *m64_dev, const float *b64_dev, float *out192_dev, void *stream);
diff --git a/soar_amd/csrc/adam_update.h b/soar_amd/csrc/adam_update.h
--- /dev/null
+++ b/soar_amd/csrc/adam_update.h
@@ -0,0 +1,104 @@
+#pragma once
+
+#include "soar_common.h"
+
+#include <cstdint>
+
+namespace soar {
+
+constexpr int ADAM_MAX_ROWS = 8;
+template <int N>
+struct AdamTableT {
+    SoarAdamRow row[N];
+    int64_t first_block[N + 1];
+    int n;
+};
+using AdamTable = AdamTableT<ADAM_MAX_ROWS>;
+struct AdamState {
+    int32_t step;
+    float bias_correction1, bias_correction2_sqrt;
+    int32_t pad;
+};
+struct AdamCoef { float beta2, one_minus_b1, one_minus_b2, eps; };
+
+struct AdamGather {
+    int n_frames, num_frames_seq, floats_per_frame, n_sets;
+    int64_t first_block;
+    int32_t id[MAX_BATCH];
+    const float *table;
+    float *mats_out;
+    int32_t *set_out;
+};
+
+__device__ __forceinline__ void adam_update_element(float g, float &p, float &m, float &v, float step_size, float bc2s, const AdamCoef &c)
+{
+#pragma clang fp contract(off)
+    m = m + (g - m) * c.one_minus_b1;
+    v = c.beta2 * v + c.one_minus_b2 * (g * g);
+    const float denom = sqrtf(v) / bc2s + c.eps;
+    p = p - step_size * (m / denom);
+}
+
+__device__ __forceinline__ void adam_gather_workgroup(const AdamGather &ga, int f)
+{
+    int id = ga.id[f] % ga.num_frames_seq;
+    if (id < 0) id += ga.num_frames_seq;
+    for (int k = threadIdx.x; k < ga.floats_per_frame; k += 256)
+        ga.mats_out[(size_t)f * ga.floats_per_frame + k] = ga.table[(size_t)id * ga.floats_per_frame + k];
+    if (threadIdx.x == 0 && ga.set_out) ga.set_out[f] = ga.n_sets > 0 ? id % ga.n_sets : 0;
+}
+
+template <typename Table>
+__device__ __forceinline__ void adam_rows_workgroup(const Table &tab, const AdamState *st, const AdamCoef &c, int64_t blk)
+{
+    if (st->step <= 0) return;
+    int r = 0;
+    while (r + 1 < tab.n && blk >= tab.first_block[r + 1]) r++;
+    const SoarAdamRow row = tab.row[r];
+    const int64_t i0 = (blk - tab.first_block[r]) * 1024 + threadIdx.x * 4;
+    const float step_size = row.lr / st->bias_correction1, bc2s = st->bias_correction2_sqrt;
+    const bool vec = i0 + 3 < row.count && (((uintptr_t)row.param | (uintptr_t)row.grad | (uintptr_t)row.exp_avg | (uintptr_t)row.exp_avg_sq) & 15u) == 0u;
+    if (vec) {
+        const float4 g = *reinterpret_cast<const float4 *>(row.grad + i0);
+        float4 p = *reinterpret_cast<const float4 *>(row.param + i0), m = *reinterpret_cast<const float4 *>(row.exp_avg + i0),
+               v = *reinterpret_cast<const float4 *>(row.exp_avg_sq + i0);
+        adam_update_element(g.x, p.x, m.x, v.x, step_size, bc2s, c); adam_update_element(g.y, p.y, m.y, v.y, step_size, bc2s, c);
+        adam_update_element(g.z, p.z, m.z, v.z, step_size, bc2s, c); adam_update_element(g.w, p.w, m.w, v.w, step_size, bc2s, c);
+        *reinterpret_cast<float4 *>(row.param + i0) = p;
+        *reinterpret_cast<float4 *>(row.exp_avg + i0) = m;
+        *reinterpret_cast<float4 *>(row.exp_avg_sq + i0) = v;
+        return;
+    }
+    for (int k = 0; k < 4; k++) {
+        const int64_t i = i0 + k;
+        if (i >= row.count) break;
+        float p = row.param[i], m = row.exp_avg[i], v = row.exp_avg_sq[i];
+        adam_update_element(row.grad[i], p, m, v, step_size, bc2s, c);
+        row.param[i] = p;
+        row.exp_avg[i] = m;
+        row.exp_avg_sq[i] = v;
+    }
+}
+
+template <typename Table>
+inline bool adam_fill(Table &tab, int32_t n_rows, const SoarAdamRow *rows_host, int max_rows, int64_t &blocks, const char *who)
+{
+    tab.n = n_rows;
+    blocks = 0;
+    for (int r = 0; r < n_rows; r++) {
+        const SoarAdamRow &w = rows_host[r];
+        if (w.count < 0 || (w.count && (!w.param || !w.grad || !w.exp_avg || !w.exp_avg_sq))) {
+            set_error("%s: row %d has a NULL pointer or a negative count", who, r);
+            return false;
+        }
+        tab.row[r] = w;
+        tab.first_block[r] = blocks;
+        blocks += (w.count + 1023) / 1024;
+    }
+    for (int r = n_rows; r <= max_rows; r++) tab.first_block[r] = blocks;
+    return true;
+}
+
+AdamState adam_state_at(double beta1, double beta2, int64_t step);
+
+}
diff --git a/soar_amd/csrc/api.hip b/soar_amd/csrc/api.hip
--- a/soar_amd/csrc/api.hip
+++ b/soar_amd/csrc/api.hip
@@ -637,6 +637,17 @@
 
 }
 
+static void backward_zero_ranges(const SoarRastParams &prm, void *workspace, float *dL_dviewmat, float *dL_dprojmat, float *dL_dcampos,
+                                 ZeroRange zr[4])
+{
+    const bool wide = (prm.debug & 2) != 0;
+    void *acc64 = static_cast<char *>(workspace) + align_up(sizeof(float) * ACC_STRIDE * (size_t)prm.P);
+    zr[0] = {wide ? acc64 : workspace, (wide ? sizeof(double) : sizeof(float)) * ACC_STRIDE * (size_t)prm.P};
+    zr[1] = {dL_dviewmat, 16 * sizeof(float)};
+    zr[2] = {dL_dprojmat, 16 * sizeof(float)};
+    zr[3] = {dL_dcampos, 3 * sizeof(float)};
+}
+
 static int backward_impl(const SoarRastParams *prm, const float *means3D, const int32_t *radii, const float *shs,
                               const float *colors_precomp, const float *scales, const float *rotations,
                               const float *cov3D_precomp, const void *geom_buffer, const void *binning_buffer,
@@ -646,7 +657,7 @@
                               float *dL_dmeans3D, float *dL_dcov3D, float *dL_dsh, float *dL_dscales, float *dL_drotations,
                               float *dL_dviewmat, float *dL_dprojmat, float *dL_dcampos, void *workspace,
                               size_t workspace_bytes, const float *dL_dout_occ, float *dL_docc, const float *normal_scale_dev, int occ_planes,
-                              int region, void *stream_)
+                              int region, void *stream_, bool rows_cleared = false)
 {
     hipStream_t stream = static_cast<hipStream_t>(stream_);
     if (check_params(prm)) return 1;
@@ -687,9 +698,9 @@
     const bool wide = (prm->debug & 2) != 0;
     double *acc64 = wide ? reinterpret_cast<double *>(static_cast<char *>(workspace) + align_up(sizeof(float) * ACC_STRIDE * (size_t)prm->P))
                          : nullptr;
-    {
-        const ZeroRange zr[4] = {{wide ? (void *)acc64 : (void *)acc, (wide ? sizeof(double) : sizeof(float)) * ACC_STRIDE * (size_t)prm->P},
-                                 {dL_dviewmat, 16 * sizeof(float)}, {dL_dprojmat, 16 * sizeof(float)}, {dL_dcampos, 3 * sizeof(float)}};
+    if (!rows_cleared) {
+        ZeroRange zr[4];
+        backward_zero_ranges(*prm, workspace, dL_dviewmat, dL_dprojmat, dL_dcampos, zr);
         if (launch_zero_ranges(zr, 4, stream)) return 1;
     }
     if (num_rendered > 0 || wide) {
@@ -776,6 +787,58 @@
                          num_rendered, dL_dout_color, dL_dout_normal, dL_dout_depth, dL_dout_opac, nullptr, dL_dmeans2D, dL_dcolors,
                          dL_dopacity, dL_dmeans3D, dL_dcov3D, dL_dsh, dL_dscales, dL_drotations, dL_dviewmat, dL_dprojmat, dL_dcampos, workspace,
                          workspace_bytes, dL_dout_occ, dL_docc, normal_scale_dev, occ_planes, region, stream_);
+}
+
+int soar_rast_backward_zero_ranges(const SoarRastParams *prm, void *workspace, float *dL_dviewmat, float *dL_dprojmat, float *dL_dcampos,
+                                   SoarZeroRange *out, int32_t *count)
+{
+    if (check_params(prm)) return 1;
+    if (!out || !count) { set_error("soar_rast_backward_zero_ranges: out / count is NULL"); return 1; }
+    *count = 0;
+    if (prm->P == 0) return 0;
+    if (!workspace || !dL_dviewmat || !dL_dprojmat || !dL_dcampos) { set_error("soar_rast_backward_zero_ranges: a required pointer is NULL"); return 1; }
+    if (check_aligned(workspace, "workspace")) return 1;
+    ZeroRange zr[4];
+    backward_zero_ranges(*prm, workspace, dL_dviewmat, dL_dprojmat, dL_dcampos, zr);
+    for (int r = 0; r < 4; r++) { out[r].ptr = zr[r].ptr; out[r].bytes = zr[r].bytes; }
+    *count = 4;
+    return 0;
+}
+
+int soar_rast_backward_plan_cleared(const SoarRastParams *prm, int32_t region, int32_t rows_cleared, const float *means3D, const int32_t *radii,
+                                    const float *shs, const float *colors_precomp, const float *scales, const float *rotations,
+                                    const float *cov3D_precomp, const void *geom_buffer, const void *binning_buffer,
+                                    const void *image_buffer, int64_t num_rendered, const float *dL_dout_color,
+                                    const float *dL_dout_normal, const float *dL_dout_depth, const float *dL_dout_opac,
+                                    float *dL_dmeans2D, float *dL_dcolors, float *dL_dopacity, float *dL_dmeans3D, float *dL_dcov3D,
+                                    float *dL_dsh, float *dL_dscales, float *dL_drotations, float *dL_dviewmat, float *dL_dprojmat,
+                                    float *dL_dcampos, void *workspace, size_t workspace_bytes, void *stream_)
+{
+    if (region != 1 && region != 2) { set_error("soar_rast_backward_plan_cleared: region is 1 or 2, got %d", region); return 1; }
+    return backward_impl(prm, means3D, radii, shs, colors_precomp, scales, rotations, cov3D_precomp, geom_buffer, binning_buffer, image_buffer,
+                         num_rendered, dL_dout_color, dL_dout_normal, dL_dout_depth, dL_dout_opac, nullptr, dL_dmeans2D, dL_dcolors,
+                         dL_dopacity, dL_dmeans3D, dL_dcov3D, dL_dsh, dL_dscales, dL_drotations, dL_dviewmat, dL_dprojmat, dL_dcampos, workspace,
+                         workspace_bytes, nullptr, nullptr, nullptr, 3, region, stream_, rows_cleared != 0);
+}
+
+int soar_rast_backward_occ_plan_cleared(const SoarRastParams *prm, int32_t region, int32_t rows_cleared, const float *means3D,
+                                        const int32_t *radii, const float *shs, const float *colors_precomp, const float *scales,
+                                        const float *rotations, const float *cov3D_precomp, const void *geom_buffer,
+                                        const void *binning_buffer, const void *image_buffer, int64_t num_rendered,
+                                        const float *dL_dout_color, const float *dL_dout_normal, const float *dL_dout_depth,
+                                        const float *dL_dout_opac, const float *dL_dout_occ, const float *normal_scale_dev,
+                                        int32_t occ_planes, float *dL_dmeans2D, float *dL_dcolors, float *dL_dopacity, float *dL_dmeans3D,
+                                        float *dL_dcov3D, float *dL_dsh, float *dL_dscales, float *dL_drotations, float *dL_dviewmat,
+                                        float *dL_dprojmat, float *dL_dcampos, float *dL_docc, void *workspace, size_t workspace_bytes,
+                                        void *stream_)
+{
+    if (region != 1 && region != 2) { set_error("soar_rast_backward_occ_plan_cleared: region is 1 or 2, got %d", region); return 1; }
+    if (!dL_dout_occ || !dL_docc) { set_error("soar_rast_backward_occ_plan_cleared: dL_dout_occ / dL_docc must not be NULL"); return 1; }
+    if (occ_planes != 1 && occ_planes != 3) { set_error("soar_rast_backward_occ_plan_cleared: occ_planes is 3 or 1, got %d", occ_planes); return 1; }
+    return backward_impl(prm, means3D, radii, shs, colors_precomp, scales, rotations, cov3D_precomp, geom_buffer, binning_buffer, image_buffer,
+                         num_rendered, dL_dout_color, dL_dout_normal, dL_dout_depth, dL_dout_opac, nullptr, dL_dmeans2D, dL_dcolors,
+                         dL_dopacity, dL_dmeans3D, dL_dcov3D, dL_dsh, dL_dscales, dL_drotations, dL_dviewmat, dL_dprojmat, dL_dcampos, workspace,
+                         workspace_bytes, dL_dout_occ, dL_docc, normal_scale_dev, occ_planes, region, stream_, rows_cleared != 0);
 }
 
 int soar_rast_backward_region_counts(int64_t *single_blocks, int64_t *pairs)
diff --git a/soar_amd/csrc/lbs_knn.hip b/soar_amd/csrc/lbs_knn.hip
--- a/soar_amd/csrc/lbs_knn.hip
+++ b/soar_amd/csrc/lbs_knn.hip
@@ -1,3 +1,4 @@
+#include "adam_update.h"
 #include "soar_common.h"
 
 #include <cstdio>
@@ -737,9 +738,17 @@
 #define SOAR_KNN_CERT_PAIRS 2
 #endif
 constexpr int KNN_CERT_PAIRS = SOAR_KNN_CERT_PAIRS;
-__global__ void __launch_bounds__(KNN_WAVES *WAVE)
-knn_certify_kernel(const float *__restrict__ xyz, int P, const float4 *__restrict__ sorted_verts, const uint32_t *__restrict__ order,
-                   KnnStatePtrs st)
+struct KnnAdamXyz {
+    float *param;
+    const float *grad;
+    float *exp_avg, *exp_avg_sq;
+    float lr;
+    AdamState st;
+    AdamCoef coef;
+};
+template <bool ADAM>
+__device__ __forceinline__ void knn_certify_body(const float *xyz, int P, const float4 *__restrict__ sorted_verts,
+                                                 const uint32_t *__restrict__ order, const KnnStatePtrs &st, const KnnAdamXyz &adam)
 {
     const int wave = threadIdx.x >> 6, lane = threadIdx.x & 63, l5 = lane & (KNN_KEEP - 1);
     const int q_base = ((int)blockIdx.x * KNN_WAVES + wave) * (2 * KNN_CERT_PAIRS) + (lane >> 5);
@@ -747,6 +756,9 @@
     int qs[KNN_CERT_PAIRS];
     float4 ra[KNN_CERT_PAIRS], rb[KNN_CERT_PAIRS], vv[KNN_CERT_PAIRS];
     float xs[KNN_CERT_PAIRS], ys[KNN_CERT_PAIRS], zs[KNN_CERT_PAIRS];
+    int ps[ADAM ? KNN_CERT_PAIRS : 1];
+    float gg[ADAM ? KNN_CERT_PAIRS : 1][3], mm[ADAM ? KNN_CERT_PAIRS : 1][3], ww[ADAM ? KNN_CERT_PAIRS : 1][3];
+    (void)ps; (void)gg; (void)mm; (void)ww;
 #pragma unroll
     for (int i = 0; i < KNN_CERT_PAIRS; i++) {
         qs[i] = q_base + 2 * i;
@@ -756,11 +768,28 @@
         ra[i] = st.ref30[qc]; rb[i] = st.ref32[qc];
         xs[i] = xyz[3 * p]; ys[i] = xyz[3 * p + 1]; zs[i] = xyz[3 * p + 2];
         vv[i] = sorted_verts[pos];
+        if constexpr (ADAM) {
+            ps[i] = p;
+#pragma unroll
+            for (int c = 0; c < 3; c++) { gg[i][c] = adam.grad[3 * p + c]; mm[i][c] = adam.exp_avg[3 * p + c]; ww[i][c] = adam.exp_avg_sq[3 * p + c]; }
+        }
     }
 #pragma unroll
     for (int i = 0; i < KNN_CERT_PAIRS; i++) {
         const int q = qs[i];
         const bool valid = q < P;
+        if constexpr (ADAM) {
+            const float step_size = adam.lr / adam.st.bias_correction1, bc2s = adam.st.bias_correction2_sqrt;
+            adam_update_element(gg[i][0], xs[i], mm[i][0], ww[i][0], step_size, bc2s, adam.coef);
+            adam_update_element(gg[i][1], ys[i], mm[i][1], ww[i][1], step_size, bc2s, adam.coef);
+            adam_update_element(gg[i][2], zs[i], mm[i][2], ww[i][2], step_size, bc2s, adam.coef);
+            if (valid && l5 == 0) {
+                const size_t at = 3 * (size_t)ps[i];
+                adam.param[at] = xs[i]; adam.param[at + 1] = ys[i]; adam.param[at + 2] = zs[i];
+#pragma unroll
+                for (int c = 0; c < 3; c++) { adam.exp_avg[at + c] = mm[i][c]; adam.exp_avg_sq[at + c] = ww[i][c]; }
+            }
+        }
         const float x = xs[i], y = ys[i], z = zs[i];
         const float d2 = dist2_exact(x, y, z, vv[i]);
         const float ax = x - ra[i].x, ay = y - ra[i].y, az = z - ra[i].z, bx = x - rb[i].x, by = y - rb[i].y, bz = z - rb[i].z;
@@ -788,17 +817,73 @@
     }
 }
 
+__global__ void __launch_bounds__(KNN_WAVES *WAVE)
+knn_certify_kernel(const float *__restrict__ xyz, int P, const float4 *__restrict__ sorted_verts, const uint32_t *__restrict__ order,
+                   KnnStatePtrs st)
+{
+    knn_certify_body<false>(xyz, P, sorted_verts, order, st, KnnAdamXyz{});
+}
+
+constexpr int KNN_ZERO_MAX = MAX_BATCH * 4;
+constexpr size_t KNN_ZERO_BLOCK_WORDS = 256 * 4 * 8;
+struct KnnRiders {
+    unsigned first, adam_blocks, gather_blocks, zero_blocks;
+    AdamTable tab;
+    AdamState st;
+    AdamCoef coef;
+    AdamGather ga;
+    int n_zero;
+    uint32_t *zero_ptr[KNN_ZERO_MAX];
+    size_t zero_words[KNN_ZERO_MAX];
+    unsigned zero_first[KNN_ZERO_MAX + 1];
+};
+__device__ __forceinline__ void knn_rider_workgroup(const KnnRiders &rd, unsigned blk)
+{
+    static_assert(KNN_WAVES * WAVE == 256, "the riders' workgroups are those of adam_update_kernel / zero_ranges_kernel");
+    if (blk < rd.adam_blocks) { adam_rows_workgroup(rd.tab, &rd.st, rd.coef, (int64_t)blk); return; }
+    blk -= rd.adam_blocks;
+    if (blk < rd.gather_blocks) { adam_gather_workgroup(rd.ga, (int)blk); return; }
+    blk -= rd.gather_blocks;
+    if (blk >= rd.zero_blocks) return;
+    int r = 0;
+    while (r + 1 < rd.n_zero && blk >= rd.zero_first[r + 1]) r++;
+    const size_t b0 = (size_t)(blk - rd.zero_first[r]) * KNN_ZERO_BLOCK_WORDS;
+    uint32_t *p = rd.zero_ptr[r];
+    const size_t n = rd.zero_words[r];
+    if (b0 + KNN_ZERO_BLOCK_WORDS <= n && (reinterpret_cast<uintptr_t>(p) & 15) == 0) {
+#pragma unroll
+        for (int u = 0; u < 8; u++) *reinterpret_cast<uint4 *>(p + b0 + (size_t)u * 1024 + threadIdx.x * 4) = make_uint4(0u, 0u, 0u, 0u);
+    } else {
+        for (size_t w = b0 + threadIdx.x; w < n && w < b0 + KNN_ZERO_BLOCK_WORDS; w += 256) p[w] = 0u;
+    }
+}
+
+__global__ void __launch_bounds__(KNN_WAVES *WAVE)
+knn_certify_step_kernel(float *xyz, int P, const float4 *__restrict__ sorted_verts, const uint32_t *__restrict__ order, KnnStatePtrs st,
+                        KnnAdamXyz ax, KnnRiders rd)
+{
+    if (blockIdx.x >= rd.first) { knn_rider_workgroup(rd, blockIdx.x - rd.first); return; }
+    knn_certify_body<true>(xyz, P, sorted_verts, order, st, ax);
+}
+__global__ void __launch_bounds__(KNN_WAVES *WAVE)
+knn_certify_riders_kernel(const float *xyz, int P, const float4 *__restrict__ sorted_verts, const uint32_t *__restrict__ order, KnnStatePtrs st,
+                          KnnRiders rd)
+{
+    if (blockIdx.x >= rd.first) { knn_rider_workgroup(rd, blockIdx.x - rd.first); return; }
+    knn_certify_body<false>(xyz, P, sorted_verts, order, st, KnnAdamXyz{});
+}
+
 #ifndef SOAR_KNN_SEARCH_BLOCKS
 #define SOAR_KNN_SEARCH_BLOCKS 768
 #endif
 #ifndef SOAR_KNN_BS_WPE
 #define SOAR_KNN_BS_WPE 4
 #endif
-__global__ void __launch_bounds__(KNN_WAVES *WAVE) __attribute__((amdgpu_waves_per_eu(SOAR_KNN_BS_WPE, 8)))
-knn_blend_search_kernel(const float *__restrict__ xyz, int P, int search_blocks, const GridMeta *__restrict__ meta,
-                        const uint2 *__restrict__ cell_range, const float4 *__restrict__ sorted_verts, const float *__restrict__ rows_padded,
-                        int J, const uint32_t *__restrict__ order, KnnStatePtrs st, float *__restrict__ weights_out,
-                        uint32_t *__restrict__ counters)
+__device__ __forceinline__ void
+knn_blend_search_body(const float *__restrict__ xyz, int P, int search_blocks, const GridMeta *__restrict__ meta,
+                      const uint2 *__restrict__ cell_range, const float4 *__restrict__ sorted_verts, const float *__restrict__ rows_padded,
+                      int J, const uint32_t *__restrict__ order, const KnnStatePtrs &st, float *__restrict__ weights_out,
+                      uint32_t *__restrict__ counters)
 {
     constexpr int KEEP = KNN_KEEP;
     __shared__ uint32_t c_pos[KNN_WAVES][RF_CAP];
@@ -1042,6 +1127,25 @@
     }
 }
 
+__global__ void __launch_bounds__(KNN_WAVES *WAVE) __attribute__((amdgpu_waves_per_eu(SOAR_KNN_BS_WPE, 8)))
+knn_blend_search_kernel(const float *__restrict__ xyz, int P, int search_blocks, const GridMeta *__restrict__ meta,
+                        const uint2 *__restrict__ cell_range, const float4 *__restrict__ sorted_verts, const float *__restrict__ rows_padded,
+                        int J, const uint32_t *__restrict__ order, KnnStatePtrs st, float *__restrict__ weights_out,
+                        uint32_t *__restrict__ counters)
+{
+    knn_blend_search_body(xyz, P, search_blocks, meta, cell_range, sorted_verts, rows_padded, J, order, st, weights_out, counters);
+}
+
+__global__ void __launch_bounds__(KNN_WAVES *WAVE) __attribute__((amdgpu_waves_per_eu(SOAR_KNN_BS_WPE, 8)))
+knn_blend_search_riders_kernel(const float *__restrict__ xyz, int P, int search_blocks, const GridMeta *__restrict__ meta,
+                               const uint2 *__restrict__ cell_range, const float4 *__restrict__ sorted_verts,
+                               const float *__restrict__ rows_padded, int J, const uint32_t *__restrict__ order, KnnStatePtrs st,
+                               float *__restrict__ weights_out, uint32_t *__restrict__ counters, KnnRiders rd)
+{
+    if (blockIdx.x >= rd.first) { knn_rider_workgroup(rd, blockIdx.x - rd.first); return; }
+    knn_blend_search_body(xyz, P, search_blocks, meta, cell_range, sorted_verts, rows_padded, J, order, st, weights_out, counters);
+}
+
 }
 
 }
@@ -1320,6 +1424,101 @@
     return 0;
 }
 
+extern "C" int soar_lbs_knn_refresh_step(const void *grid_buffer, int32_t V, int32_t J, float *xyz, int32_t P, const uint32_t *order,
+                                         void *state_buffer, float *weights_out, uint32_t *searched_counter_dev, const SoarKnnStepRiders *rd_host,
+                                         void *stream_)
+{
+    hipStream_t stream = static_cast<hipStream_t>(stream_);
+    if (check_knn_sizes(P, V, J, KNN_K)) return 1;
+    if (J > KNN_JMAX) { set_error("soar_lbs_knn_refresh_step: J <= %d", KNN_JMAX); return 1; }
+    if (V < KNN_STATE_STRIDE) { set_error("soar_lbs_knn_refresh_step: the neighbour state keeps %d vertices per query, V=%d", KNN_STATE_STRIDE, V); return 1; }
+    if (!rd_host) { set_error("soar_lbs_knn_refresh_step: riders is NULL (soar_lbs_knn_refresh is the plain form)"); return 1; }
+    if (P == 0) { set_error("soar_lbs_knn_refresh_step: P = 0: nothing would carry the riders"); return 1; }
+    if (!grid_buffer || !xyz || !weights_out || !state_buffer) { set_error("soar_lbs_knn_refresh_step: NULL pointer"); return 1; }
+    if (check_ws("soar_lbs_knn_refresh_step", state_buffer, 0)) return 1;
+    const SoarKnnStepRiders &h = *rd_host;
+    KnnRiders rd = {};
+    KnnAdamXyz ax = {};
+    const bool adam = h.n_rows > 0;
+    int64_t adam_blocks = 0;
+    if (adam) {
+        if (h.n_rows > ADAM_MAX_ROWS || !h.rows || h.step < 1 || h.xyz_row < 0 || h.xyz_row >= h.n_rows) {
+            set_error("soar_lbs_knn_refresh_step: 1 <= n_rows <= %d, rows given, 0 <= xyz_row < n_rows, step >= 1", ADAM_MAX_ROWS);
+            return 1;
+        }
+        const SoarAdamRow &x = h.rows[h.xyz_row];
+        if (x.param != xyz || x.count != 3 * (int64_t)P || !x.grad || !x.exp_avg || !x.exp_avg_sq) {
+            set_error("soar_lbs_knn_refresh_step: row %d must be the positions themselves ([P,3] at xyz) with gradient and moments", h.xyz_row);
+            return 1;
+        }
+        SoarAdamRow others[ADAM_MAX_ROWS];
+        int n_others = 0;
+        for (int r = 0; r < h.n_rows; r++)
+            if (r != h.xyz_row) others[n_others++] = h.rows[r];
+        if (!adam_fill(rd.tab, n_others, others, ADAM_MAX_ROWS, adam_blocks, "soar_lbs_knn_refresh_step")) return 1;
+        rd.st = adam_state_at(h.beta1, h.beta2, h.step);
+        rd.coef = AdamCoef{(float)h.beta2, (float)(1.0 - h.beta1), (float)(1.0 - h.beta2), (float)h.eps};
+        ax.param = x.param; ax.grad = x.grad; ax.exp_avg = x.exp_avg; ax.exp_avg_sq = x.exp_avg_sq; ax.lr = x.lr;
+        ax.st = rd.st; ax.coef = rd.coef;
+    }
+    if (h.n_frames) {
+        if (h.n_frames < 0 || h.n_frames > MAX_BATCH || h.num_frames_seq <= 0 || h.floats_per_frame <= 0 || !h.frame_ids || !h.table || !h.mats_out) {
+            set_error("soar_lbs_knn_refresh_step: bad gather arguments (at most %d frames per step)", MAX_BATCH);
+            return 1;
+        }
+        rd.ga.n_frames = h.n_frames; rd.ga.num_frames_seq = h.num_frames_seq; rd.ga.floats_per_frame = h.floats_per_frame; rd.ga.n_sets = h.n_sets;
+        for (int f = 0; f < h.n_frames; f++) rd.ga.id[f] = h.frame_ids[f];
+        rd.ga.table = h.table; rd.ga.mats_out = h.mats_out; rd.ga.set_out = h.set_index_out;
+    }
+    if (h.n_zero < 0 || h.n_zero > KNN_ZERO_MAX || (h.n_zero && !h.zero)) {
+        set_error("soar_lbs_knn_refresh_step: 0 <= n_zero <= %d ranges", KNN_ZERO_MAX);
+        return 1;
+    }
+    size_t zero_blocks = 0;
+    rd.n_zero = h.n_zero;
+    for (int r = 0; r < h.n_zero; r++) {
+        if (!h.zero[r].ptr || (h.zero[r].bytes & 3) || (reinterpret_cast<uintptr_t>(h.zero[r].ptr) & 3)) {
+            set_error("soar_lbs_knn_refresh_step: zero range %d: a non-NULL, 4-byte aligned pointer and a multiple of 4 bytes", r);
+            return 1;
+        }
+        rd.zero_ptr[r] = static_cast<uint32_t *>(h.zero[r].ptr);
+        rd.zero_words[r] = h.zero[r].bytes / 4;
+        rd.zero_first[r] = (unsigned)zero_blocks;
+        zero_blocks += (rd.zero_words[r] + KNN_ZERO_BLOCK_WORDS - 1) / KNN_ZERO_BLOCK_WORDS;
+    }
+    for (int r = h.n_zero; r <= KNN_ZERO_MAX; r++) rd.zero_first[r] = (unsigned)zero_blocks;
+    if (adam_blocks + zero_blocks > (size_t)1 << 30) { set_error("soar_lbs_knn_refresh_step: too many rider workgroups"); return 1; }
+    rd.adam_blocks = (unsigned)adam_blocks; rd.gather_blocks = (unsigned)h.n_frames; rd.zero_blocks = (unsigned)zero_blocks;
+    const unsigned riders = rd.adam_blocks + rd.gather_blocks + rd.zero_blocks;
+    KnnGrid g;
+    if (carve_knn_grid(const_cast<void *>(grid_buffer), V, &g, stream)) return 1;
+    KnnState st;
+    carve_knn_state(state_buffer, P, &st);
+    StageTimer timer(ST_LBS_KNN, stream);
+    const int per_block = KNN_WAVES * 2 * KNN_CERT_PAIRS, nblocks = (P + per_block - 1) / per_block;
+    const int search_blocks = SOAR_KNN_SEARCH_BLOCKS, blend_blocks = (P + KNN_WAVES * KNN_FSLOTS - 1) / (KNN_WAVES * KNN_FSLOTS);
+    const bool in_cert = h.in_certify != 0 && riders > 0, in_blend = !in_cert && riders > 0;
+    rd.first = (unsigned)nblocks;
+    if (adam)
+        hipLaunchKernelGGL(knn_certify_step_kernel, dim3((unsigned)nblocks + (in_cert ? riders : 0u)), dim3(KNN_WAVES * WAVE), 0, stream, xyz, P,
+                           g.sorted_verts, order, st.p, ax, rd);
+    else if (in_cert)
+        hipLaunchKernelGGL(knn_certify_riders_kernel, dim3((unsigned)nblocks + riders), dim3(KNN_WAVES * WAVE), 0, stream, (const float *)xyz, P,
+                           g.sorted_verts, order, st.p, rd);
+    else
+        hipLaunchKernelGGL(knn_certify_kernel, dim3(nblocks), dim3(KNN_WAVES * WAVE), 0, stream, (const float *)xyz, P, g.sorted_verts, order, st.p);
+    rd.first = (unsigned)(search_blocks + blend_blocks);
+    if (in_blend)
+        hipLaunchKernelGGL(knn_blend_search_riders_kernel, dim3((unsigned)(search_blocks + blend_blocks) + riders), dim3(KNN_WAVES * WAVE), 0, stream,
+                           (const float *)xyz, P, search_blocks, g.meta, g.cell_range, g.sorted_verts, g.rows, J, order, st.p, weights_out,
+                           searched_counter_dev, rd);
+    else
+        hipLaunchKernelGGL(knn_blend_search_kernel, dim3(search_blocks + blend_blocks), dim3(KNN_WAVES * WAVE), 0, stream, (const float *)xyz, P,
+                           search_blocks, g.meta, g.cell_range, g.sorted_verts, g.rows, J, order, st.p, weights_out, searched_counter_dev);
+    SOAR_LAUNCH_OK("lbs_knn_refresh_step", stream, 0);
+    return 0;
+}
+
 extern "C" int soar_lbs_knn_weights_bytes(int32_t P, int32_t V, size_t *bytes)
 {
     if (P < 0 || V <= 0 || !bytes) { set_error("soar_lbs_knn_weights_bytes: bad arguments"); return 1; }
diff --git a/soar_amd/csrc/optim.hip b/soar_amd/csrc/optim.hip
--- a/soar_amd/csrc/optim.hip
+++ b/soar_amd/csrc/optim.hip
@@ -1,27 +1,24 @@
-#include "soar_common.h"
+#include "adam_update.h"
 
 #include <cmath>
 #include <cstdint>
 
 namespace soar {
 
+AdamState adam_state_at(double beta1, double beta2, int64_t step)
+{
+    AdamState st;
+    st.step = (int32_t)step;
+    st.bias_correction1 = (float)(1.0 - pow(beta1, (double)step));
+    st.bias_correction2_sqrt = (float)sqrt(1.0 - pow(beta2, (double)step));
+    st.pad = 0;
+    return st;
+}
+
 namespace {
 
-constexpr int ADAM_MAX_ROWS = 8;
 constexpr int ADAM_MAX_ROWS_WIDE = 40;
-template <int N>
-struct AdamTableT {
-    SoarAdamRow row[N];
-    int64_t first_block[N + 1];
-    int n;
-};
-using AdamTable = AdamTableT<ADAM_MAX_ROWS>;
 using AdamTableWide = AdamTableT<ADAM_MAX_ROWS_WIDE>;
-struct AdamState {
-    int32_t step;
-    float bias_correction1, bias_correction2_sqrt;
-    int32_t pad;
-};
 
 __global__ void adam_tick_kernel(AdamState *st, double beta1, double beta2)
 {
@@ -31,81 +28,16 @@
     st->bias_correction2_sqrt = (float)sqrt(1.0 - pow(beta2, (double)t));
 }
 
-struct AdamGather {
-    int n_frames, num_frames_seq, floats_per_frame, n_sets;
-    int64_t first_block;
-    int32_t id[MAX_BATCH];
-    const float *table;
-    float *mats_out;
-    int32_t *set_out;
-};
-
 template <typename Table>
 __global__ void __launch_bounds__(256) adam_update_kernel(Table tab, const AdamState *__restrict__ st_dev, AdamState st_host, float beta2,
                                                           float one_minus_b1, float one_minus_b2, float eps, AdamGather ga)
 {
     if (ga.n_frames && (int64_t)blockIdx.x >= ga.first_block) {
-        const int f = (int)((int64_t)blockIdx.x - ga.first_block);
-        int id = ga.id[f] % ga.num_frames_seq;
-        if (id < 0) id += ga.num_frames_seq;
-        for (int k = threadIdx.x; k < ga.floats_per_frame; k += 256)
-            ga.mats_out[(size_t)f * ga.floats_per_frame + k] = ga.table[(size_t)id * ga.floats_per_frame + k];
-        if (threadIdx.x == 0 && ga.set_out) ga.set_out[f] = ga.n_sets > 0 ? id % ga.n_sets : 0;
+        adam_gather_workgroup(ga, (int)((int64_t)blockIdx.x - ga.first_block));
         return;
     }
     const AdamState *st = st_dev ? st_dev : &st_host;
-    if (st->step <= 0) return;
-    int r = 0;
-    while (r + 1 < tab.n && (int64_t)blockIdx.x >= tab.first_block[r + 1]) r++;
-    const SoarAdamRow row = tab.row[r];
-    const int64_t i0 = ((int64_t)blockIdx.x - tab.first_block[r]) * 1024 + threadIdx.x * 4;
-    const float step_size = row.lr / st->bias_correction1, bc2s = st->bias_correction2_sqrt;
-    auto update = [&](float g, float &p, float &m, float &v) {
-#pragma clang fp contract(off)
-        m = m + (g - m) * one_minus_b1;
-        v = beta2 * v + one_minus_b2 * (g * g);
-        const float denom = sqrtf(v) / bc2s + eps;
-        p = p - step_size * (m / denom);
-    };
-    const bool vec = i0 + 3 < row.count && (((uintptr_t)row.param | (uintptr_t)row.grad | (uintptr_t)row.exp_avg | (uintptr_t)row.exp_avg_sq) & 15u) == 0u;
-    if (vec) {
-        const float4 g = *reinterpret_cast<const float4 *>(row.grad + i0);
-        float4 p = *reinterpret_cast<const float4 *>(row.param + i0), m = *reinterpret_cast<const float4 *>(row.exp_avg + i0),
-               v = *reinterpret_cast<const float4 *>(row.exp_avg_sq + i0);
-        update(g.x, p.x, m.x, v.x); update(g.y, p.y, m.y, v.y); update(g.z, p.z, m.z, v.z); update(g.w, p.w, m.w, v.w);
-        *reinterpret_cast<float4 *>(row.param + i0) = p;
-        *reinterpret_cast<float4 *>(row.exp_avg + i0) = m;
-        *reinterpret_cast<float4 *>(row.exp_avg_sq + i0) = v;
-        return;
-    }
-    for (int k = 0; k < 4; k++) {
-        const int64_t i = i0 + k;
-        if (i >= row.count) break;
-        float p = row.param[i], m = row.exp_avg[i], v = row.exp_avg_sq[i];
-        update(row.grad[i], p, m, v);
-        row.param[i] = p;
-        row.exp_avg[i] = m;
-        row.exp_avg_sq[i] = v;
-    }
-}
-
-template <typename Table>
-bool adam_fill(Table &tab, int32_t n_rows, const SoarAdamRow *rows_host, int max_rows, int64_t &blocks, const char *who)
-{
-    tab.n = n_rows;
-    blocks = 0;
-    for (int r = 0; r < n_rows; r++) {
-        const SoarAdamRow &w = rows_host[r];
-        if (w.count < 0 || (w.count && (!w.param || !w.grad || !w.exp_avg || !w.exp_avg_sq))) {
-            set_error("%s: row %d has a NULL pointer or a negative count", who, r);
-            return false;
-        }
-        tab.row[r] = w;
-        tab.first_block[r] = blocks;
-        blocks += (w.count + 1023) / 1024;
-    }
-    for (int r = n_rows; r <= max_rows; r++) tab.first_block[r] = blocks;
-    return true;
+    adam_rows_workgroup(tab, st, AdamCoef{beta2, one_minus_b1, one_minus_b2, eps}, (int64_t)blockIdx.x);
 }
 
 }
@@ -153,24 +85,9 @@
         return 1;
     }
     AdamTable tab;
-    tab.n = n_rows;
     int64_t blocks = 0;
-    for (int r = 0; r < n_rows; r++) {
-        const SoarAdamRow &w = rows_host[r];
-        if (w.count < 0 || (w.count && (!w.param || !w.grad || !w.exp_avg || !w.exp_avg_sq))) {
-            set_error("soar_adam_step_at: row %d has a NULL pointer or a negative count", r);
-            return 1;
-        }
-        tab.row[r] = w;
-        tab.first_block[r] = blocks;
-        blocks += (w.count + 1023) / 1024;
-    }
-    for (int r = n_rows; r <= ADAM_MAX_ROWS; r++) tab.first_block[r] = blocks;
-    AdamState st;
-    st.step = (int32_t)step;
-    st.bias_correction1 = (float)(1.0 - pow(beta1, (double)step));
-    st.bias_correction2_sqrt = (float)sqrt(1.0 - pow(beta2, (double)step));
-    st.pad = 0;
+    if (!adam_fill(tab, n_rows, rows_host, ADAM_MAX_ROWS, blocks, "soar_adam_step_at")) return 1;
+    const AdamState st = adam_state_at(beta1, beta2, step);
     AdamGather ga = {};
     if (gather) { ga = *gather; ga.first_block = blocks; }
     StageTimer timer(ST_OPTIMIZER, stream);
diff --git a/soar_amd/hip_lib.py b/soar_amd/hip_lib.py
--- a/soar_amd/hip_lib.py
+++ b/soar_amd/hip_lib.py
@@ -35,6 +35,18 @@
 class SoarAdamRow(C.Structure):
     _fields_ = [("param", _vp), ("grad", _vp), ("exp_avg", _vp), ("exp_avg_sq", _vp), ("count", C.c_int64), ("lr", C.c_float),
                 ("pad_", C.c_int32)]
+
+
+class SoarZeroRange(C.Structure):
+    _fields_ = [("ptr", _vp), ("bytes", C.c_size_t)]
+
+
+class SoarKnnStepRiders(C.Structure):
+    _fields_ = [("n_rows", C.c_int32), ("xyz_row", C.c_int32), ("rows", C.POINTER(SoarAdamRow)),
+                ("beta1", C.c_double), ("beta2", C.c_double), ("eps", C.c_double), ("step", C.c_int64),
+                ("n_frames", C.c_int32), ("num_frames_seq", C.c_int32), ("floats_per_frame", C.c_int32), ("n_sets", C.c_int32),
+                ("frame_ids", C.POINTER(C.c_int32)), ("table", _vp), ("mats_out", _vp), ("set_index_out", _vp),
+                ("n_zero", C.c_int32), ("in_certify", C.c_int32), ("zero", C.POINTER(SoarZeroRange))]
 
 
 class SoarPoseArgs(C.Structure):
@@ -186,6 +198,11 @@
                                 + [_vp] * 11 + [_vp, C.c_size_t, _vp]),
     "soar_rast_backward_occ_plan": (C.c_int, [C.POINTER(SoarRastParams), C.c_int32] + [_vp] * 7 + [_vp, _vp, _vp, C.c_int64] + [_vp] * 6
                                     + [C.c_int32] + [_vp] * 12 + [_vp, C.c_size_t, _vp]),
+    "soar_rast_backward_plan_cleared": (C.c_int, [C.POINTER(SoarRastParams), C.c_int32, C.c_int32] + [_vp] * 7 + [_vp, _vp, _vp, C.c_int64]
+                                        + [_vp] * 4 + [_vp] * 11 + [_vp, C.c_size_t, _vp]),
+    "soar_rast_backward_occ_plan_cleared": (C.c_int, [C.POINTER(SoarRastParams), C.c_int32, C.c_int32] + [_vp] * 7 + [_vp, _vp, _vp, C.c_int64]
+                                            + [_vp] * 6 + [C.c_int32] + [_vp] * 12 + [_vp, C.c_size_t, _vp]),
+    "soar_rast_backward_zero_ranges": (C.c_int, [C.POINTER(SoarRastParams), _vp, _vp, _vp, _vp, C.POINTER(SoarZeroRange), C.POINTER(C.c_int32)]),
     "soar_rast_backward_region_counts": (C.c_int, [C.POINTER(C.c_int64), C.POINTER(C.c_int64)]),
     "soar_batch_begin": (C.c_int, [C.c_int32]),
     "soar_batch_frame": (C.c_int, [C.c_int32]),
@@ -204,6 +221,7 @@
     "soar_lbs_knn_state_bytes": (C.c_int, [C.c_int32, C.POINTER(C.c_size_t)]),
     "soar_lbs_knn_query_state": (C.c_int, [_vp, C.c_int32, _vp, C.c_int32, _vp, C.c_int32, _vp, C.c_int32, _vp, _vp, _vp, C.c_size_t, _vp]),
     "soar_lbs_knn_refresh": (C.c_int, [_vp, C.c_int32, C.c_int32, _vp, C.c_int32, _vp, _vp, _vp, _vp, _vp]),
+    "soar_lbs_knn_refresh_step": (C.c_int, [_vp, C.c_int32, C.c_int32, _vp, C.c_int32, _vp, _vp, _vp, _vp, C.POINTER(SoarKnnStepRiders), _vp]),
     "soar_lbs_warp_forward": (C.c_int, [_vp] * 6 + [C.c_int32, C.c_int32] + [_vp] * 4),
     "soar_lbs_warp_backward": (C.c_int, [_vp] * 5 + [C.c_int32, C.c_int32] + [_vp] * 5),
     "soar_lbs_warp_forward_batch": (C.c_int, [_vp] * 4 + [C.c_int32] * 3 + [_vp] * 3),
diff --git a/soar_amd/lbs.py b/soar_amd/lbs.py
--- a/soar_amd/lbs.py
+++ b/soar_amd/lbs.py
@@ -109,6 +109,20 @@
                                                  ptr(self.searched), stream), "soar_lbs_knn_refresh")
         self.calls += 1
         return out
+
+    def refresh_step(self, xyz: torch.Tensor, out: torch.Tensor, riders, stream: Optional[int] = None) -> torch.Tensor:
+        import ctypes as C
+        g = self.grid
+        stream = _stream(xyz.device) if stream is None else stream
+        if self.refresh_is_full():
+            raise RuntimeError("KnnFollower.refresh_step: this call is a full search; it carries nothing")
+        check(hip_lib.lib().soar_lbs_knn_refresh_step(ptr(g.buffer), g.V, g.J, ptr(xyz), self.P, ptr(self.order), ptr(self.state), ptr(out),
+                                                      ptr(self.searched), C.byref(riders), stream), "soar_lbs_knn_refresh_step")
+        self.calls += 1
+        return out
+
+    def refresh_is_full(self) -> bool:
+        return self.calls == 0 or self.calls % self.RESORT_EVERY == 0
 
     def __call__(self, xyz: torch.Tensor, out: Optional[torch.Tensor] = None) -> torch.Tensor:
         _need_hip(xyz, "xyz")
diff --git a/soar_amd/optim.py b/soar_amd/optim.py
--- a/soar_amd/optim.py
+++ b/soar_amd/optim.py
@@ -36,6 +36,13 @@
             rows[k].count, rows[k].lr = p.numel(), self.lr[n]
         return rows
 
+    def begin_step_rows(self):
+        if self.device_counter:
+            raise ValueError("a step carried by another launch needs the host step counter (device_counter = False)")
+        self.flat.check_views()
+        self.steps += 1
+        return self._table(self.names), self.names.index("xyz"), self.steps
+
     def step(self, stream: Optional[int] = None, names=None, advance: bool = True, gather=None) -> None:
         self.flat.check_views()
         dev = self.flat.flat.device
diff --git a/soar_amd/step_plan.py b/soar_amd/step_plan.py
--- a/soar_amd/step_plan.py
+++ b/soar_amd/step_plan.py
@@ -116,6 +116,11 @@
         if self.loss_in_tail:
             self._loss_finish = (hip_lib.SoarLossFinish * self.n)()
         self.gather_in_adam = fold and self.n <= 8 and os.environ.get("SOAR_PLAN_GATHER_IN_ADAM", "1") != "0"
+        self.adam_in_knn = fold and self.n <= 8 and os.environ.get("SOAR_PLAN_ADAM_IN_KNN", "1") != "0"
+        self.zero_in_knn = fold and self.n <= 8 and os.environ.get("SOAR_PLAN_ZERO_IN_KNN", "1") != "0"
+        self.riders_in_certify = os.environ.get("SOAR_PLAN_KNN_RIDERS", "blend") == "certify"
+        self.folded = dict(adam=False, zero=False)
+        self._rows_cleared = False
         self._call_cache = {}
         self.optimizer = None
         self.optimizer_in_two_parts = None
@@ -240,7 +245,19 @@
         n_sets = int(self.pool.shape[0]) if self.pool is not None else 0
         return (self.n, s.num_frames, 55 * 16, n_sets, (C.c_int32 * self.n)(*self._frames_now), ptr(s.cano2live), ptr(self.mats), ptr(self.frame_sel))
 
-    def _prologue(self, stream: int, resort: bool = True, gathered: bool = False) -> None:
+    def _zero_ranges(self):
+        out = (hip_lib.SoarZeroRange * (4 * self.n))()
+        k = 0
+        for v in self.views:
+            four, n = (hip_lib.SoarZeroRange * 4)(), C.c_int32(0)
+            check(self.L.soar_rast_backward_zero_ranges(C.byref(self.ctx.params), ptr(v["work"]), ptr(v["g_view"]), ptr(v["g_proj"]),
+                                                        ptr(v["g_campos"]), four, C.byref(n)), "backward_zero_ranges")
+            for r in range(n.value):
+                out[k].ptr, out[k].bytes = four[r].ptr, four[r].bytes
+                k += 1
+        return out, k
+
+    def _prologue(self, stream: int, resort: bool = True, gathered: bool = False, opt=None, zero: bool = False) -> None:
         L, s = self.L, self.seq
         self._stamp(0, stream)
         n_sets = int(self.pool.shape[0]) if self.pool is not None else 0
@@ -255,6 +272,24 @@
                                             ptr(self.frame_sel), stream), "gather_step_inputs")
         if resort:
             self.knn.full(s.xyz.detach(), self.blend_weights, stream)
+        elif opt is not None or zero:
+            rd = hip_lib.SoarKnnStepRiders()
+            keep = []
+            if opt is not None:
+                rows, xyz_row, step = opt.begin_step_rows()
+                rd.n_rows, rd.xyz_row, rd.rows, rd.step = len(rows), xyz_row, rows, step
+                rd.beta1, rd.beta2, rd.eps = opt.betas[0], opt.betas[1], opt.eps
+                if gathered:
+                    n, num, width, sets, ids, table, mats, sel = self._gather_args()
+                    rd.n_frames, rd.num_frames_seq, rd.floats_per_frame, rd.n_sets = n, num, width, sets
+                    rd.frame_ids, rd.table, rd.mats_out, rd.set_index_out = ids, table, mats, sel
+                    keep.append(ids)
+            if zero:
+                ranges, n_ranges = self._zero_ranges()
+                rd.n_zero, rd.zero = n_ranges, ranges
+            rd.in_certify = 1 if self.riders_in_certify else 0
+            self.knn.calls = 1
+            self.knn.refresh_step(s.xyz.detach(), self.blend_weights, rd, stream)
         else:
             self.knn.calls = 1
             self.knn.refresh(s.xyz.detach(), self.blend_weights, stream)
@@ -327,26 +362,34 @@
     def _f_backward(self, i: int, stream: int) -> None:
         def build():
             L, s, v = self.L, self.seq, self.views[i]
-            return (L.soar_rast_backward_plan, (C.byref(self.ctx.params), self.bwd_region, ptr(v["xyz_p"]), ptr(v["radii"]), None,
+            if self._rows_cleared:
+                head = (L.soar_rast_backward_plan_cleared, (C.byref(self.ctx.params), self.bwd_region, 1))
+            else:
+                head = (L.soar_rast_backward_plan, (C.byref(self.ctx.params), self.bwd_region))
+            return (head[0], head[1] + (ptr(v["xyz_p"]), ptr(v["radii"]), None,
                                                 ptr(s.colors.detach()), ptr(s.scales.detach()), ptr(v["rot_p"]), None, ptr(v["geom"]),
                                                 ptr(v["binning"]), ptr(v["img"]), self.capacity, ptr(v["gC"]), ptr(v["gN"]), ptr(v["gD"]),
                                                 ptr(v["gO"]), ptr(v["g_means2D"]), ptr(self.g_colors[i]), ptr(v["g_opacity"]),
                                                 ptr(v["g_means3D"]), ptr(v["g_cov3D"]), None, ptr(self.g_scales[i]), ptr(v["g_rot_p"]),
                                                 ptr(v["g_view"]), ptr(v["g_proj"]), ptr(v["g_campos"]), ptr(v["work"]), v["work"].numel(),
                                                 stream), "backward")
-        self._call(("backward", i, stream), build)
+        self._call(("backward", i, stream, self._rows_cleared), build)
 
     def _f_backward_occ(self, i: int, stream: int) -> None:
         def build():
             L, s, v = self.L, self.seq, self.views[i]
-            return (L.soar_rast_backward_occ_plan, (C.byref(self.ctx.params), self.bwd_region, ptr(v["xyz_p"]), ptr(v["radii"]), None, ptr(s.colors.detach()),
+            if self._rows_cleared:
+                head = (L.soar_rast_backward_occ_plan_cleared, (C.byref(self.ctx.params), self.bwd_region, 1))
+            else:
+                head = (L.soar_rast_backward_occ_plan, (C.byref(self.ctx.params), self.bwd_region))
+            return (head[0], head[1] + (ptr(v["xyz_p"]), ptr(v["radii"]), None, ptr(s.colors.detach()),
                                                ptr(s.scales.detach()), ptr(v["rot_p"]), None, ptr(v["geom"]), ptr(v["binning"]), ptr(v["img"]),
                                                self.capacity, ptr(v["gC"]), ptr(v["gN"]), ptr(v["gD"]), ptr(v["gO"]), ptr(v["g_occ_img"]),
                                                self.av_cos_scale_all.data_ptr() + 4 * i, 1, ptr(v["g_means2D"]), ptr(self.g_colors[i]), ptr(v["g_opacity"]), ptr(v["g_means3D"]),
                                                ptr(v["g_cov3D"]), None, ptr(self.g_scales[i]), ptr(v["g_rot_p"]), ptr(v["g_view"]),
                                                ptr(v["g_proj"]), ptr(v["g_campos"]), ptr(self.g_occ_all[i]), ptr(v["work"]), v["work"].numel(),
                                                stream), "backward_occ")
-        self._call(("backward_occ", i, stream), build)
+        self._call(("backward_occ", i, stream, self._rows_cleared), build)
 
     def _frame(self, i: int, stream: int) -> None:
         self._stamp(2 + 2 * i, stream)
@@ -459,9 +502,18 @@
             in_flight = in_flight and self.flat.n_buckets > 1
             self.flat.wait_bucket(0)
             ride = opt is not None and self.gather_in_adam and self._ids_by_value and not opt.device_counter
-            if opt is not None:
+            resort = self.steps % self.RESORT_EVERY == 0
+            alone = not self.flat.pending and not self.flat._collectives_on()
+            from .optim import FusedAdam
+            fold_adam = (self.adam_in_knn and opt is not None and not resort and alone and not in_flight and self._ids_by_value
+                         and type(opt) is FusedAdam and opt.flat is self.flat and not opt.device_counter and "xyz" in opt.names
+                         and opt.flat.leaves["xyz"].data_ptr() == self.seq.xyz.data_ptr())
+            fold_zero = self.zero_in_knn and not resort and alone and self._ids_by_value and self.batched
+            self.folded = dict(adam=bool(fold_adam), zero=bool(fold_zero))
+            self._rows_cleared = bool(fold_zero)
+            if opt is not None and not fold_adam:
                 opt.step(main.cuda_stream, names=("xyz",) if in_flight else None, advance=True, gather=self._gather_args() if ride else None)
-            self._prologue(main.cuda_stream, self.steps % self.RESORT_EVERY == 0, gathered=ride)
+            self._prologue(main.cuda_stream, resort, gathered=ride, opt=opt if fold_adam else None, zero=fold_zero)
             self.flat.wait_all()
             if opt is not None and in_flight:
                 opt.step(main.cuda_stream, names=tuple(n for n in opt.names if n != "xyz"), advance=False)
```
